# wang-xinyu/tensorrtx

Measured on AMD Instinct MI355X. Metric: images/sec @ batch=32 640x640 fp16 (yolov8n conv backbone + YoloLayer decode + NMS), higher is better.
Workload: dtype f16

## Files before the change

include/trtx_hip.h:

```cpp
#ifndef TRTX_HIP_H_
#define TRTX_HIP_H_

#include <stddef.h>
#include <stdint.h>

#ifdef __cplusplus
extern "C" {
#endif

#ifndef TRTX_NO_HIP_TYPES
struct ihipStream_t;
typedef struct ihipStream_t* trtx_stream_t;
#endif

#define TRTX_ABI_VERSION 1
#define TRTX_OK 0
#define TRTX_ERR_INVALID 1
#define TRTX_ERR_HIP 2
#define TRTX_ERR_WORKSPACE 3
#define TRTX_ERR_UNSUPPORTED 4
#define TRTX_ERR_NO_DEVICE 5
#define TRTX_ERR_IO 6
#define TRTX_ERR_STATE 7

const char* trtx_status_string(int32_t status);
int32_t trtx_abi_version(void);
int32_t trtx_device_count(void);


size_t trtx_yolo_decode_workspace(int batch, int net_h, int net_w, const int* strides, int n_levels);
int32_t trtx_yolo_decode(const float* const* inputs, int n_levels, int batch, int classes, int net_h, int net_w,
                         const int* strides, int max_out, float* output, void* workspace, size_t workspace_bytes,
                         trtx_stream_t stream);

int32_t trtx_yolo_decode_ex(const float* const* inputs, int n_levels, int batch, int classes, int net_h, int net_w,
                            const int* strides, int max_out, int n_kpt, float kpt_conf, int is_seg, int is_pose, int is_obb,
                            float* output, void* workspace, size_t workspace_bytes, trtx_stream_t stream);
size_t trtx_yolo_head_decode_workspace(int batch, int net_h, int net_w, const int* strides, int n_levels);
int32_t trtx_yolo_head_decode_nhwc(const void* const* heads, const int* ld, int n_levels, int batch, int classes,
                                   int net_h, int net_w, const int* strides, const float* dfl_weights, int max_out,
                                   float* output, void* workspace, size_t workspace_bytes, trtx_stream_t stream);
int32_t trtx_yolo_head_decode_nhwc_f32(const void* const* heads, const int* ld, int n_levels, int batch, int classes,
                                   int net_h, int net_w, const int* strides, const float* dfl_weights, int max_out,
                                   float* output, void* workspace, size_t workspace_bytes, trtx_stream_t stream);
int32_t trtx_yolo_task_head_decode_nhwc(const void* const* heads, const int* ld, const void* const* branches, const int* branch_ld,
                                        int n_levels, int batch, int classes, int net_h, int net_w, const int* strides,
                                        const float* dfl_weights, int max_out, int is_seg, int is_pose, int is_obb, int n_kpt,
                                        float kpt_conf, float* output, void* workspace, size_t workspace_bytes, trtx_stream_t stream);
int32_t trtx_yolo_task_head_decode_nhwc_f32(const void* const* heads, const int* ld, const void* const* branches, const int* branch_ld,
                                            int n_levels, int batch, int classes, int net_h, int net_w, const int* strides,
                                            const float* dfl_weights, int max_out, int is_seg, int is_pose, int is_obb, int n_kpt,
                                            float kpt_conf, float* output, void* workspace, size_t workspace_bytes, trtx_stream_t stream);

size_t trtx_yolo_nms_workspace(int batch);
int32_t trtx_yolo_nms(const float* decode_out, int batch, int max_out, float conf_thresh, float nms_thresh,
                      int32_t* keep_idx, int32_t* keep_cnt, float* keep_det, void* workspace, size_t workspace_bytes,
                      trtx_stream_t stream);


size_t trtx_yolov5_decode_workspace(int batch, const int* grid_w, const int* grid_h, int n_levels);
int32_t trtx_yolov5_decode(const float* const* inputs, int n_levels, int batch, int classes, int net_h, int net_w,
                           const int* grid_w, const int* grid_h, const float* anchors, int max_out, int is_segmentation,
                           float* output, void* workspace, size_t workspace_bytes, trtx_stream_t stream);
size_t trtx_yolov5_head_decode_workspace(int batch, const int* grid_w, const int* grid_h, int n_levels);
int32_t trtx_yolov5_head_decode_nhwc(const void* const* heads, const int* ld, int n_levels, int batch, int classes, int net_h, int net_w,
                                     const int* grid_w, const int* grid_h, const float* anchors, int max_out, float* output,
                                     void* workspace, size_t workspace_bytes, trtx_stream_t stream);
int32_t trtx_yolov5_head_decode_nhwc_f32(const void* const* heads, const int* ld, int n_levels, int batch, int classes, int net_h, int net_w,
                                         const int* grid_w, const int* grid_h, const float* anchors, int max_out, float* output,
                                         void* workspace, size_t workspace_bytes, trtx_stream_t stream);
size_t trtx_yolov7_decode_workspace(int batch, const int* grid_w, const int* grid_h, int n_levels);
int32_t trtx_yolov7_decode(const float* const* inputs, int n_levels, int batch, int classes, int net_h, int net_w,
                           const int* grid_w, const int* grid_h, const float* anchors, int max_out, float* output, void* workspace,
                           size_t workspace_bytes, trtx_stream_t stream);
size_t trtx_yolov7_head_decode_workspace(int batch, const int* grid_w, const int* grid_h, int n_levels);
int32_t trtx_yolov7_head_decode_nhwc(const void* const* heads, const int* ld, int n_levels, int batch, int classes, int net_h, int net_w,
                                     const int* grid_w, const int* grid_h, const float* anchors, int max_out, float* output,
                                     void* workspace, size_t workspace_bytes, trtx_stream_t stream);
int32_t trtx_yolov7_head_decode_nhwc_f32(const void* const* heads, const int* ld, int n_levels, int batch, int classes, int net_h, int net_w,
                                         const int* grid_w, const int* grid_h, const float* anchors, int max_out, float* output,
                                         void* workspace, size_t workspace_bytes, trtx_stream_t stream);
size_t trtx_yolov9_decode_workspace(int batch, int net_h, int net_w);
int32_t trtx_yolov9_decode(const float* const* inputs, int batch, int classes, int net_h, int net_w, int max_out, int is_segmentation,
                           float* output, void* workspace, size_t workspace_bytes, trtx_stream_t stream);
size_t trtx_yolov9_head_decode_workspace(int batch, int net_h, int net_w);
int32_t trtx_yolov9_head_decode_nhwc(const void* const* box, const int* box_ld, const void* const* cls, const int* cls_ld, int batch, int classes,
                                     int net_h, int net_w, const float* dfl_weights, int max_out, float* output, void* workspace,
                                     size_t workspace_bytes, trtx_stream_t stream);
int32_t trtx_yolov9_head_decode_nhwc_f32(const void* const* box, const int* box_ld, const void* const* cls, const int* cls_ld, int batch, int classes,
                                         int net_h, int net_w, const float* dfl_weights, int max_out, float* output, void* workspace,
                                         size_t workspace_bytes, trtx_stream_t stream);
int32_t trtx_yolo_nms_obb(const float* decode_out, int batch, int max_out, float conf_thresh, float nms_thresh, int32_t* keep_idx,
                          int32_t* keep_cnt, float* keep_det, void* workspace, size_t workspace_bytes, trtx_stream_t stream);
int32_t trtx_yolo_postprocess_gpu_obb(const float* decode_out, int batch, int max_out, float conf_thresh, float nms_thresh, float* out,
                                      trtx_stream_t stream);
int32_t trtx_yolov5_nms(const float* decode_out, int batch, int max_out, float conf_thresh, float nms_thresh, int32_t* keep_idx,
                        int32_t* keep_cnt, float* keep_det, void* workspace, size_t workspace_bytes, trtx_stream_t stream);
int32_t trtx_yolov9_nms(const float* decode_out, int batch, int max_out, float conf_thresh, float nms_thresh, int32_t* keep_idx,
                        int32_t* keep_cnt, float* keep_det, void* workspace, size_t workspace_bytes, trtx_stream_t stream);
int32_t trtx_yolov7_nms(const float* decode_out, int batch, int max_out, float conf_thresh, float nms_thresh, int32_t* keep_idx,
                        int32_t* keep_cnt, float* keep_det, void* workspace, size_t workspace_bytes, trtx_stream_t stream);
int32_t trtx_seg_masks(const float* decode_out, int det_floats, int box_format, const int32_t* keep_idx, const int32_t* keep_cnt, int batch,
                       int max_out, int max_keep, const float* proto, int mask_h, int mask_w, int net_h, int net_w, float* masks,
                       trtx_stream_t stream);

void trtx_letterbox_matrix(int src_w, int src_h, int dst_w, int dst_h, float* d2s_out );
int32_t trtx_letterbox_batch(const void* const* src, const int* src_w, const int* src_h, int batch, float* dst, int dst_w, int dst_h,
                             trtx_stream_t stream);
int32_t trtx_preprocess_init(int max_image_size, int ring_depth);
void trtx_preprocess_destroy(void);
int32_t trtx_batch_preprocess(const void* const* src_host, const int* src_w, const int* src_h, int batch, float* dst, int dst_w, int dst_h,
                              trtx_stream_t stream);

int32_t trtx_yolo_postprocess_gpu(const float* decode_out, int batch, int max_out, float conf_thresh, float nms_thresh,
                                  float* out, trtx_stream_t stream);

int32_t trtx_mish(const float* in, float* out, size_t n, trtx_stream_t stream);

size_t trtx_retina_decode_output_floats(int net_h, int net_w);
size_t trtx_retina_decode_workspace(int batch, int net_h, int net_w);
int32_t trtx_retina_decode(const float* const* inputs, int batch, int net_h, int net_w, float* output, void* workspace,
                           size_t workspace_bytes, trtx_stream_t stream);
size_t trtx_retina_nms_workspace(int batch, int net_h, int net_w);
int32_t trtx_retina_nms(const float* decode_out, int batch, int net_h, int net_w, double conf_thresh, float nms_thresh,
                        int max_keep, int32_t* keep_idx, int32_t* keep_cnt, float* keep_det, void* workspace,
                        size_t workspace_bytes, trtx_stream_t stream);

size_t trtx_rpn_decode_workspace(int batch, int num_anchors, int height, int width);
int32_t trtx_rpn_decode(int batch, const float* scores, const float* deltas, int height, int width, int image_height,
                        int image_width, float stride, const float* anchors_host, int num_anchors, int top_n,
                        float* out_scores, float* out_boxes, void* workspace, size_t workspace_bytes,
                        trtx_stream_t stream);
size_t trtx_sorted_nms_workspace(int batch, int n);
int32_t trtx_rpn_nms(int batch, const float* scores, const float* boxes, int pre_nms_topk, int post_nms_topk,
                     float nms_thresh, float* out_boxes, void* workspace, size_t workspace_bytes,
                     trtx_stream_t stream);
int32_t trtx_roi_align(int batch, const float* boxes, const float* features, int pooler_resolution, float spatial_scale,
                       int sampling_ratio, int num_proposals, int channels, int feature_h, int feature_w, float* out,
                       trtx_stream_t stream);
int32_t trtx_roi_align_nhwc_f16(int batch, const float* boxes, const void* features, int ld_in, int pooler_resolution,
                                float spatial_scale, int sampling_ratio, int num_proposals, int channels, int feature_h,
                                int feature_w, void* out, int ld_out, trtx_stream_t stream);
int32_t trtx_roi_align_nhwc_f16_strided(int batch, const float* boxes, const void* features, int ld_in, int pooler_resolution,
                                        float spatial_scale, int sampling_ratio, int num_proposals, int channels, int feature_h,
                                        int feature_w, void* out, int ld_out, int bin_step, trtx_stream_t stream);
size_t trtx_predictor_decode_workspace(int batch, int num_boxes, int num_classes);
int32_t trtx_predictor_decode(int batch, const float* scores, const float* deltas, const float* proposals, int num_boxes,
                              int num_classes, int image_height, int image_width, const float* bbox_reg_weights_host,
                              float* out_scores, float* out_boxes, float* out_classes, void* workspace,
                              size_t workspace_bytes, trtx_stream_t stream);
int32_t trtx_batched_nms(int nms_method, int batch, const float* scores, const float* boxes, const float* classes,
                         int count, int detections_per_im, float nms_thresh, float* out_scores, float* out_boxes,
                         float* out_classes, void* workspace, size_t workspace_bytes, trtx_stream_t stream);

int32_t trtx_mask_rcnn_inference(int batch, const float* labels, const float* masks, int detections_per_im, int output_size,
                                 int num_classes, float* out_masks, trtx_stream_t stream);

#define TRTX_ACT_NONE 0
#define TRTX_ACT_RELU 1
#define TRTX_ACT_SIGMOID 2
#define TRTX_ACT_SILU 3
#define TRTX_ACT_LEAKY 4
#define TRTX_ACT_TANH 5
int32_t trtx_conv_packed_dims(int cout, int cin_pad, int kh, int kw, int32_t* cout_pad, int32_t* kpad, int32_t* bn);
int32_t trtx_conv_pack_weights_f16(const float* w_kcrs, int cout, int cin, int kh, int kw, int cin_pad,
                                   const float* ch_scale, uint16_t* packed);
int32_t trtx_op_conv2d_nhwc_f16(const void* in, int N, int H, int W, int Cin, int ld_in, const void* wpacked,
                                const float* bias, void* out, int Cout, int ld_out, int kh, int kw, int sh, int sw,
                                int ph, int pw, int act1, const void* residual, int ld_res, int act2,
                                trtx_stream_t stream);
int32_t trtx_op_conv2d_tactics(int N, int H, int W, int Cin, int ld_in, int Cout, int ld_out, int kh, int kw, int sh, int sw, int ph, int pw,
                               int has_residual, int ld_res, int32_t* out6, int32_t max_out);
int32_t trtx_op_conv_force_tactic(const int32_t* tactic6);
int32_t trtx_op_conv_stem_nchw_f16(const float* in, int N, int C, int H, int W, const float* w_taps_cout, const float* bias, void* out, int Cout,
                                   int ld_out, int k, int stride, int pad, int act, trtx_stream_t stream);
int32_t trtx_op_conv_stem_pair_f16(const float* in, int N, int C, int H, int W, const float* stem_w_taps_cout, const float* stem_bias, int stem_act,
                                   const void* conv_wpacked, const float* conv_bias, int conv_act, void* out, int ld_out, trtx_stream_t stream);
int32_t trtx_op_conv_bneck_pair_f16(const void* in, int N, int H, int W, int ld_in, int in_coff, const void* w1_packed, const float* bias1, int act1,
                                    const void* w2_packed, const float* bias2, int act2, int shortcut, int act_after, void* out, int ld_out,
                                    trtx_stream_t stream);
int32_t trtx_op_conv_bneck_pair_or_two_f16(const void* in, int N, int H, int W, int ld_in, int in_coff, const void* w1_packed, const float* bias1, int act1,
                                           const void* w2_packed, const float* bias2, int act2, int shortcut, int act_after, void* mid, void* out,
                                           int ld_out, trtx_stream_t stream);
int32_t trtx_reorg_fold_weights(const float* w_kcrs, int cout, int cin, int kh, int kw, float* folded);
int32_t trtx_conv_packed_dims_f32(int cout, int cin_pad, int kh, int kw, int32_t* cout_pad, int32_t* kpad, int32_t* cink);
int32_t trtx_conv_pack_weights_f32(const float* w_kcrs, int cout, int cin, int kh, int kw, int cin_pad, const float* ch_scale, float* packed);
int32_t trtx_op_conv2d_nhwc_f32(const void* in, int N, int H, int W, int Cin, int ld_in, const void* wpacked, const float* bias, void* out, int Cout,
                                int ld_out, int kh, int kw, int sh, int sw, int ph, int pw, int act1, const void* residual, int ld_res, int act2,
                                const int32_t* tile4, trtx_stream_t stream);
int32_t trtx_op_conv2d_tactics_f32(int N, int H, int W, int Cin, int ld_in, int Cout, int ld_out, int kh, int kw, int sh, int sw, int ph, int pw,
                                   int has_residual, int ld_res, int32_t* out4, int32_t max_out);
int32_t trtx_conv_pack_weights_i8(const float* w_kcrs, int cout, int cin, int kh, int kw, const float* ch_scale, int8_t* packed, float* wscale_out,
                                  int32_t* cout_pad_out, int32_t* kpad_out);
int32_t trtx_op_conv2d_nhwc_i8(const void* in, int N, int H, int W, int Cin, int ld_in, const void* wpacked, const float* cscale, const float* bias, void* out,
                               int out_is_i8, float out_inv_scale, int Cout, int ld_out, int kh, int kw, int sh, int sw, int ph, int pw, int act1,
                               const void* residual, int res_is_i8, float res_scale, int ld_res, int act2, trtx_stream_t stream);
int32_t trtx_conv_pack_weights_grouped_f16(const float* w_kcrs, int cout, int cin_g, int kh, int kw, const float* ch_scale, uint16_t* packed,
                                           int32_t* kpad_out);
int32_t trtx_op_conv2d_grouped_nhwc_f16(const void* in, int N, int H, int W, int Cin, int ld_in, const void* wpacked, const float* bias, void* out,
                                        int Cout, int ld_out, int groups, int k, int pad, int act1, const void* residual, int ld_res, int act2,
                                        trtx_stream_t stream);
int32_t trtx_op_conv2d_dw_nhwc(const void* in, int dtype, int N, int H, int W, int C, int ld_in, const float* w_taps_c, const float* bias, void* out, int ld_out,
                               const void* residual, int ld_res, int k, int stride, int pad, int dilation, int act1, float alpha1, int act2, float alpha2,
                               trtx_stream_t stream);
int32_t trtx_op_psa_attention_f16(const void* qkv, int ld_qkv, void* out, int ld_out, void* vimg, int ld_v, int B, int heads, int N, int kd, int hd, float scale,
                                  trtx_stream_t stream);
int32_t trtx_op_area_attention_f16(const void* qkv, int ld_qkv, void* out, int ld_out, void* vimg, int ld_v, int B, int heads, int N, int area, int kd, int hd,
                                   float scale, trtx_stream_t stream);
int32_t trtx_op_area_attention_split_f16(const void* q, int ld_q, const void* k, int ld_k, const void* v, int ld_v, void* out, int ld_out, int B, int heads,
                                         int N, int area, int kd, int hd, float scale, trtx_stream_t stream);
size_t trtx_op_hgconv_workspace_bytes(int B, int N, int D, int E);
int32_t trtx_op_hgconv_geometry(int32_t* tiles, int max_tiles, int32_t* n_tiles);
int32_t trtx_op_hgconv_f16(const void* x, int ld_x, void* out, int ld_out, int B, int N, int D, int E, float logit_scale, const float* w_ctx, const float* b_ctx,
                           const float* proto, const float* w_pre, const float* b_pre, const float* w_edge, const float* b_edge, const float* w_node,
                           const float* b_node, void* workspace, size_t workspace_bytes, trtx_stream_t stream);
int32_t trtx_op_poison_lds(void* device_word, trtx_stream_t stream);
int32_t trtx_op_nchw_f32_to_nhwc_f16(const float* in, void* out, int N, int C, int H, int W, int Cpad, int ld_out,
                                     trtx_stream_t stream);
int32_t trtx_op_nhwc_f16_to_nchw_f32(const void* in, float* out, int N, int C, int H, int W, int ld_in,
                                     trtx_stream_t stream);

typedef struct trtx_builder trtx_builder;
typedef struct trtx_network trtx_network;
typedef struct trtx_hostmem trtx_hostmem;
typedef struct trtx_engine trtx_engine;
typedef struct trtx_context trtx_context;
typedef struct trtx_plugin trtx_plugin;

#define TRTX_MAX_DIMS 8
typedef struct trtx_dims {
    int32_t nb;
    int64_t d[TRTX_MAX_DIMS];
} trtx_dims;

#define TRTX_DTYPE_FLOAT 0
#define TRTX_DTYPE_HALF 1
#define TRTX_DTYPE_INT8 2
#define TRTX_DTYPE_INT32 3
#define TRTX_ACTIVATION_RELU 0
#define TRTX_ACTIVATION_SIGMOID 1
#define TRTX_ACTIVATION_TANH 2
#define TRTX_ACTIVATION_LEAKY_RELU 3
#define TRTX_POOLING_MAX 0
#define TRTX_POOLING_AVERAGE 1
#define TRTX_ELEMENTWISE_SUM 0
#define TRTX_ELEMENTWISE_PROD 1
#define TRTX_ELEMENTWISE_MAX 2
#define TRTX_ELEMENTWISE_MIN 3
#define TRTX_ELEMENTWISE_SUB 4
#define TRTX_ELEMENTWISE_DIV 5
#define TRTX_ELEMENTWISE_POW 6
#define TRTX_SCALE_UNIFORM 0
#define TRTX_SCALE_CHANNEL 1
#define TRTX_SCALE_ELEMENTWISE 2
#define TRTX_REDUCE_SUM 0
#define TRTX_REDUCE_PROD 1
#define TRTX_REDUCE_MAX 2
#define TRTX_REDUCE_MIN 3
#define TRTX_REDUCE_AVG 4
#define TRTX_MATMUL_NONE 0
#define TRTX_MATMUL_TRANSPOSE 1
#define TRTX_MATMUL_VECTOR 2
#define TRTX_UNARY_EXP 0
#define TRTX_UNARY_LAST 23
#define TRTX_RESIZE_NEAREST 0
#define TRTX_RESIZE_LINEAR 1
#define TRTX_FLAG_FP16 0
#define TRTX_FLAG_INT8 1
#define TRTX_P_STRIDE 1
#define TRTX_P_PADDING 2
#define TRTX_P_DILATION 3
#define TRTX_P_GROUPS 4
#define TRTX_P_ALPHA 5
#define TRTX_P_BETA 6
#define TRTX_P_AXIS 7
#define TRTX_P_RESHAPE 8
#define TRTX_P_FIRST_TRANSPOSE 9
#define TRTX_P_SECOND_TRANSPOSE 10
#define TRTX_P_RESIZE_MODE 11
#define TRTX_P_RESIZE_SCALES 12
#define TRTX_P_RESIZE_OUT_DIMS 13
#define TRTX_P_AVG_EXCLUSIVE 14
#define TRTX_P_KERNEL 15
#define TRTX_P_NB_OUT 16

typedef struct trtx_plugin_vtbl {
    void* self;
    int32_t (*get_nb_outputs)(void* self);
    int32_t (*get_output_dims)(void* self, int32_t index, const trtx_dims* inputs, int32_t nb_inputs, trtx_dims* out);
    int32_t (*configure)(void* self, const trtx_dims* in, int32_t nb_in, const trtx_dims* out, int32_t nb_out,
                         int32_t max_batch);
    int32_t (*initialize)(void* self);
    void (*terminate)(void* self);
    size_t (*workspace_size)(void* self, int32_t max_batch);
    int32_t (*enqueue)(void* self, int32_t batch, const void* const* inputs, void* const* outputs, void* workspace,
                       trtx_stream_t stream);
    size_t (*serialization_size)(void* self);
    void (*serialize)(void* self, void* buffer);
    const char* (*plugin_type)(void* self);
    const char* (*plugin_version)(void* self);
    int32_t (*clone)(void* self, struct trtx_plugin_vtbl* out);
    void (*destroy)(void* self);
} trtx_plugin_vtbl;

typedef struct trtx_plugin_field {
    const char* name;
    const void* data;
    int32_t type;
    int32_t length;
} trtx_plugin_field;

typedef struct trtx_creator_vtbl {
    void* self;
    const char* (*plugin_name)(void* self);
    const char* (*plugin_version)(void* self);
    int32_t (*create)(void* self, const char* name, const trtx_plugin_field* fields, int32_t nb_fields,
                      trtx_plugin_vtbl* out);
    int32_t (*deserialize)(void* self, const char* name, const void* data, size_t length, trtx_plugin_vtbl* out);
} trtx_creator_vtbl;

int32_t trtx_registry_register(const trtx_creator_vtbl* creator);
int32_t trtx_registry_get(const char* name, const char* version, trtx_creator_vtbl* out);

typedef struct trtx_wts trtx_wts;
int32_t trtx_wts_load(const char* path, trtx_wts** out);
int32_t trtx_wts_count(const trtx_wts* w);
int32_t trtx_wts_entry(const trtx_wts* w, int32_t i, const char** name, const float** values, int64_t* count);
int32_t trtx_wts_find(const trtx_wts* w, const char* name, const float** values, int64_t* count);
void trtx_wts_free(trtx_wts* w);

int32_t trtx_builder_create(trtx_builder** out);
void trtx_builder_destroy(trtx_builder* b);
int32_t trtx_builder_set_max_batch(trtx_builder* b, int32_t n);
int32_t trtx_builder_set_flag(trtx_builder* b, int32_t flag, int32_t on);
int32_t trtx_builder_set_workspace(trtx_builder* b, size_t bytes);
typedef struct trtx_calibrator_vtbl {
    void* self;
    int32_t (*get_batch_size)(void* self);
    int32_t (*get_batch)(void* self, void** bindings, const char* const* names, int32_t nb_bindings);
    const void* (*read_cache)(void* self, size_t* length);
    void (*write_cache)(void* self, const void* cache, size_t length);
    int32_t (*get_algorithm)(void* self);
} trtx_calibrator_vtbl;
int32_t trtx_builder_set_max_aux_streams(trtx_builder* b, int32_t n);
int32_t trtx_builder_set_int8_calibrator(trtx_builder* b, const trtx_calibrator_vtbl* calibrator);
float trtx_int8_entropy_threshold(const double* hist, int32_t bins, float range);
float trtx_int8_clip_limited_threshold(const double* hist, int32_t bins, float range, float thr, double limit);
int32_t trtx_network_create(trtx_builder* b, uint32_t flags, trtx_network** out);
void trtx_network_destroy(trtx_network* n);
const char* trtx_network_last_error(const trtx_network* n);

int32_t trtx_add_input(trtx_network* n, const char* name, int32_t dtype, const trtx_dims* dims);
int32_t trtx_add_convolution(trtx_network* n, int32_t input, int32_t nb_out, int32_t kh, int32_t kw,
                             const float* kernel, int64_t kernel_count, const float* bias, int64_t bias_count);
int32_t trtx_add_deconvolution(trtx_network* n, int32_t input, int32_t nb_out, int32_t kh, int32_t kw,
                               const float* kernel, int64_t kernel_count, const float* bias, int64_t bias_count);
int32_t trtx_add_fully_connected(trtx_network* n, int32_t input, int32_t nb_out, const float* kernel,
                                 int64_t kernel_count, const float* bias, int64_t bias_count);
int32_t trtx_add_activation(trtx_network* n, int32_t input, int32_t type);
int32_t trtx_add_pooling(trtx_network* n, int32_t input, int32_t type, int32_t kh, int32_t kw);
int32_t trtx_add_scale(trtx_network* n, int32_t input, int32_t mode, const float* shift, int64_t shift_count,
                       const float* scale, int64_t scale_count, const float* power, int64_t power_count);
int32_t trtx_add_elementwise(trtx_network* n, int32_t a, int32_t b, int32_t op);
int32_t trtx_add_concatenation(trtx_network* n, const int32_t* inputs, int32_t nb_inputs);
int32_t trtx_add_slice(trtx_network* n, int32_t input, const trtx_dims* start, const trtx_dims* size,
                       const trtx_dims* stride);
int32_t trtx_add_shuffle(trtx_network* n, int32_t input);
int32_t trtx_add_resize(trtx_network* n, int32_t input);
int32_t trtx_add_softmax(trtx_network* n, int32_t input);
int32_t trtx_add_matrix_multiply(trtx_network* n, int32_t a, int32_t op_a, int32_t b, int32_t op_b);
int32_t trtx_add_constant(trtx_network* n, const trtx_dims* dims, const float* values, int64_t count);
int32_t trtx_add_reduce(trtx_network* n, int32_t input, int32_t op, uint32_t axes, int32_t keep_dims);
int32_t trtx_add_identity(trtx_network* n, int32_t input);
int32_t trtx_network_add_unary(trtx_network* n, int32_t input, int32_t op);
int32_t trtx_add_plugin_v2(trtx_network* n, const int32_t* inputs, int32_t nb_inputs, const trtx_plugin_vtbl* plugin);

int32_t trtx_layer_nb_outputs(const trtx_network* n, int32_t layer);
int32_t trtx_layer_output(const trtx_network* n, int32_t layer, int32_t index);
int32_t trtx_layer_set_name(trtx_network* n, int32_t layer, const char* name);
int32_t trtx_layer_set_ints(trtx_network* n, int32_t layer, int32_t param, const int32_t* v, int32_t count);
int32_t trtx_layer_set_floats(trtx_network* n, int32_t layer, int32_t param, const float* v, int32_t count);
int32_t trtx_layer_set_dims(trtx_network* n, int32_t layer, int32_t param, const trtx_dims* d);
int32_t trtx_tensor_get_dims(const trtx_network* n, int32_t tensor, trtx_dims* out);
int32_t trtx_tensor_set_name(trtx_network* n, int32_t tensor, const char* name);
const char* trtx_tensor_get_name(const trtx_network* n, int32_t tensor);
int32_t trtx_mark_output(trtx_network* n, int32_t tensor);

int32_t trtx_build_serialized(trtx_builder* b, trtx_network* n, trtx_hostmem** out);
const void* trtx_hostmem_data(const trtx_hostmem* m);
size_t trtx_hostmem_size(const trtx_hostmem* m);
void trtx_hostmem_destroy(trtx_hostmem* m);
int32_t trtx_hostmem_create(const void* data, size_t size, trtx_hostmem** out);
int32_t trtx_plan_describe(const void* plan, size_t size, int32_t lowered, char** json_out);
void trtx_string_free(char* s);

int32_t trtx_engine_deserialize(const void* plan, size_t size, trtx_engine** out);
int32_t trtx_engine_serialize(const trtx_engine* e, trtx_hostmem** out);
void trtx_engine_destroy(trtx_engine* e);
int32_t trtx_engine_nb_bindings(const trtx_engine* e);
int32_t trtx_engine_binding_index(const trtx_engine* e, const char* name);
const char* trtx_engine_binding_name(const trtx_engine* e, int32_t index);
int32_t trtx_engine_binding_is_input(const trtx_engine* e, int32_t index);
int32_t trtx_engine_binding_dims(const trtx_engine* e, int32_t index, trtx_dims* out);
int32_t trtx_engine_binding_dtype(const trtx_engine* e, int32_t index);
int32_t trtx_engine_max_batch(const trtx_engine* e);
size_t trtx_engine_device_memory(const trtx_engine* e);
int32_t trtx_engine_tactics(const trtx_engine* e, char** json_out);
int32_t trtx_engine_device(const trtx_engine* e);
int32_t trtx_context_create(trtx_engine* e, trtx_context** out);
void trtx_context_destroy(trtx_context* c);
int32_t trtx_context_enqueue(trtx_context* c, int32_t batch, void* const* bindings, trtx_stream_t stream);
int32_t trtx_context_enqueue_frames(trtx_context* c, int32_t batch, const void* const* frames, const int32_t* frame_w, const int32_t* frame_h,
                                    void* const* bindings, trtx_stream_t stream);
int32_t trtx_context_set_tensor_address(trtx_context* c, const char* name, void* ptr);
int32_t trtx_context_enqueue_v3(trtx_context* c, trtx_stream_t stream);
int32_t trtx_context_profile(trtx_context* c, int32_t batch, void* const* bindings, trtx_stream_t stream,
                             char** json_out);

#ifdef __cplusplus
}
#endif
#endif
```

tensorrtx_amd/capi.py:

```python
import ctypes
import os

_HERE = os.path.dirname(os.path.abspath(__file__))
_LIB = None


class TrtxError(RuntimeError):
    def __init__(self, status, what):
        self.status = status
        msg = lib().trtx_status_string(status).decode() if _LIB is not None else "?"
        super().__init__(f"{what}: status {status} ({msg})")


def lib_path() -> str:
    return os.environ.get("TRTX_HIP_LIB") or os.path.join(_HERE, "lib", "libtrtx_hip.so")


def hip_runtimes_mapped():
    seen = []
    with open("/proc/self/maps") as f:
        for line in f:
            path = line.rsplit(" ", 1)[-1].strip()
            if "libamdhip64" in os.path.basename(path) and path not in seen:
                seen.append(path)
# ... 154 lines not shown
        return status
    check(status, "trtx_yolo_task_head_decode_nhwc")
    return out


def yolo_nms_obb(decode_out, max_out=1000, conf_thresh=0.5, nms_thresh=0.45, out=None, ws=None):
    L = lib()
    B = decode_out.shape[0]
    keep_idx, keep_cnt, keep_det, ws = _nms_buffers(B, max_out, 7, decode_out.device, out, ws)
    check(L.trtx_yolo_nms_obb(_p(decode_out), B, max_out, ctypes.c_float(conf_thresh), ctypes.c_float(nms_thresh), _p(keep_idx), _p(keep_cnt),
                              _p(keep_det), _p(ws), ctypes.c_size_t(ws.numel()), _stream()), "trtx_yolo_nms_obb")
    return keep_idx, keep_cnt, keep_det


def yolo_postprocess_gpu_obb(decode_out, max_out=1000, conf_thresh=0.5, nms_thresh=0.45, out=None, ws=None):
    import torch
    if out is None:
        out = torch.empty((decode_out.shape[0], 1 + max_out * 8), dtype=torch.float32, device=decode_out.device)
    check(lib().trtx_yolo_postprocess_gpu_obb(_p(decode_out), decode_out.shape[0], max_out, ctypes.c_float(conf_thresh), ctypes.c_float(nms_thresh),
                                              _p(out), _stream()), "trtx_yolo_postprocess_gpu_obb")
    return out


DET5_FLOATS = 38


def yolov5_decode(inputs, classes, net_h, net_w, grids, anchors, max_out=1000, is_seg=False):
    import numpy as np
    import torch
    L = lib()
    n = len(inputs)
    ins = [x.contiguous() for x in inputs]
    B, dev = ins[0].shape[0], ins[0].device
    arr = (ctypes.c_void_p * n)(*[x.data_ptr() for x in ins])
    gw = (ctypes.c_int * n)(*[g[0] for g in grids])
    gh = (ctypes.c_int * n)(*[g[1] for g in grids])
    an = np.ascontiguousarray(anchors, dtype=np.float32).reshape(n, 6)
    L.trtx_yolov5_decode_workspace.restype = ctypes.c_size_t
    ws_bytes = L.trtx_yolov5_decode_workspace(B, gw, gh, n)
    ws = torch.empty(max(ws_bytes, 256), dtype=torch.uint8, device=dev)
    out = torch.zeros((B, 1 + max_out * DET5_FLOATS), dtype=torch.float32, device=dev)
    check(L.trtx_yolov5_decode(arr, n, B, classes, net_h, net_w, gw, gh, an.ctypes.data_as(ctypes.c_void_p), max_out, 1 if is_seg else 0,
                               _p(out), _p(ws), ctypes.c_size_t(ws_bytes), _stream()), "trtx_yolov5_decode")
    return out


def yolov5_head_decode_nhwc(heads, classes, net_h, net_w, grids, anchors, max_out=1000):
    import numpy as np
    import torch
    L = lib()
    B, n, dev = heads[0].shape[0], len(heads), heads[0].device
    hp, hl = _head_table(heads)
    gw = (ctypes.c_int * n)(*[g[0] for g in grids])
    gh = (ctypes.c_int * n)(*[g[1] for g in grids])
    an = np.ascontiguousarray(anchors, dtype=np.float32).reshape(n, 6)
    L.trtx_yolov5_head_decode_workspace.restype = ctypes.c_size_t
    ws_bytes = L.trtx_yolov5_head_decode_workspace(B, gw, gh, n)
    ws = torch.empty(max(ws_bytes, 256), dtype=torch.uint8, device=dev)
    out = torch.zeros((B, 1 + max_out * DET5_FLOATS), dtype=torch.float32, device=dev)
    fn = L.trtx_yolov5_head_decode_nhwc_f32 if heads[0].dtype == torch.float32 else L.trtx_yolov5_head_decode_nhwc
    check(fn(hp, hl, n, B, classes, net_h, net_w, gw, gh, an.ctypes.data_as(ctypes.c_void_p), max_out, _p(out), _p(ws), ctypes.c_size_t(ws_bytes),
             _stream()), "trtx_yolov5_head_decode_nhwc")
    return out


def yolov5_nms(decode_out, max_out=1000, conf_thresh=0.5, nms_thresh=0.45, out=None, ws=None):
    L = lib()
    B = decode_out.shape[0]
    keep_idx, keep_cnt, keep_det, ws = _nms_buffers(B, max_out, 6, decode_out.device, out, ws)
    check(L.trtx_yolov5_nms(_p(decode_out), B, max_out, ctypes.c_float(conf_thresh), ctypes.c_float(nms_thresh), _p(keep_idx), _p(keep_cnt),
                            _p(keep_det), _p(ws), ctypes.c_size_t(ws.numel()), _stream()), "trtx_yolov5_nms")
    return keep_idx, keep_cnt, keep_det


def reorg_fold_weights(w):
    import numpy as np
    w = np.ascontiguousarray(w, dtype=np.float32)
    cout, c4, kh, kw = w.shape
    out = np.empty((cout, c4 // 4, 2 * kh, 2 * kw), dtype=np.float32)
    check(lib().trtx_reorg_fold_weights(w.ctypes.data_as(ctypes.c_void_p), cout, c4 // 4, kh, kw, out.ctypes.data_as(ctypes.c_void_p)),
          "trtx_reorg_fold_weights")
    return out


DET7_FLOATS = 6


def _grid_tables(grids, anchors, n):
    import numpy as np
    gw = (ctypes.c_int * max(n, 1))(*[g[0] for g in grids[:n]])
    gh = (ctypes.c_int * max(n, 1))(*[g[1] for g in grids[:n]])
    an = np.ascontiguousarray(anchors, dtype=np.float32).reshape(-1, 6)
    return gw, gh, an


def yolov7_decode(inputs, classes, net_h, net_w, grids, anchors, max_out=1000, out=None):
    import torch
    L = lib()
    n = len(inputs)
    ins = [x.contiguous() for x in inputs]
    B, dev = ins[0].shape[0], ins[0].device
    arr = (ctypes.c_void_p * n)(*[x.data_ptr() for x in ins])
    gw, gh, an = _grid_tables(grids, anchors, n)
    L.trtx_yolov7_decode_workspace.restype = ctypes.c_size_t
    ws_bytes = L.trtx_yolov7_decode_workspace(B, gw, gh, n)
    ws = torch.empty(max(ws_bytes, 256), dtype=torch.uint8, device=dev)
    if out is None:
        out = torch.zeros((B, 1 + max_out * DET7_FLOATS), dtype=torch.float32, device=dev)
    check(L.trtx_yolov7_decode(arr, n, B, classes, net_h, net_w, gw, gh, an.ctypes.data_as(ctypes.c_void_p), max_out, _p(out), _p(ws),
                               ctypes.c_size_t(ws_bytes), _stream()), "trtx_yolov7_decode")
    return out


def yolov7_head_decode_workspace(batch, grids):
    L = lib()
    n = len(grids)
    gw, gh, _ = _grid_tables(grids, [0.0] * 6 * n, n)
    L.trtx_yolov7_head_decode_workspace.restype = ctypes.c_size_t
    return L.trtx_yolov7_head_decode_workspace(batch, gw, gh, n)


def yolov7_head_decode_nhwc(heads, classes, net_h, net_w, grids, anchors, max_out=1000, out=None, ws=None, ld=None, n_levels=None,
                            status_only=False):
    import torch
    L = lib()
    B, n, dev = heads[0].shape[0], len(heads), heads[0].device
    hp, hl = _head_table(heads)
    if ld is not None:
        hl = (ctypes.c_int * n)(*ld)
    gw, gh, an = _grid_tables(grids, anchors, n)
    if ws is None:
        ws = torch.empty(max(yolov7_head_decode_workspace(B, grids), 256), dtype=torch.uint8, device=dev)
    if out is None:
        out = torch.zeros((B, 1 + max_out * DET7_FLOATS), dtype=torch.float32, device=dev)
    fn = L.trtx_yolov7_head_decode_nhwc_f32 if heads[0].dtype == torch.float32 else L.trtx_yolov7_head_decode_nhwc
    st = fn(hp, hl, n if n_levels is None else n_levels, B, classes, net_h, net_w, gw, gh, an.ctypes.data_as(ctypes.c_void_p), max_out, _p(out),
            _p(ws), ctypes.c_size_t(ws.numel()), _stream())
    if status_only:
        return st
    check(st, "trtx_yolov7_head_decode_nhwc")
    return out


def yolov7_nms(decode_out, max_out=1000, conf_thresh=0.5, nms_thresh=0.45, out=None, ws=None):
    L = lib()
    B = decode_out.shape[0]
    keep_idx, keep_cnt, keep_det, ws = _nms_buffers(B, max_out, 6, decode_out.device, out, ws)
    check(L.trtx_yolov7_nms(_p(decode_out), B, max_out, ctypes.c_float(conf_thresh), ctypes.c_float(nms_thresh), _p(keep_idx), _p(keep_cnt),
                            _p(keep_det), _p(ws), ctypes.c_size_t(ws.numel()), _stream()), "trtx_yolov7_nms")
    return keep_idx, keep_cnt, keep_det


def yolov9_decode(inputs, classes, net_h, net_w, max_out=1000, is_seg=False, out=None):
    import torch
    L = lib()
    ins = [x.contiguous() for x in inputs]
    assert len(ins) == 3 and all(x.is_cuda and x.dtype == torch.float32 for x in ins)
    B, dev = ins[0].shape[0], ins[0].device
    arr = (ctypes.c_void_p * 3)(*[x.data_ptr() for x in ins])
    L.trtx_yolov9_decode_workspace.restype = ctypes.c_size_t
    ws_bytes = L.trtx_yolov9_decode_workspace(B, net_h, net_w)
    ws = torch.empty(max(ws_bytes, 256), dtype=torch.uint8, device=dev)
    if out is None:
        out = torch.zeros((B, 1 + max_out * DET5_FLOATS), dtype=torch.float32, device=dev)
    check(L.trtx_yolov9_decode(arr, B, classes, net_h, net_w, max_out, 1 if is_seg else 0, _p(out), _p(ws), ctypes.c_size_t(ws_bytes), _stream()),
          "trtx_yolov9_decode")
    return out


def yolov9_head_decode_nhwc(box, cls, classes, net_h, net_w, dfl_w, max_out=1000, out=None, batch=None, box_ld=None, cls_ld=None, ws=None):
    import torch
    L = lib()
    assert len(box) == 3 and len(cls) == 3
    B = box[0].shape[0] if batch is None else batch
    dev = box[0].device
    bp = (ctypes.c_void_p * 3)(*[x.data_ptr() for x in box])
    cp = (ctypes.c_void_p * 3)(*[x.data_ptr() for x in cls])
    bl = (ctypes.c_int * 3)(*(box_ld if box_ld is not None else [x.shape[-1] for x in box]))
    cl = (ctypes.c_int * 3)(*(cls_ld if cls_ld is not None else [x.shape[-1] for x in cls]))
    L.trtx_yolov9_head_decode_workspace.restype = ctypes.c_size_t
    if ws is None:
        ws = torch.empty(max(L.trtx_yolov9_head_decode_workspace(B, net_h, net_w), 256), dtype=torch.uint8, device=dev)
    if out is None:
        out = torch.zeros((B, 1 + max_out * DET5_FLOATS), dtype=torch.float32, device=dev)
    fn = L.trtx_yolov9_head_decode_nhwc_f32 if box[0].dtype == torch.float32 else L.trtx_yolov9_head_decode_nhwc
    check(fn(bp, bl, cp, cl, B, classes, net_h, net_w, _p(dfl_w), max_out, _p(out), _p(ws), ctypes.c_size_t(ws.numel()), _stream()),
          "trtx_yolov9_head_decode_nhwc")
    return out


def yolov9_nms(decode_out, max_out=1000, conf_thresh=0.5, nms_thresh=0.45, out=None, ws=None):
    L = lib()
    B = decode_out.shape[0]
    keep_idx, keep_cnt, keep_det, ws = _nms_buffers(B, max_out, 6, decode_out.device, out, ws)
    check(L.trtx_yolov9_nms(_p(decode_out), B, max_out, ctypes.c_float(conf_thresh), ctypes.c_float(nms_thresh), _p(keep_idx), _p(keep_cnt),
                            _p(keep_det), _p(ws), ctypes.c_size_t(ws.numel()), _stream()), "trtx_yolov9_nms")
    return keep_idx, keep_cnt, keep_det


def seg_masks(decode_out, keep_idx, keep_cnt, proto, net_h, net_w, max_keep, box_format=0, out=None):
    import torch
    B, max_out = keep_idx.shape
    assert decode_out.shape[0] == B and (decode_out.shape[1] - 1) % max_out == 0
    det_floats = (decode_out.shape[1] - 1) // max_out
    assert proto.dim() == 4 and proto.shape[0] == B and proto.shape[1] == 32
    mask_h, mask_w = int(proto.shape[2]), int(proto.shape[3])
    for t, dt in ((decode_out, torch.float32), (keep_idx, torch.int32), (keep_cnt, torch.int32), (proto, torch.float32)):
        assert t.is_cuda and t.dtype == dt and t.is_contiguous()
    if out is None:
        out = torch.zeros((B, max(max_keep, 0), mask_h, mask_w), dtype=torch.float32, device=proto.device)
    assert out.is_cuda and out.dtype == torch.float32 and out.is_contiguous() and out.numel() >= B * max(max_keep, 0) * mask_h * mask_w
    check(lib().trtx_seg_masks(_p(decode_out), det_floats, box_format, _p(keep_idx), _p(keep_cnt), B, max_out, max_keep, _p(proto), mask_h,
                               mask_w, net_h, net_w, _p(out), _stream()), "trtx_seg_masks")
    return out


def yolo_postprocess_gpu(decode_out, max_out=1000, conf_thresh=0.5, nms_thresh=0.45, out=None, ws=None):
    import torch
    B = decode_out.shape[0]
    if out is None:
        out = torch.empty((B, 1 + max_out * 7), dtype=torch.float32, device=decode_out.device)
    check(lib().trtx_yolo_postprocess_gpu(_p(decode_out), B, max_out, ctypes.c_float(conf_thresh), ctypes.c_float(nms_thresh),
                                          _p(out), _stream()), "trtx_yolo_postprocess_gpu")
    return out


ACT = {"none": 0, "relu": 1, "sigmoid": 2, "silu": 3, "leaky": 4, "tanh": 5, "mish": 6}


def _hw(v):
    if isinstance(v, (tuple, list)):
        h, w = v
        return int(h), int(w)
    return int(v), int(v)


def pack_conv_weights_f16(w_kcrs, cin_pad=None, ch_scale=None):
    import numpy as np
    L = lib()
    w = np.ascontiguousarray(w_kcrs, dtype=np.float32)
    cout, cin, kh, kw = w.shape
    cin_pad = cin_pad or (cin + 7) // 8 * 8
    cp, kp, bn = ctypes.c_int32(), ctypes.c_int32(), ctypes.c_int32()
    check(L.trtx_conv_packed_dims(cout, cin_pad, kh, kw, ctypes.byref(cp), ctypes.byref(kp), ctypes.byref(bn)),
          "trtx_conv_packed_dims")
    packed = np.zeros((cp.value, kp.value), dtype=np.uint16)
    sc = None
    if ch_scale is not None:
        sc = np.ascontiguousarray(ch_scale, dtype=np.float32)
    check(L.trtx_conv_pack_weights_f16(w.ctypes.data_as(ctypes.c_void_p), cout, cin, kh, kw, cin_pad,
                                       sc.ctypes.data_as(ctypes.c_void_p) if sc is not None else None,
                                       packed.ctypes.data_as(ctypes.c_void_p)), "trtx_conv_pack_weights_f16")
    return packed, cp.value, kp.value, bn.value


def conv2d_nhwc_f16(x, wpacked, bias, cout, kh, kw, stride, pad, act1="none", residual=None, act2="none",
                    out=None, out_ld=None):
    import torch
    L = lib()
    N, H, W, Cin = x.shape
    (sh, sw), (ph, pw) = _hw(stride), _hw(pad)
    Ho = (H + 2 * ph - kh) // sh + 1
    Wo = (W + 2 * pw - kw) // sw + 1
    if out is None:
        out = torch.empty((N, Ho, Wo, cout), dtype=torch.float16, device=x.device)
    ld_out = out_ld or out.shape[-1]
    check(L.trtx_op_conv2d_nhwc_f16(_p(x), N, H, W, Cin, x.stride(2), _p(wpacked), _p(bias), _p(out), cout, ld_out,
                                    kh, kw, sh, sw, ph, pw, ACT[act1], _p(residual),
                                    residual.stride(2) if residual is not None else 0, ACT[act2], _stream()),
          "trtx_op_conv2d_nhwc_f16")
    return out


def stem_weights(w_kcrs):
    import numpy as np
    w = np.ascontiguousarray(w_kcrs, dtype=np.float32)
    return np.ascontiguousarray(w.reshape(w.shape[0], -1).T)


def conv_stem_nchw_f16(x, w_taps_cout, bias, k, stride, pad, act="none", out=None, out_ld=None):
    import torch
    N, C, H, W = x.shape
    cout = w_taps_cout.shape[1]
    Ho, Wo = (H + 2 * pad - k) // stride + 1, (W + 2 * pad - k) // stride + 1
    if out is None:
        out = torch.empty((N, Ho, Wo, cout), dtype=torch.float16, device=x.device)
    check(lib().trtx_op_conv_stem_nchw_f16(_p(x), N, C, H, W, _p(w_taps_cout), _p(bias), _p(out), cout, out_ld or out.shape[-1], k, stride, pad,
                                           ACT[act], _stream()), "trtx_op_conv_stem_nchw_f16")
    return out


def conv_stem_pair_f16(x, stem_w_taps_cout, stem_bias, conv_wpacked, conv_bias, stem_act="silu", conv_act="silu", out=None, out_ld=None):
    import torch
    N, C, H, W = x.shape
    Hi, Wi = (H - 1) // 2 + 1, (W - 1) // 2 + 1
    Ho, Wo = (Hi - 1) // 2 + 1, (Wi - 1) // 2 + 1
    if out is None:
        out = torch.empty((N, Ho, Wo, 32), dtype=torch.float16, device=x.device)
    check(lib().trtx_op_conv_stem_pair_f16(_p(x), N, C, H, W, _p(stem_w_taps_cout), _p(stem_bias), ACT[stem_act], _p(conv_wpacked), _p(conv_bias),
                                           ACT[conv_act], _p(out), out_ld or out.shape[-1], _stream()), "trtx_op_conv_stem_pair_f16")
    return out


def conv_bneck_pair_f16(x, w1_packed, bias1, w2_packed, bias2, act1="silu", act2="silu", shortcut=True, act_after="none", out=None, out_ld=None, in_coff=None,
                        mid=None):
    import torch
    N, H, W, C = x.shape
    assert x.dtype == torch.float16 and x.stride(3) == 1 and (C == 16 if in_coff is None else in_coff + 16 <= C)
    if out is None:
        out = torch.empty((N, H, W, 16), dtype=torch.float16, device=x.device)
    head = (_p(x), N, H, W, x.stride(2), in_coff or 0, _p(w1_packed), _p(bias1), ACT[act1], _p(w2_packed), _p(bias2), ACT[act2], 1 if shortcut else 0, ACT[act_after])
    if mid is None:
        check(lib().trtx_op_conv_bneck_pair_f16(*head, _p(out), out_ld or out.shape[-1], _stream()), "trtx_op_conv_bneck_pair_f16")
    else:
        assert mid.dtype == torch.float16 and mid.is_contiguous() and tuple(mid.shape) == (N, H, W, 16)
        check(lib().trtx_op_conv_bneck_pair_or_two_f16(*head, _p(mid), _p(out), out_ld or out.shape[-1], _stream()), "trtx_op_conv_bneck_pair_or_two_f16")
    return out


def pack_conv_weights_grouped_f16(w_kcrs, ch_scale=None):
    import numpy as np
    L = lib()
    w = np.ascontiguousarray(w_kcrs, dtype=np.float32)
    cout, cin_g, kh, kw = w.shape
    kp = ctypes.c_int32()
    check(L.trtx_conv_pack_weights_grouped_f16(w.ctypes.data_as(ctypes.c_void_p), cout, cin_g, kh, kw, None, None, ctypes.byref(kp)),
          "trtx_conv_pack_weights_grouped_f16 (dims)")
    packed = np.zeros((cout, kp.value), dtype=np.uint16)
    sc = None if ch_scale is None else np.ascontiguousarray(ch_scale, dtype=np.float32)
    check(L.trtx_conv_pack_weights_grouped_f16(w.ctypes.data_as(ctypes.c_void_p), cout, cin_g, kh, kw,
                                               sc.ctypes.data_as(ctypes.c_void_p) if sc is not None else None,
                                               packed.ctypes.data_as(ctypes.c_void_p), ctypes.byref(kp)), "trtx_conv_pack_weights_grouped_f16")
    return packed


def conv2d_grouped_nhwc_f16(x, wpacked, bias, cout, groups, k, pad, act1="none", residual=None, act2="none", out=None, out_ld=None):
    import torch
    N, H, W, Cin = x.shape
    if out is None:
        out = torch.empty((N, H + 2 * pad - k + 1, W + 2 * pad - k + 1, cout), dtype=torch.float16, device=x.device)
    check(lib().trtx_op_conv2d_grouped_nhwc_f16(_p(x), N, H, W, Cin, x.stride(2), _p(wpacked), _p(bias), _p(out), cout, out_ld or out.shape[-1], groups, k,
                                                pad, ACT[act1], _p(residual), residual.stride(2) if residual is not None else 0, ACT[act2], _stream()),
          "trtx_op_conv2d_grouped_nhwc_f16")
    return out


def conv2d_dw_nhwc(x, w, bias, k, stride, act1="none", residual=None, act2="none", out=None, out_ld=None, alpha1=0.1, alpha2=0.1, pad=None, dilation=1):
    import numpy as np
    import torch
    N, H, W, C = x.shape
    assert x.dtype in (torch.float16, torch.float32) and (residual is None or residual.dtype == x.dtype)
    pad = k // 2 if pad is None else pad
    Ho, Wo = (H + 2 * pad - dilation * (k - 1) - 1) // stride + 1, (W + 2 * pad - dilation * (k - 1) - 1) // stride + 1
    taps = np.ascontiguousarray(np.asarray(w, dtype=np.float32).reshape(C, k * k).T)
    wg = torch.from_numpy(taps).to(x.device)
    if out is None:
        out = torch.empty((N, Ho, Wo, C), dtype=x.dtype, device=x.device)
    assert out.dtype == x.dtype
    check(lib().trtx_op_conv2d_dw_nhwc(_p(x), 1 if x.dtype == torch.float16 else 0, N, H, W, C, x.stride(2), _p(wg), _p(bias), _p(out),
                                       out_ld or out.shape[-1], _p(residual), residual.stride(2) if residual is not None else 0, k, stride, pad, dilation,
                                       ACT[act1], ctypes.c_float(alpha1), ACT[act2], ctypes.c_float(alpha2), _stream()), "trtx_op_conv2d_dw_nhwc")
    return out


def _attention(fn, what, qkv, heads, scale, out, vimg, out_ld, v_ld, qkv_ld, kd, hd, extra):
    import torch
    B, N, _ = qkv.shape
    for t in (qkv, out, vimg):
        assert t.is_cuda and t.dtype == torch.float16
    check(fn(_p(qkv), qkv_ld or qkv.stride(1), _p(out), out_ld or out.stride(1), _p(vimg), v_ld or vimg.stride(1), B, heads, N, *extra, kd, hd,
             ctypes.c_float(scale), _stream()), what)
    return out, vimg


def psa_attention(qkv, heads, scale, out=None, vimg=None, out_ld=None, v_ld=None, qkv_ld=None, kd=32, hd=64):
    import torch
    B, N, _ = qkv.shape
    out = torch.empty((B, N, heads * hd), dtype=torch.float16, device=qkv.device) if out is None else out
    vimg = torch.empty((B, N, heads * hd), dtype=torch.float16, device=qkv.device) if vimg is None else vimg
    return _attention(lib().trtx_op_psa_attention_f16, "trtx_op_psa_attention_f16", qkv, heads, scale, out, vimg, out_ld, v_ld, qkv_ld, kd, hd, ())


def area_attention(qkv, heads, area, scale, out=None, vimg=None, out_ld=None, v_ld=None, qkv_ld=None, kd=32, hd=32):
    import torch
    B, N, _ = qkv.shape
    out = torch.empty((B, N, heads * hd), dtype=torch.float16, device=qkv.device) if out is None else out
    vimg = torch.empty((B, N, heads * hd), dtype=torch.float16, device=qkv.device) if vimg is None else vimg
    return _attention(lib().trtx_op_area_attention_f16, "trtx_op_area_attention_f16", qkv, heads, scale, out, vimg, out_ld, v_ld, qkv_ld, kd, hd, (area,))


def area_attention_split(q, k, v, heads, area, scale, out=None, q_ld=None, k_ld=None, v_ld=None, out_ld=None, kd=32, hd=32):
    import torch
    B, N, _ = q.shape
    out = torch.empty((B, N, heads * hd), dtype=torch.float16, device=q.device) if out is None else out
    for t in (q, k, v, out):
        assert t.is_cuda and t.dtype == torch.float16
    check(lib().trtx_op_area_attention_split_f16(_p(q), q_ld or q.stride(1), _p(k), k_ld or k.stride(1), _p(v), v_ld or v.stride(1), _p(out),
                                                 out_ld or out.stride(1), B, heads, N, area, kd, hd, ctypes.c_float(scale), _stream()),
          "trtx_op_area_attention_split_f16")
    return out


HGCONV_WEIGHTS = ("w_ctx", "b_ctx", "proto", "w_pre", "b_pre", "w_edge", "b_edge", "w_node", "b_node")


def hgconv_workspace_bytes(B, N, D, E):
    L = lib()
    L.trtx_op_hgconv_workspace_bytes.restype = ctypes.c_size_t
    return int(L.trtx_op_hgconv_workspace_bytes(int(B), int(N), int(D), int(E)))


def hgconv_geometry():
    arr, n = (ctypes.c_int32 * 8)(), ctypes.c_int32()
    check(lib().trtx_op_hgconv_geometry(arr, 8, ctypes.byref(n)), "trtx_op_hgconv_geometry")
    return [int(arr[i]) for i in range(min(n.value, 8))]


def hgconv(x, E, logit_scale, weights, out=None, x_ld=None, out_ld=None, D=None, workspace=None):
    import torch
    L = lib()
    B, N, Dx = x.shape
    D = Dx if D is None else D
    assert x.is_cuda and x.dtype == torch.float16
    out = torch.empty((B, N, D), dtype=torch.float16, device=x.device) if out is None else out
    assert out.is_cuda and out.dtype == torch.float16
    ws = workspace if workspace is not None else torch.empty(max(hgconv_workspace_bytes(B, N, D, E), 256), dtype=torch.uint8, device=x.device)
    ws_arr = [weights[k].contiguous() for k in HGCONV_WEIGHTS]
    for w in ws_arr:
        assert w.is_cuda and w.dtype == torch.float32
    L.trtx_op_hgconv_f16.argtypes = ([ctypes.c_void_p, ctypes.c_int, ctypes.c_void_p, ctypes.c_int] + [ctypes.c_int] * 4 + [ctypes.c_float] +
                                     [ctypes.c_void_p] * 9 + [ctypes.c_void_p, ctypes.c_size_t, ctypes.c_void_p])
    check(L.trtx_op_hgconv_f16(_p(x), x_ld or x.stride(1), _p(out), out_ld or out.stride(1), B, N, D, E, float(logit_scale), *[_p(w) for w in ws_arr],
                               _p(ws), ws.numel(), _stream()), "trtx_op_hgconv_f16")
    return out


def pack_conv_weights_f32(w_kcrs, cin_pad=None, ch_scale=None):
    import numpy as np
    L = lib()
    w = np.ascontiguousarray(w_kcrs, dtype=np.float32)
    cout, cin, kh, kw = w.shape
    cin_pad = cin_pad or (cin + 3) // 4 * 4
    cp, kp, ck = ctypes.c_int32(), ctypes.c_int32(), ctypes.c_int32()
    check(L.trtx_conv_packed_dims_f32(cout, cin_pad, kh, kw, ctypes.byref(cp), ctypes.byref(kp), ctypes.byref(ck)), "trtx_conv_packed_dims_f32")
    packed = np.zeros((cp.value, kp.value), dtype=np.float32)
    sc = np.ascontiguousarray(ch_scale, dtype=np.float32) if ch_scale is not None else None
    check(L.trtx_conv_pack_weights_f32(w.ctypes.data_as(ctypes.c_void_p), cout, cin, kh, kw, cin_pad,
                                       sc.ctypes.data_as(ctypes.c_void_p) if sc is not None else None,
                                       packed.ctypes.data_as(ctypes.c_void_p)), "trtx_conv_pack_weights_f32")
    return packed, cp.value, kp.value, ck.value


def conv2d_nhwc_f32(x, wpacked, bias, cout, kh, kw, stride, pad, act1="none", residual=None, act2="none", out=None, out_ld=None, tile=None):
    import torch
    L = lib()
    N, H, W, Cin = x.shape
    if bias is not None and bias.numel() < (cout + 15) // 16 * 16:
        raise ValueError(f"bias holds {bias.numel()} floats, the fp32 tile reads cout_pad = {(cout + 15) // 16 * 16}")
    (sh, sw), (ph, pw) = _hw(stride), _hw(pad)
    Ho = (H + 2 * ph - kh) // sh + 1
    Wo = (W + 2 * pw - kw) // sw + 1
    if out is None:
        out = torch.empty((N, Ho, Wo, cout), dtype=torch.float32, device=x.device)
    ld_out = out_ld or out.shape[-1]
    t2 = (ctypes.c_int32 * 4)(*tile) if tile is not None else None
    check(L.trtx_op_conv2d_nhwc_f32(_p(x), N, H, W, Cin, x.stride(2), _p(wpacked), _p(bias), _p(out), cout, ld_out, kh, kw, sh, sw, ph, pw,
                                    ACT[act1], _p(residual), residual.stride(2) if residual is not None else 0, ACT[act2], t2, _stream()),
          "trtx_op_conv2d_nhwc_f32")
    return out


def conv2d_tactics_f32(N, H, W, Cin, Cout, k, stride, pad, residual=False, ld_in=None, ld_out=None, ld_res=None, max_out=32):
    arr = (ctypes.c_int32 * (4 * max_out))()
    (kh, kw), (sh, sw), (ph, pw) = _hw(k), _hw(stride), _hw(pad)
    n = lib().trtx_op_conv2d_tactics_f32(N, H, W, Cin, ld_in or Cin, Cout, ld_out or Cout, kh, kw, sh, sw, ph, pw, 1 if residual else 0,
                                         (ld_res or Cout) if residual else 0, arr, max_out)
    return [(arr[4 * i], arr[4 * i + 1], arr[4 * i + 2], arr[4 * i + 3]) for i in range(n)]


def poison_lds(sync=True):
    import torch
    w = torch.zeros(4, dtype=torch.int32, device="cuda")
    check(lib().trtx_op_poison_lds(_p(w), _stream()), "trtx_op_poison_lds")
    if sync:
        torch.cuda.synchronize()


def conv2d_tactics(N, H, W, Cin, Cout, k, stride, pad, residual=False, ld_in=None, ld_out=None, ld_res=None, max_out=32):
    arr = (ctypes.c_int32 * (6 * max_out))()
    (kh, kw), (sh, sw), (ph, pw) = _hw(k), _hw(stride), _hw(pad)
    n = lib().trtx_op_conv2d_tactics(N, H, W, Cin, ld_in or Cin, Cout, ld_out or Cout, kh, kw, sh, sw, ph, pw, 1 if residual else 0,
                                     (ld_res or Cout) if residual else 0, arr, max_out)
    return [tuple(arr[6 * i + j] for j in range(6)) for i in range(n)]


def conv_force_tactic(tactic=None):
    if tactic is None:
        check(lib().trtx_op_conv_force_tactic(None), "trtx_op_conv_force_tactic")
    else:
        check(lib().trtx_op_conv_force_tactic((ctypes.c_int32 * 6)(*tactic)), "trtx_op_conv_force_tactic")


def pack_conv_weights_i8(w_kcrs, ch_scale=None):
    import numpy as np
    L = lib()
    w = np.ascontiguousarray(w_kcrs, dtype=np.float32)
    cout, cin, kh, kw = w.shape
    cp, kp = ctypes.c_int32(), ctypes.c_int32()
    check(L.trtx_conv_pack_weights_i8(w.ctypes.data_as(ctypes.c_void_p), cout, cin, kh, kw, None, None, None, ctypes.byref(cp), ctypes.byref(kp)),
          "trtx_conv_pack_weights_i8 (dims)")
    packed = np.zeros((cp.value, kp.value), dtype=np.int8)
    wscale = np.zeros((cp.value,), dtype=np.float32)
    sc = None if ch_scale is None else np.ascontiguousarray(ch_scale, dtype=np.float32)
    check(L.trtx_conv_pack_weights_i8(w.ctypes.data_as(ctypes.c_void_p), cout, cin, kh, kw,
                                      sc.ctypes.data_as(ctypes.c_void_p) if sc is not None else None, packed.ctypes.data_as(ctypes.c_void_p),
                                      wscale.ctypes.data_as(ctypes.c_void_p), ctypes.byref(cp), ctypes.byref(kp)), "trtx_conv_pack_weights_i8")
    return packed, wscale


def conv2d_nhwc_i8(x_i8, wpacked, cscale, bias, cout, kh, kw, stride, pad, act1="none", out_scale=None, residual=None, res_scale=1.0,
                   act2="none", out=None, out_ld=None):
    import torch
    N, H, W, Cin = x_i8.shape
    (sh, sw), (ph, pw) = _hw(stride), _hw(pad)
    Ho, Wo = (H + 2 * ph - kh) // sh + 1, (W + 2 * pw - kw) // sw + 1
    if out is None:
        out = torch.empty((N, Ho, Wo, cout), dtype=torch.int8 if out_scale else torch.float16, device=x_i8.device)
    res_i8 = residual is not None and residual.dtype == torch.int8
    check(lib().trtx_op_conv2d_nhwc_i8(_p(x_i8), N, H, W, Cin, x_i8.stride(2), _p(wpacked), _p(cscale), _p(bias), _p(out), 1 if out_scale else 0,
                                       ctypes.c_float(1.0 / out_scale if out_scale else 0.0), cout, out_ld or out.shape[-1], kh, kw, sh, sw, ph, pw, ACT[act1],
                                       _p(residual), 1 if res_i8 else 0, ctypes.c_float(res_scale), residual.stride(2) if residual is not None else 0,
                                       ACT[act2], _stream()), "trtx_op_conv2d_nhwc_i8")
    return out
```

tensorrtx_amd/csrc/kernels/conv_stem_pair.hip:

```cpp
#include <hip/hip_fp16.h>
#include <hip/hip_runtime.h>
#include <stdint.h>

#include "../common.h"
#include "act.h"
#include "kernels.h"
#include "launch.h"
#include "stem_pair_index.h"
#include "stem_tile.h"

namespace trtx {
namespace {

namespace px = pairidx;

constexpr int kPairPatchBytesMax = (4 * px::kPR * px::kPCA / 4 + 255) / 256 * 256 * 16;
static_assert(kPairPatchBytesMax + px::kImageBytes <= 80 * 1024, "two workgroups per CU and room for other contexts");

__device__ __forceinline__ size_t pair_patch_bytes(int cin) { return (size_t)((cin * px::kPR * px::kPCA / 4 + 255) / 256 * 256) * 16; }

__global__ __launch_bounds__(256) void conv_stem_pair_kernel(const ConvArgs ps, const ConvArgs p1, const StemGeom g, unsigned in_bytes, int total_tiles) {
    extern __shared__ __attribute__((aligned(16))) float s_patch[];
    char* const s_img = reinterpret_cast<char*>(s_patch) + pair_patch_bytes(ps.Cin);
    const int tid = threadIdx.x;
    const int lane = tid & 63;
    const int wave = __builtin_amdgcn_readfirstlane(tid >> 6);
    const int grp = lane >> 4, col = lane & 15;

    StemRegs<1, 1> R;
    stem_setup<1, 1>(ps, g, R);
    half8 w1[2][px::kSteps];
    {
        const _Float16* __restrict__ w = static_cast<const _Float16*>(p1.wgt);
#pragma unroll
        for (int j = 0; j < 2; ++j)
#pragma unroll
            for (int kt = 0; kt < px::kSteps; ++kt)
                w1[j][kt] = *reinterpret_cast<const half8*>(w + (size_t)px::weight_row_channel(j, col) * p1.Kpad + kt * 32 + grp * 8);
    }
    float4 b0 = make_float4(0.f, 0.f, 0.f, 0.f), b1 = b0;
    if (p1.bias) {
        b0 = *reinterpret_cast<const float4*>(p1.bias + grp * 8);
        b1 = *reinterpret_cast<const float4*>(p1.bias + grp * 8 + 4);
    }
    _Float16* __restrict__ out = static_cast<_Float16*>(p1.out);

    auto fetch = [&](int tile) {
        const px::Tile t = px::tile_of(tile, g.tiles_x, g.tiles_y);
        stem_patch_fetch(ps, g, in_bytes, s_patch, t.n, px::patch_start(t.y0), px::patch_aligned_start(px::patch_start(t.x0)));
    };
    if ((int)blockIdx.x < total_tiles) fetch(blockIdx.x);
    for (int tile = blockIdx.x; tile < total_tiles; tile += gridDim.x) {
        const px::Tile t = px::tile_of(tile, g.tiles_x, g.tiles_y);
        const int hi_start = px::patch_start(t.y0), wi_start = px::patch_start(t.x0);
        const int al_start = px::patch_aligned_start(wi_start);
        const int shift = wi_start - al_start;
        asm volatile("s_waitcnt vmcnt(0)" ::: "memory");
        __syncthreads();
        stem_patch_tail(ps, g, s_patch, t.n, hi_start, al_start);
        const int iy0 = px::region_start(t.y0), ix0 = px::region_start(t.x0);
#pragma nounroll
        for (int gi = wave; gi < px::kGroups; gi += 4) {
            const px::RegionPixel rp = px::region_pixel(gi, lane);
            floatx4 acc[1];
            stem_group_mfma<1, 1>(R, s_patch + px::patch_offset(rp.ry, rp.rx, shift), acc);
            half4 o = stem_finish4(ps, acc[0], R.bias4[0]);
            const int iy = iy0 + rp.ry, ix = ix0 + rp.rx;
            if ((unsigned)iy >= (unsigned)p1.H || (unsigned)ix >= (unsigned)p1.W) o = half4{0, 0, 0, 0};
            if (rp.live) *reinterpret_cast<half4*>(s_img + px::image_offset(rp.ry, rp.rx, grp * 4)) = o;
        }
        __syncthreads();
        const int next = tile + (int)gridDim.x;
        if (next < total_tiles) fetch(next);
        floatx4 acc[2][2];
#pragma unroll
        for (int i = 0; i < 2; ++i)
#pragma unroll
            for (int j = 0; j < 2; ++j) acc[i][j] = floatx4{0.f, 0.f, 0.f, 0.f};
#pragma unroll
        for (int kt = 0; kt < px::kSteps; ++kt) {
            const int tap = px::step_tap(kt, lane);
            half8 xf[2];
#pragma unroll
            for (int i = 0; i < 2; ++i) {
                xf[i] = half8{0, 0, 0, 0, 0, 0, 0, 0};
                if (tap < px::kTaps) xf[i] = *reinterpret_cast<const half8*>(s_img + px::frag_offset(2 * wave + i, col, tap, px::step_chunk(lane)));
            }
#pragma unroll
            for (int j = 0; j < 2; ++j)
#pragma unroll
                for (int i = 0; i < 2; ++i) acc[i][j] = __builtin_amdgcn_mfma_f32_16x16x32_f16(w1[j][kt], xf[i], acc[i][j], 0, 0, 0);
        }
#pragma unroll
        for (int i = 0; i < 2; ++i) {
            const int ho = t.y0 + 2 * wave + i, wo = t.x0 + col;
            if (ho >= p1.Ho || wo >= p1.Wo) continue;
            float x[8] = {acc[i][0][0], acc[i][0][1], acc[i][0][2], acc[i][0][3], acc[i][1][0], acc[i][1][1], acc[i][1][2], acc[i][1][3]};
            if (p1.bias) {
                x[0] += b0.x; x[1] += b0.y; x[2] += b0.z; x[3] += b0.w;
                x[4] += b1.x; x[5] += b1.y; x[6] += b1.z; x[7] += b1.w;
            }
            half8 v;
            if (p1.act1 == ACT_SILU) {
#pragma unroll
                for (int e = 0; e < 8; ++e) v[e] = round_to_half(x[e] * __builtin_amdgcn_rcpf(1.0f + __expf(-x[e])));
            } else if (p1.act1 == ACT_RELU) {
#pragma unroll
                for (int e = 0; e < 8; ++e) v[e] = round_to_half(x[e] > 0.f ? x[e] : 0.f);
            } else {
#pragma unroll
                for (int e = 0; e < 8; ++e) v[e] = round_to_half(x[e]);
            }
            const size_t m = ((size_t)t.n * p1.Ho + ho) * p1.Wo + wo;
            *reinterpret_cast<half8*>(out + m * p1.ld_out + grp * 8) = v;
        }
    }
}

}

bool conv_stem_pair_possible(const ConvArgs& s, const ConvArgs& c) {
    const bool stem_ok = conv_stem_supported(s) && !s.f32 && s.Cin <= 4 && s.Cout == 16 && s.kh == 3 && s.kw == 3 && s.stride_h == 2 && s.stride_w == 2 &&
                         s.pad_h == 1 && s.pad_w == 1 && s.N >= 1 && (size_t)s.N * s.Cin * s.H * s.W * 4 < 2000000000u &&
                         s.Ho == (s.H - 1) / 2 + 1 && s.Wo == (s.W - 1) / 2 + 1;
    const bool fast_act = c.act1 == ACT_SILU || c.act1 == ACT_RELU || c.act1 == ACT_NONE;
    const bool conv_ok = !c.f32 && !c.in_i8 && !c.out_i8 && !c.res_i8 && !c.residual && !c.up_C && c.act2 == ACT_NONE && fast_act && !c.scalar_out &&
                         c.groups == 1 && c.dil_h == 1 && c.dil_w == 1 && c.Cin == 16 && c.CinK == 16 && c.bk == 32 && c.Kpad == 160 && c.Cout == 32 &&
                         c.Cout_pad == 32 && c.kh == 3 && c.kw == 3 && c.stride_h == 2 && c.stride_w == 2 && c.pad_h == 1 && c.pad_w == 1 &&
                         c.ld_out % 8 == 0 && c.ld_out >= 32;
    const bool chained = c.N == s.N && c.H == s.Ho && c.W == s.Wo && c.Ho == (c.H - 1) / 2 + 1 && c.Wo == (c.W - 1) / 2 + 1;
    const bool aligned = (reinterpret_cast<uintptr_t>(s.in) & 15) == 0 && (reinterpret_cast<uintptr_t>(c.out) & 15) == 0 &&
                         (reinterpret_cast<uintptr_t>(c.wgt) & 15) == 0 && (reinterpret_cast<uintptr_t>(c.bias) & 15) == 0;
    return stem_ok && conv_ok && chained && aligned;
}

int32_t conv_stem_pair_f16(const ConvArgs& s, const ConvArgs& c, hipStream_t stream) {
    if (!conv_stem_pair_possible(s, c) || !s.in || !s.wgt || !c.wgt || !c.out) return TRTX_ERR_UNSUPPORTED;
    namespace px = pairidx;
    StemGeom g;
    g.PR = px::kPR;
    g.PCA = px::kPCA;
    g.tiles_x = (c.Wo + px::kTW - 1) / px::kTW;
    g.tiles_y = (c.Ho + px::kTH - 1) / px::kTH;
    g.chunks = s.Cin * g.PR * g.PCA / 4;
    const size_t lds = (size_t)((g.chunks + 255) / 256 * 256) * 16 + px::kImageBytes;
    const unsigned in_bytes = (unsigned)((size_t)s.N * s.Cin * s.H * s.W * 4);
    const long total_l = (long)s.N * g.tiles_x * g.tiles_y;
    if (total_l > 0x7fffffffL - 65536) return TRTX_ERR_UNSUPPORTED;
    const int total = (int)total_l;
    static thread_local int resident[3] = {-1, 0, 0};
    int dev = 0;
    if (hipGetDevice(&dev) != hipSuccess) dev = 0;
    if (resident[0] != dev || resident[1] != (int)lds || resident[2] <= 0) {
        int per_cu = 0, cus = 0;
        if (hipOccupancyMaxActiveBlocksPerMultiprocessor(&per_cu, conv_stem_pair_kernel, 256, lds) != hipSuccess || per_cu < 1) per_cu = 1;
        if (hipDeviceGetAttribute(&cus, hipDeviceAttributeMultiprocessorCount, dev) != hipSuccess || cus < 1) cus = 256;
        (void)hipGetLastError();
        resident[0] = dev;
        resident[1] = (int)lds;
        resident[2] = per_cu * cus;
    }
    const int grid = total < resident[2] ? total : resident[2];
    TRTX_LAUNCH(conv_stem_pair_kernel, dim3((unsigned)grid), dim3(256), lds, stream, s, c, g, in_bytes, total);
    return check_launch("conv_stem_pair_f16");
}

}
```

tensorrtx_amd/csrc/kernels/kernels.h:

```cpp
#pragma once
#include <hip/hip_runtime.h>
#include <stddef.h>
#include <stdint.h>

namespace trtx {

enum Act : int { ACT_NONE = 0, ACT_RELU = 1, ACT_SIGMOID = 2, ACT_SILU = 3, ACT_LEAKY = 4, ACT_TANH = 5,
                 ACT_MISH = 6 ,
                 ACT_GELU_TANH = 7 ,
                 ACT_EXP = 8  };
enum DType : int { DT_F32 = 0, DT_F16 = 1, DT_I8 = 2 };
inline size_t dtype_size(int dt) { return dt == DT_F16 ? 2 : (dt == DT_I8 ? 1 : 4); }
enum EwOp : int { EW_SUM = 0, EW_PROD = 1, EW_MAX = 2, EW_MIN = 3, EW_SUB = 4, EW_DIV = 5, EW_POW = 6 };
enum PoolOp : int { POOL_MAX = 0, POOL_AVG = 1 };

enum Ws : int {
    WS_AUTO = 0,
    WS_OFF = 1,
    WS_ON = 2,
    WS_PATCH = 3,
    WS_F32_REGS = 5,
    WS_F32_ROLES = 6,
    WS_RES3 = 7,
    WS_RES1 = 8,
};
enum Wsk : int {
    WSK_RULE = 0,
    WSK_OFF = 1,
    WSK_ON = 2,
};

struct ConvArgs {
    const void* in;
    const void* wgt;
    const float* bias;
    void* out;
    const void* residual;
    int N, H, W, Cin, ld_in;
    int Ho, Wo, Cout, Cout_pad, ld_out, ld_res;
    int kh, kw, stride_h, stride_w, pad_h, pad_w, dil_h, dil_w, groups;
    int K, Kpad, M;
    int act1, act2;
    float alpha1, alpha2;
    int bn;
    int scalar_out;
    int CinK;
    int bk;
    int in_i8, out_i8, res_i8;
    const float* cscale;
    float out_inv_scale, res_scale;
    int bm;
    int t_wsk;
    int t_ws;
    int t_rs;
    const void* up_in;
    int up_C, up_ld, up_H, up_W;
    int f32;
    int k_pinned;
};

struct ConvTactic {
    int bn, bk, bm;
    int wsk, ws;
};

struct LaunchProbe {
    hipEvent_t start = nullptr, stop = nullptr;
    int launches = 0;
};
void conv_set_launch_probe(LaunchProbe* p);
LaunchProbe* conv_launch_probe();

int conv_igemm_pick_bn(int cout);
int conv_igemm_pick_bk(int cin, int taps);
int conv_igemm_pick_cink(int cin, int bk);
bool conv_igemm_supported(const ConvArgs& a);
void conv_pack_weights_i8(const float* w_kcrs, int cout, int cin, int kh, int kw, int cink, const float* ch_scale, int cout_pad, int kpad,
                          int8_t* packed, float* wscale_out);
int32_t conv_igemm_f16(const ConvArgs& a, hipStream_t s);
int conv_tactics(const ConvArgs& a, ConvTactic* out, int max_out, bool work_efficient_only = false);
void conv_apply_tactic(ConvArgs* a, const ConvTactic& t);
constexpr int kMaxConvGroup = 4;
bool conv_igemm_group_supported(const ConvArgs* a, int n);
int32_t conv_igemm_group_f16(const ConvArgs* a, int n, hipStream_t s);
bool conv_gemm256_possible(const ConvArgs& a);
bool conv_gemm256_worthwhile(const ConvArgs& a);
int32_t conv_gemm256_f16(const ConvArgs& a, hipStream_t s);
int conv_igemm_f32_pick_cink(int cin);
bool conv_igemm_f32_supported(const ConvArgs& a);
int32_t conv_igemm_f32(const ConvArgs& a, hipStream_t s);
int conv_tactics_f32(const ConvArgs& a, ConvTactic* out, int max_out);
void conv_pack_weights_igemm_f32(const float* w_kcrs, int cout, int cin, int kh, int kw, int cink, int kpad, int cout_pad, const float* ch_scale, float* packed);
bool conv_res_possible(const ConvArgs& a);
bool conv_res_group_possible(const ConvArgs* a, int n);
int32_t conv_res_f16(const ConvArgs* a, int n, hipStream_t s);
bool conv_res1_possible(const ConvArgs& a);
int32_t conv_res1_f16(const ConvArgs& a, hipStream_t s);
bool conv_ws_supported(const ConvArgs& a);
int32_t conv_ws_f16(const ConvArgs& a, hipStream_t s);
int32_t poison_lds(unsigned* device_word, hipStream_t s);
bool conv_stem_supported(const ConvArgs& a);
int32_t conv_stem_nchw_f32(const ConvArgs& a, hipStream_t s);
bool conv_stem_f32_supported(const ConvArgs& a);
int32_t conv_stem_nchw_f32_out_f32(const ConvArgs& a, hipStream_t s);
constexpr int kStemMaxFrames = 64;
struct StemFrame {
    const void* src;
    int w, h;
    float d2s[6];
};
int32_t conv_stem_frames_f32(const ConvArgs& a, const StemFrame* frames, hipStream_t s);
bool conv_stem_pair_possible(const ConvArgs& stem, const ConvArgs& conv);
int32_t conv_stem_pair_f16(const ConvArgs& stem, const ConvArgs& conv, hipStream_t s);
bool conv_bneck_pair_possible(const ConvArgs& first, const ConvArgs& second);
int32_t conv_bneck_pair_f16(const ConvArgs& first, const ConvArgs& second, hipStream_t s);
int32_t conv_bneck_pair_or_two_f16(const ConvArgs& first, const ConvArgs& second, hipStream_t s);
int32_t conv_direct(const ConvArgs& a, int dtype, hipStream_t s);
bool conv_dw_supported(const ConvArgs& a);
bool psa_attention_supported(int kd, int hd);
int32_t psa_attention_f16(const void* qkv, int ld_qkv, void* out, int ld_out, void* vimg, int ld_v, int B, int heads, int N, int kd, int hd,
                          float scale, hipStream_t s);
bool area_attention_supported(int kd, int hd);
int32_t area_attention_f16(const void* qkv, int ld_qkv, void* out, int ld_out, void* vimg, int ld_v, int B, int heads, int N, int area, int kd,
                           int hd, float scale, hipStream_t s);
bool area_attention_split_supported(int kd, int hd);
int32_t area_attention_split_f16(const void* q, int ld_q, const void* k, int ld_k, const void* v, int ld_v, void* out, int ld_out, int B, int heads, int N,
                                 int area, int kd, int hd, float scale, hipStream_t s);
int32_t conv_dw(const ConvArgs& a, int dtype, hipStream_t s);
struct HgconvWeights {
    const float* w_ctx;
    const float* b_ctx;
    const float* proto;
    const float* w_pre;
    const float* b_pre;
    const float* w_edge;
    const float* b_edge;
    const float* w_node;
    const float* b_node;
};
bool hgconv_supported(int D, int E);
size_t hgconv_workspace_bytes(int B, int N, int D, int E);
int hgconv_geometry(int32_t* tiles, int max_tiles);
int32_t hgconv_f16(const void* x, int ld_x, void* out, int ld_out, int B, int N, int D, int E, float logit_scale, const HgconvWeights& w, void* workspace,
                   size_t workspace_bytes, hipStream_t s);
bool conv_grouped_supported(const ConvArgs& a);
int conv_grouped_kpad(const ConvArgs& a);
int32_t conv_grouped(const ConvArgs& a, hipStream_t s);
int32_t deconv_direct(const ConvArgs& a, int dtype, hipStream_t s);

int32_t nchw_f32_to_nhwc(const float* in, void* out, int dtype, int N, int C, int H, int W, int Cpad, int ld_out,
                         hipStream_t s);
int32_t nhwc_to_nchw_f32(const void* in, int dtype, float* out, int N, int C, int H, int W, int ld_in, hipStream_t s);

int32_t nhwc_maxpool_chain3_f16(const void* in, void* o1, void* o2, void* o3, int N, int H, int W, int C, int ld_in, int ld1,
                                int ld2, int ld3, int k, hipStream_t s, int f32 = 0);
int32_t nhwc_depth_to_space_f16(const void* in, void* out, int N, int H, int W, int C, int bh, int bw, int ld_in, int ld_out,
                                hipStream_t s);
int32_t nhwc_pool(const void* in, void* out, int dtype, int op, int N, int H, int W, int C, int ld_in, int Ho, int Wo,
                  int ld_out, int kh, int kw, int sh, int sw, int ph, int pw, int avg_exclusive, hipStream_t s);
int32_t nhwc_resize_nearest(const void* in, void* out, int dtype, int N, int H, int W, int C, int ld_in, int Ho,
                            int Wo, int ld_out, hipStream_t s);
int32_t nhwc_elementwise(const void* a, const void* b, void* out, int dtype, int op, long pixels, int C, int ld_a,
                         int ld_b, int ld_out, hipStream_t s);
int32_t nhwc_activation(const void* in, void* out, int dtype, int act, float alpha, long pixels, int C, int ld_in,
                        int ld_out, hipStream_t s);
int32_t nhwc_gated_add(const void* a, const void* b, const float* gate, void* out, int dtype, long pixels, int C, int ld_a, int ld_b, int ld_out,
                       hipStream_t s);
int32_t nhwc_scale(const void* in, void* out, int dtype, const float* scale, const float* shift, long pixels, int C,
                   int ld_in, int ld_out, hipStream_t s);
int32_t nhwc_copy(const void* in, void* out, int dtype, long pixels, int C, int ld_in, int ld_out, hipStream_t s);
int32_t nhwc_reduce_hw_avg(const void* in, void* out, int dtype, int N, int HW, int C, int ld_in, int ld_out,
                           hipStream_t s);

int32_t nhwc_absmax_f16(const void* x, long pixels, int C, int ld, unsigned* out_float_bits, hipStream_t s);
int32_t nhwc_hist_f16(const void* x, long pixels, int C, int ld, float range, unsigned long long* hist8192, hipStream_t s);
int32_t nhwc_resize_nearest_i8(const void* in, void* out, int N, int H, int W, int C, int ld_in, int Ho, int Wo, int ld_out, float ratio,
                               hipStream_t s);

struct StridedView {
    int rank;
    long shape[6];
    long stride_in[6];
    long stride_in2[6];
};
int32_t lin_gather(const float* in, float* out, const StridedView& v, hipStream_t s);
int32_t lin_scatter(const float* in, float* out, const StridedView& v, hipStream_t s);
int32_t lin_elementwise(const float* a, const float* b, float* out, int op, const StridedView& v, hipStream_t s);
int32_t lin_activation(const float* in, float* out, int act, float alpha, long n, hipStream_t s);
int32_t lin_softmax(const float* in, float* out, long outer, long axis, long inner, hipStream_t s);
int32_t lin_matmul(const float* A, const float* B, float* C, int batch, int M, int N, int K, int ta, int tb,
                   long bsA, long bsB, hipStream_t s, int binner = 1, long bsA2 = 0, long bsB2 = 0);
int32_t lin_reduce(const float* in, float* out, int op , long outer, long axis, long inner,
                   hipStream_t s);
int32_t lin_scale(const float* in, float* out, const float* scale, const float* shift, const float* power, int mode,
                  long outer, long C, long inner, hipStream_t s);

}
```

tensorrtx_amd/csrc/ops_capi.cpp:

```cpp
#include <hip/hip_runtime.h>
#include <stdlib.h>
#include <string.h>

#include <vector>

#include "common.h"
#include "options.h"
#include "kernels/kernels.h"
#include "runtime/pack.h"

using namespace trtx;

extern "C" const char* trtx_status_string(int32_t s) {
    switch (s) {
        case TRTX_OK: return "ok";
        case TRTX_ERR_INVALID: return "invalid argument";
        case TRTX_ERR_HIP: return "HIP error";
        case TRTX_ERR_WORKSPACE: return "workspace too small";
        case TRTX_ERR_UNSUPPORTED: return "unsupported configuration";
        case TRTX_ERR_NO_DEVICE: return "no HIP device";
        case TRTX_ERR_IO: return "I/O or parse error";
        case TRTX_ERR_STATE: return "invalid call order";
        default: return "unknown status";
    }
}

extern "C" int32_t trtx_abi_version(void) {
    return TRTX_ABI_VERSION;
}

extern "C" int32_t trtx_device_count(void) {
    int n = 0;
    if (hipGetDeviceCount(&n) != hipSuccess) {
        (void)hipGetLastError();
        return 0;
    }
    return n;
}

extern "C" int32_t trtx_conv_packed_dims(int cout, int cin_pad, int kh, int kw, int32_t* cout_pad, int32_t* kpad,
                                         int32_t* bn) {
    if (cout < 1 || cin_pad < 1 || kh < 1 || kw < 1) return TRTX_ERR_INVALID;
    const int b = conv_igemm_pick_bn(cout);
    if (bn) *bn = b;
    if (cout_pad) *cout_pad = (cout + b - 1) / b * b;
    if (kpad) {
        const int bk = conv_igemm_pick_bk(cin_pad, kh * kw);
        *kpad = (kh * kw * conv_igemm_pick_cink(cin_pad, bk) + bk - 1) / bk * bk;
    }
    return TRTX_OK;
}

extern "C" int32_t trtx_conv_pack_weights_f16(const float* w_kcrs, int cout, int cin, int kh, int kw, int cin_pad,
                                              const float* ch_scale, uint16_t* packed) {
    if (!w_kcrs || !packed || cin_pad < cin) return TRTX_ERR_INVALID;
    const int bk = conv_igemm_pick_bk(cin_pad, kh * kw);
    pack_conv_weights_f16(w_kcrs, cout, cin, kh, kw, conv_igemm_pick_cink(cin_pad, bk), bk, ch_scale, packed);
    return TRTX_OK;
}

static ConvArgs op_conv_args(int N, int H, int W, int Cin, int ld_in, int Cout, int ld_out, int kh, int kw, int sh, int sw, int ph, int pw,
                             int act1, int has_res, int ld_res, int act2) {
    ConvArgs a{};
    a.N = N; a.H = H; a.W = W; a.Cin = Cin; a.ld_in = ld_in;
    a.Ho = (H + 2 * ph - kh) / sh + 1;
    a.Wo = (W + 2 * pw - kw) / sw + 1;
    a.Cout = Cout;
    a.bn = conv_igemm_pick_bn(Cout);
    a.Cout_pad = (Cout + a.bn - 1) / a.bn * a.bn;
    a.ld_out = ld_out; a.ld_res = ld_res;
    a.kh = kh; a.kw = kw; a.stride_h = sh; a.stride_w = sw; a.pad_h = ph; a.pad_w = pw; a.dil_h = 1; a.dil_w = 1;
    a.groups = 1;
    a.bk = conv_igemm_pick_bk(Cin, kh * kw);
    a.CinK = conv_igemm_pick_cink(Cin, a.bk);
    a.K = kh * kw * a.CinK;
    a.Kpad = (a.K + a.bk - 1) / a.bk * a.bk;
    a.M = N * a.Ho * a.Wo;
    a.act1 = act1; a.act2 = act2; a.alpha1 = 0.1f; a.alpha2 = 0.1f;
    a.scalar_out = (Cout % 8 || ld_out % 8 || (has_res && ld_res % 8)) ? 1 : 0;
    return a;
}

static bool g_force_tactic = false;
static ConvTactic g_forced{};

extern "C" int32_t trtx_op_conv_force_tactic(const int32_t* t) {
    if (t && t[5] != 0) return TRTX_ERR_UNSUPPORTED;
    g_force_tactic = t != nullptr;
    if (t) g_forced = ConvTactic{t[0], t[1], t[2], t[3], t[4]};
    return TRTX_OK;
}

extern "C" int32_t trtx_op_conv2d_tactics(int N, int H, int W, int Cin, int ld_in, int Cout, int ld_out, int kh, int kw, int sh, int sw, int ph,
                                          int pw, int has_residual, int ld_res, int32_t* out6, int32_t max_out) {
    if (!out6 || max_out < 1 || N < 1 || kh < 1 || kw < 1 || sh < 1 || sw < 1) return 0;
    ConvArgs a = op_conv_args(N, H, W, Cin, ld_in, Cout, ld_out, kh, kw, sh, sw, ph, pw, 0, has_residual, ld_res, 0);
    a.residual = has_residual ? reinterpret_cast<const void*>(1) : nullptr;
    std::vector<ConvTactic> t(max_out);
    const int n = conv_tactics(a, t.data(), max_out);
    for (int i = 0; i < n; ++i) {
        out6[6 * i + 0] = t[i].bn; out6[6 * i + 1] = t[i].bk; out6[6 * i + 2] = t[i].bm; out6[6 * i + 3] = t[i].wsk; out6[6 * i + 4] = t[i].ws;
        out6[6 * i + 5] = 0;
    }
    return n;
}

extern "C" int32_t trtx_op_conv2d_nhwc_f16(const void* in, int N, int H, int W, int Cin, int ld_in, const void* wpacked,
                                           const float* bias, void* out, int Cout, int ld_out, int kh, int kw, int sh,
                                           int sw, int ph, int pw, int act1, const void* residual, int ld_res,
                                           int act2, trtx_stream_t stream) {
    ConvArgs a = op_conv_args(N, H, W, Cin, ld_in, Cout, ld_out, kh, kw, sh, sw, ph, pw, act1, residual != nullptr, ld_res, act2);
    a.in = in;
    a.wgt = wpacked;
    a.bias = bias;
    a.out = out;
    a.residual = residual;
    if (reinterpret_cast<uintptr_t>(out) & 15) a.scalar_out = 1;
    if (g_force_tactic) conv_apply_tactic(&a, g_forced);
    const int reps = options().op_reps;
    int32_t st = TRTX_OK;
    for (int r = 0; r < reps && st == TRTX_OK; ++r) st = conv_igemm_f16(a, stream);
    return st;
}

static ConvArgs op_stem_args(const float* in, int N, int C, int H, int W, const float* w_taps_cout, const float* bias, int Cout, int k, int stride, int pad, int act) {
    ConvArgs a{};
    a.in = in; a.wgt = w_taps_cout; a.bias = bias;
    a.N = N; a.H = H; a.W = W; a.Cin = C; a.ld_in = C;
    a.Ho = (H + 2 * pad - k) / stride + 1;
    a.Wo = (W + 2 * pad - k) / stride + 1;
    a.Cout = Cout; a.Cout_pad = Cout;
    a.kh = k; a.kw = k; a.stride_h = stride; a.stride_w = stride; a.pad_h = pad; a.pad_w = pad; a.dil_h = 1; a.dil_w = 1;
    a.groups = 1;
    a.K = k * k * C; a.Kpad = a.K;
    a.M = N * a.Ho * a.Wo;
    a.act1 = act; a.alpha1 = 0.1f; a.alpha2 = 0.1f;
    return a;
}

extern "C" int32_t trtx_op_conv_stem_nchw_f16(const float* in, int N, int C, int H, int W, const float* w_taps_cout, const float* bias, void* out, int Cout,
                                              int ld_out, int k, int stride, int pad, int act, trtx_stream_t stream) {
    if (!in || !w_taps_cout || !out || N < 1 || C < 1 || H < 1 || W < 1 || k < 1 || stride < 1 || pad < 0 || H + 2 * pad < k || W + 2 * pad < k) return TRTX_ERR_INVALID;
    ConvArgs a = op_stem_args(in, N, C, H, W, w_taps_cout, bias, Cout, k, stride, pad, act);
    a.out = out;
    a.ld_out = ld_out;
    return conv_stem_nchw_f32(a, static_cast<hipStream_t>(stream));
}

extern "C" int32_t trtx_op_conv_stem_pair_f16(const float* in, int N, int C, int H, int W, const float* stem_w_taps_cout, const float* stem_bias, int stem_act,
                                              const void* conv_wpacked, const float* conv_bias, int conv_act, void* out, int ld_out, trtx_stream_t stream) {
    if (!in || !stem_w_taps_cout || !conv_wpacked || !out || N < 1 || C < 1 || H < 1 || W < 1) return TRTX_ERR_INVALID;
    const ConvArgs s = op_stem_args(in, N, C, H, W, stem_w_taps_cout, stem_bias, 16, 3, 2, 1, stem_act);
    ConvArgs c = op_conv_args(N, s.Ho, s.Wo, 16, 16, 32, ld_out, 3, 3, 2, 2, 1, 1, conv_act, 0, 0, 0);
    c.wgt = conv_wpacked;
    c.bias = conv_bias;
    c.out = out;
    return conv_stem_pair_f16(s, c, static_cast<hipStream_t>(stream));
}

static int32_t op_bneck_pair(const void* in, int N, int H, int W, int ld_in, int in_coff, const void* w1_packed, const float* bias1, int act1, const void* w2_packed,
                             const float* bias2, int act2, int shortcut, int act_after, void* mid, void* out, int ld_out, bool or_two, trtx_stream_t stream) {
    if (!in || !w1_packed || !w2_packed || !out || N < 1 || H < 1 || W < 1 || ld_in < 16 || ld_in % 8 || in_coff < 0 || in_coff % 8 || in_coff + 16 > ld_in ||
        ld_out < 16 || ld_out % 8 || (or_two && !mid))
        return TRTX_ERR_INVALID;
    ConvArgs a = op_conv_args(N, H, W, 16, ld_in, 16, 16, 3, 3, 1, 1, 1, 1, act1, 0, 0, 0);
    ConvArgs b = op_conv_args(N, H, W, 16, 16, 16, ld_out, 3, 3, 1, 1, 1, 1, act2, shortcut ? 1 : 0, shortcut ? ld_in : 0, act_after);
    a.in = static_cast<const uint16_t*>(in) + in_coff;
    a.wgt = w1_packed;
    a.bias = bias1;
    a.out = mid;
    b.in = mid;
    b.wgt = w2_packed;
    b.bias = bias2;
    b.out = out;
    b.residual = shortcut ? a.in : nullptr;
    if (or_two) return conv_bneck_pair_or_two_f16(a, b, static_cast<hipStream_t>(stream));
    if (!conv_bneck_pair_possible(a, b)) return TRTX_ERR_INVALID;
    return conv_bneck_pair_f16(a, b, static_cast<hipStream_t>(stream));
}

extern "C" int32_t trtx_op_conv_bneck_pair_f16(const void* in, int N, int H, int W, int ld_in, int in_coff, const void* w1_packed, const float* bias1, int act1,
                                               const void* w2_packed, const float* bias2, int act2, int shortcut, int act_after, void* out, int ld_out,
                                               trtx_stream_t stream) {
    return op_bneck_pair(in, N, H, W, ld_in, in_coff, w1_packed, bias1, act1, w2_packed, bias2, act2, shortcut, act_after, nullptr, out, ld_out, false, stream);
}

extern "C" int32_t trtx_op_conv_bneck_pair_or_two_f16(const void* in, int N, int H, int W, int ld_in, int in_coff, const void* w1_packed, const float* bias1, int act1,
                                                      const void* w2_packed, const float* bias2, int act2, int shortcut, int act_after, void* mid, void* out,
                                                      int ld_out, trtx_stream_t stream) {
    return op_bneck_pair(in, N, H, W, ld_in, in_coff, w1_packed, bias1, act1, w2_packed, bias2, act2, shortcut, act_after, mid, out, ld_out, true, stream);
}

extern "C" int32_t trtx_conv_pack_weights_grouped_f16(const float* w_kcrs, int cout, int cin_g, int kh, int kw, const float* ch_scale, uint16_t* packed,
                                                      int32_t* kpad_out) {
    if (!w_kcrs || cout < 1 || cin_g < 1 || kh < 1 || kw < 1) return TRTX_ERR_INVALID;
    const int kpad = (kh * kw * cin_g + 31) / 32 * 32;
    if (kpad_out) *kpad_out = kpad;
    if (packed) pack_conv_weights_grouped_f16(w_kcrs, cout, cin_g, kh, kw, kpad, ch_scale, packed);
    return TRTX_OK;
}

extern "C" int32_t trtx_op_conv2d_grouped_nhwc_f16(const void* in, int N, int H, int W, int Cin, int ld_in, const void* wpacked, const float* bias, void* out,
                                                   int Cout, int ld_out, int groups, int k, int pad, int act1, const void* residual, int ld_res, int act2,
                                                   trtx_stream_t stream) {
    if (N < 1 || H < 1 || W < 1 || Cin < 1 || Cout < 1 || groups < 1 || k < 1 || pad < 0 || H + 2 * pad < k || W + 2 * pad < k) return TRTX_ERR_INVALID;
    ConvArgs a{};
    a.in = in; a.wgt = wpacked; a.bias = bias; a.out = out; a.residual = residual;
    a.N = N; a.H = H; a.W = W; a.Cin = Cin; a.ld_in = ld_in;
    a.Ho = H + 2 * pad - k + 1;
    a.Wo = W + 2 * pad - k + 1;
    a.Cout = Cout; a.Cout_pad = Cout; a.ld_out = ld_out; a.ld_res = ld_res;
    a.kh = k; a.kw = k; a.stride_h = 1; a.stride_w = 1; a.pad_h = pad; a.pad_w = pad; a.dil_h = 1; a.dil_w = 1;
    a.groups = groups;
    a.K = k * k * (Cin / groups);
    a.Kpad = conv_grouped_kpad(a);
    a.M = N * a.Ho * a.Wo;
    a.act1 = act1; a.act2 = act2; a.alpha1 = 0.1f; a.alpha2 = 0.1f;
    const int reps = options().op_reps;
    int32_t st = TRTX_OK;
    for (int r = 0; r < reps && st == TRTX_OK; ++r) st = conv_grouped(a, static_cast<hipStream_t>(stream));
    return st;
}

extern "C" int32_t trtx_op_conv2d_dw_nhwc(const void* in, int dtype, int N, int H, int W, int C, int ld_in, const float* w_taps_c, const float* bias, void* out,
                                          int ld_out, const void* residual, int ld_res, int k, int stride, int pad, int dilation, int act1, float alpha1,
                                          int act2, float alpha2, trtx_stream_t stream) {
    if (!in || !w_taps_c || !out || N < 1 || H < 1 || W < 1 || C < 1 || k < 1 || stride < 1 || pad < 0 || dilation < 1) return TRTX_ERR_INVALID;
    if (dtype != DT_F16 && dtype != DT_F32) return TRTX_ERR_UNSUPPORTED;
    if (H + 2 * pad < dilation * (k - 1) + 1 || W + 2 * pad < dilation * (k - 1) + 1) return TRTX_ERR_INVALID;
    ConvArgs a{};
    a.in = in; a.wgt = w_taps_c; a.bias = bias; a.out = out; a.residual = residual;
    a.N = N; a.H = H; a.W = W; a.Cin = C; a.ld_in = ld_in;
    a.Ho = (H + 2 * pad - dilation * (k - 1) - 1) / stride + 1;
    a.Wo = (W + 2 * pad - dilation * (k - 1) - 1) / stride + 1;
    a.Cout = C; a.Cout_pad = C; a.ld_out = ld_out; a.ld_res = ld_res;
    a.kh = k; a.kw = k; a.stride_h = stride; a.stride_w = stride; a.pad_h = pad; a.pad_w = pad; a.dil_h = dilation; a.dil_w = dilation;
    a.groups = C;
    a.K = k * k;
    a.Kpad = a.K;
    a.M = N * a.Ho * a.Wo;
    a.act1 = act1; a.act2 = act2; a.alpha1 = alpha1; a.alpha2 = alpha2;
    a.f32 = dtype == DT_F32;
    return conv_dw(a, dtype, static_cast<hipStream_t>(stream));
}

extern "C" int32_t trtx_op_psa_attention_f16(const void* qkv, int ld_qkv, void* out, int ld_out, void* vimg, int ld_v, int B, int heads, int N, int kd, int hd,
                                             float scale, trtx_stream_t stream) {
    if (!qkv || !out || !vimg) return TRTX_ERR_INVALID;
    return psa_attention_f16(qkv, ld_qkv, out, ld_out, vimg, ld_v, B, heads, N, kd, hd, scale, static_cast<hipStream_t>(stream));
}

extern "C" int32_t trtx_op_area_attention_f16(const void* qkv, int ld_qkv, void* out, int ld_out, void* vimg, int ld_v, int B, int heads, int N, int area,
                                              int kd, int hd, float scale, trtx_stream_t stream) {
    if (!qkv || !out || !vimg) return TRTX_ERR_INVALID;
    return area_attention_f16(qkv, ld_qkv, out, ld_out, vimg, ld_v, B, heads, N, area, kd, hd, scale, static_cast<hipStream_t>(stream));
}

extern "C" int32_t trtx_op_area_attention_split_f16(const void* q, int ld_q, const void* k, int ld_k, const void* v, int ld_v, void* out, int ld_out, int B,
                                                    int heads, int N, int area, int kd, int hd, float scale, trtx_stream_t stream) {
    if (!q || !k || !v || !out) return TRTX_ERR_INVALID;
    return area_attention_split_f16(q, ld_q, k, ld_k, v, ld_v, out, ld_out, B, heads, N, area, kd, hd, scale, static_cast<hipStream_t>(stream));
}

extern "C" size_t trtx_op_hgconv_workspace_bytes(int B, int N, int D, int E) { return hgconv_workspace_bytes(B, N, D, E); }

extern "C" int32_t trtx_op_hgconv_geometry(int32_t* tiles, int max_tiles, int32_t* n_tiles) {
    if (!tiles || !n_tiles || max_tiles < 1) return TRTX_ERR_INVALID;
    *n_tiles = hgconv_geometry(tiles, max_tiles);
    return TRTX_OK;
}

extern "C" int32_t trtx_op_hgconv_f16(const void* x, int ld_x, void* out, int ld_out, int B, int N, int D, int E, float logit_scale, const float* w_ctx,
                                      const float* b_ctx, const float* proto, const float* w_pre, const float* b_pre, const float* w_edge, const float* b_edge,
                                      const float* w_node, const float* b_node, void* workspace, size_t workspace_bytes, trtx_stream_t stream) {
    if (!x || !out || !w_ctx || !b_ctx || !proto || !w_pre || !b_pre || !w_edge || !b_edge || !w_node || !b_node || !workspace) return TRTX_ERR_INVALID;
    const HgconvWeights w{w_ctx, b_ctx, proto, w_pre, b_pre, w_edge, b_edge, w_node, b_node};
    return hgconv_f16(x, ld_x, out, ld_out, B, N, D, E, logit_scale, w, workspace, workspace_bytes, static_cast<hipStream_t>(stream));
}

static ConvArgs op_conv_args_f32(int N, int H, int W, int Cin, int ld_in, int Cout, int ld_out, int kh, int kw, int sh, int sw, int ph, int pw,
                                 int act1, int has_res, int ld_res, int act2) {
    ConvArgs a{};
    a.f32 = 1;
    a.N = N; a.H = H; a.W = W; a.Cin = Cin; a.ld_in = ld_in;
    a.Ho = (H + 2 * ph - kh) / sh + 1;
    a.Wo = (W + 2 * pw - kw) / sw + 1;
    a.Cout = Cout;
    a.Cout_pad = (Cout + 15) / 16 * 16;
    a.ld_out = ld_out; a.ld_res = ld_res;
    a.kh = kh; a.kw = kw; a.stride_h = sh; a.stride_w = sw; a.pad_h = ph; a.pad_w = pw; a.dil_h = 1; a.dil_w = 1;
    a.groups = 1;
    a.bk = 16;
    a.CinK = conv_igemm_f32_pick_cink(Cin);
    a.K = kh * kw * a.CinK;
    a.Kpad = (a.K + 15) / 16 * 16;
    a.M = N * a.Ho * a.Wo;
    a.act1 = act1; a.act2 = act2; a.alpha1 = 0.1f; a.alpha2 = 0.1f;
    a.scalar_out = (Cout % 4 || ld_out % 4 || (has_res && ld_res % 4)) ? 1 : 0;
    return a;
}

extern "C" int32_t trtx_conv_packed_dims_f32(int cout, int cin_pad, int kh, int kw, int32_t* cout_pad, int32_t* kpad, int32_t* cink) {
    if (cout < 1 || cin_pad < 1 || kh < 1 || kw < 1) return TRTX_ERR_INVALID;
    const int ck = conv_igemm_f32_pick_cink(cin_pad);
    if (cout_pad) *cout_pad = (cout + 15) / 16 * 16;
    if (kpad) *kpad = (kh * kw * ck + 15) / 16 * 16;
    if (cink) *cink = ck;
    return TRTX_OK;
}

extern "C" int32_t trtx_conv_pack_weights_f32(const float* w_kcrs, int cout, int cin, int kh, int kw, int cin_pad, const float* ch_scale, float* packed) {
    if (!w_kcrs || !packed || cin_pad < cin) return TRTX_ERR_INVALID;
    const int ck = conv_igemm_f32_pick_cink(cin_pad);
    conv_pack_weights_igemm_f32(w_kcrs, cout, cin, kh, kw, ck, (kh * kw * ck + 15) / 16 * 16, (cout + 15) / 16 * 16, ch_scale, packed);
    return TRTX_OK;
}

extern "C" int32_t trtx_op_conv2d_tactics_f32(int N, int H, int W, int Cin, int ld_in, int Cout, int ld_out, int kh, int kw, int sh, int sw, int ph,
                                              int pw, int has_residual, int ld_res, int32_t* out2, int32_t max_out) {
    if (!out2 || max_out < 1 || N < 1 || kh < 1 || kw < 1 || sh < 1 || sw < 1) return 0;
    ConvArgs a = op_conv_args_f32(N, H, W, Cin, ld_in, Cout, ld_out, kh, kw, sh, sw, ph, pw, 0, has_residual, ld_res, 0);
    a.residual = has_residual ? reinterpret_cast<const void*>(1) : nullptr;
    std::vector<ConvTactic> t(max_out);
    const int n = conv_tactics_f32(a, t.data(), max_out);
    for (int i = 0; i < n; ++i) {
        out2[4 * i + 0] = t[i].bn;
        out2[4 * i + 1] = t[i].bm;
        out2[4 * i + 2] = t[i].ws;
        out2[4 * i + 3] = t[i].bk;
    }
    return n;
}

extern "C" int32_t trtx_op_conv2d_nhwc_f32(const void* in, int N, int H, int W, int Cin, int ld_in, const void* wpacked, const float* bias, void* out,
                                           int Cout, int ld_out, int kh, int kw, int sh, int sw, int ph, int pw, int act1, const void* residual,
                                           int ld_res, int act2, const int32_t* tile2, trtx_stream_t stream) {
    ConvArgs a = op_conv_args_f32(N, H, W, Cin, ld_in, Cout, ld_out, kh, kw, sh, sw, ph, pw, act1, residual != nullptr, ld_res, act2);
    a.in = in;
    a.wgt = wpacked;
    a.bias = bias;
    a.out = out;
    a.residual = residual;
    if ((reinterpret_cast<uintptr_t>(out) & 15) || (residual && (reinterpret_cast<uintptr_t>(residual) & 15))) a.scalar_out = 1;
    if (tile2) {
        a.bn = tile2[0];
        a.bm = tile2[1];
        a.t_ws = tile2[2];
        a.bk = tile2[3];
    }
    const int reps = options().op_reps;
    int32_t st = TRTX_OK;
    for (int r = 0; r < reps && st == TRTX_OK; ++r) st = conv_igemm_f32(a, stream);
    return st;
}

extern "C" int32_t trtx_conv_pack_weights_i8(const float* w_kcrs, int cout, int cin, int kh, int kw, const float* ch_scale, int8_t* packed,
                                             float* wscale_out, int32_t* cout_pad_out, int32_t* kpad_out) {
    if (!w_kcrs || cout < 1 || cin < 1) return TRTX_ERR_INVALID;
    const int bn = conv_igemm_pick_bn(cout);
    const int cout_pad = (cout + bn - 1) / bn * bn, cink = (cin + 63) / 64 * 64, kpad = kh * kw * cink;
    if (cout_pad_out) *cout_pad_out = cout_pad;
    if (kpad_out) *kpad_out = kpad;
    if (packed && wscale_out) conv_pack_weights_i8(w_kcrs, cout, cin, kh, kw, cink, ch_scale, cout_pad, kpad, packed, wscale_out);
    return TRTX_OK;
}

extern "C" int32_t trtx_op_conv2d_nhwc_i8(const void* in, int N, int H, int W, int Cin, int ld_in, const void* wpacked, const float* cscale,
                                          const float* bias, void* out, int out_is_i8, float out_inv_scale, int Cout, int ld_out, int kh,
                                          int kw, int sh, int sw, int ph, int pw, int act1, const void* residual, int res_is_i8,
                                          float res_scale, int ld_res, int act2, trtx_stream_t stream) {
    if (Cin % 16 || ld_in % 16) return TRTX_ERR_INVALID;
    ConvArgs a{};
    a.in = in; a.wgt = wpacked; a.bias = bias; a.out = out; a.residual = residual;
    a.N = N; a.H = H; a.W = W;
    a.Ho = (H + 2 * ph - kh) / sh + 1;
    a.Wo = (W + 2 * pw - kw) / sw + 1;
    a.Cout = Cout;
    a.bn = conv_igemm_pick_bn(Cout);
    a.Cout_pad = (Cout + a.bn - 1) / a.bn * a.bn;
    a.ld_out = ld_out; a.ld_res = ld_res;
    a.kh = kh; a.kw = kw; a.stride_h = sh; a.stride_w = sw; a.pad_h = ph; a.pad_w = pw; a.dil_h = 1; a.dil_w = 1; a.groups = 1;
    a.bk = 32;
    const int cink = (Cin + 63) / 64 * 64;
    a.in_i8 = 1; a.out_i8 = out_is_i8; a.res_i8 = res_is_i8;
    a.cscale = cscale; a.out_inv_scale = out_inv_scale; a.res_scale = res_scale;
    a.Cin = Cin / 2; a.ld_in = ld_in / 2; a.CinK = cink / 2;
    a.K = kh * kw * a.CinK;
    a.Kpad = a.K;
    a.M = N * a.Ho * a.Wo;
    a.act1 = act1; a.act2 = act2; a.alpha1 = 0.1f; a.alpha2 = 0.1f;
    a.scalar_out = 0;
    if (Cout % 8 || ld_out % 8 || (residual && ld_res % 8)) return TRTX_ERR_UNSUPPORTED;
    return conv_igemm_f16(a, stream);
}

extern "C" int32_t trtx_op_nchw_f32_to_nhwc_f16(const float* in, void* out, int N, int C, int H, int W, int Cpad,
                                                int ld_out, trtx_stream_t stream) {
    return nchw_f32_to_nhwc(in, out, DT_F16, N, C, H, W, Cpad, ld_out, stream);
}

extern "C" int32_t trtx_op_nhwc_f16_to_nchw_f32(const void* in, float* out, int N, int C, int H, int W, int ld_in,
                                                trtx_stream_t stream) {
    return nhwc_to_nchw_f32(in, DT_F16, out, N, C, H, W, ld_in, stream);
}

extern "C" int32_t trtx_op_poison_lds(void* device_word, trtx_stream_t stream) {
    if (!device_word) return TRTX_ERR_INVALID;
    return poison_lds(static_cast<unsigned*>(device_word), static_cast<hipStream_t>(stream));
}


extern "C" int32_t trtx_reorg_fold_weights(const float* w_kcrs, int cout, int cin, int kh, int kw, float* folded) {
    if (!w_kcrs || !folded || cout < 1 || cin < 1 || kh < 1 || kw < 1) return TRTX_ERR_INVALID;
    reorg_fold_weights(w_kcrs, cout, cin, kh, kw, folded);
    return TRTX_OK;
}
```

tensorrtx_amd/csrc/options.cpp:

```cpp
#include "options.h"

#include <stdlib.h>

namespace trtx {
namespace {
const char* env(const char* name) { return getenv(name); }
int env_int(const char* name, int unset) {
    const char* v = env(name);
    return (v && *v) ? atoi(v) : unset;
}
bool env_is(const char* name, int value) {
    const char* v = env(name);
    return v && *v && atoi(v) == value;
}
bool env_set(const char* name) { return env(name) != nullptr; }
}

Options read_options() {
    Options o;
    o.tune = env_int("TRTX_TUNE", -1);
    o.tune_verbose = env_set("TRTX_TUNE_VERBOSE");
    o.tune_margin = env_int("TRTX_TUNE_MARGIN", -1);
    if (const char* v = env("TRTX_TACTIC_CACHE")) o.tactic_cache = v;
    o.graph = env_is("TRTX_GRAPH", 1);
    if (const char* v = env("TRTX_CALIB_REPORT")) o.calib_report = v;
    if (const char* v = env("TRTX_INT8_CLIP_LIMIT"); v && *v) o.int8_clip_limit = atof(v);
    o.lanes = env_int("TRTX_LANES", 0);
    o.group_convs = !env_is("TRTX_GROUP_CONVS", 0);
    o.fold_upsample = !env_is("TRTX_FOLD_UPSAMPLE", 0);
    o.stem_pair = !env_is("TRTX_STEM_PAIR", 0);
    o.bneck_pair = !env_is("TRTX_BNECK_PAIR", 0);
    o.ws = !env_set("TRTX_CONV_NOWS");
    o.wsk = !env_set("TRTX_CONV_NOWSK");
    o.gemm256 = !env_is("TRTX_GEMM256", 0);
    o.patch = !env_is("TRTX_CONV_PATCH", 0);
    o.res = env_int("TRTX_CONV_RES", 7);
    o.roles = !env_is("TRTX_CONV_ROLES", 0);
    o.f32_mfma = !env_set("TRTX_F32_DIRECT");
    o.conv_grouped = !env_is("TRTX_CONV_GROUPED", 0);
    o.area_attention = !env_is("TRTX_AREA_ATTENTION", 0);
    o.aattn_split = !env_is("TRTX_AATTN_SPLIT", 0);
    o.hgconv = !env_is("TRTX_HGCONV", 0);
    o.gated_add = !env_is("TRTX_GATED_ADD", 0);
    o.yolo5_head = !env_is("TRTX_YOLO5_HEAD", 0);
    o.yolo7_head = !env_is("TRTX_YOLO7_HEAD", 0);
    o.reorg_fold = !env_is("TRTX_REORG_FOLD", 0);
    o.spp_parallel_chain = !env_is("TRTX_SPP_PARALLEL_CHAIN", 0);
    o.yolo9_head = !env_is("TRTX_YOLO9_HEAD", 0);
    o.roialign_fused = !env_set("TRTX_ROIALIGN_PLUGIN");
    o.roialign_fold_stride = !env_is("TRTX_ROIALIGN_FOLD_STRIDE", 0);
    o.profile_kernel_events = !env_set("TRTX_PROFILE_NO_KERNEL_EVENTS");
    o.op_reps = env_int("TRTX_OP_REPS", 1);
    return o;
}

const Options& options() {
    static const Options o = read_options();
    return o;
}

}
```

tensorrtx_amd/csrc/options.h:

```cpp
#pragma once
#include <string>

namespace trtx {

struct Options {
    int tune = -1;
    bool tune_verbose = false;
    int tune_margin = -1;
    std::string tactic_cache;
    bool graph = false;
    std::string calib_report;
    double int8_clip_limit = 1e-4;
    int lanes = 0;
    bool group_convs = true;
    bool fold_upsample = true;
    bool stem_pair = true;
    bool bneck_pair = true;
    bool ws = true;
    bool wsk = true;
    bool gemm256 = true;
    bool patch = true;
    int res = 7;
    bool roles = true;
    bool f32_mfma = true;
    bool conv_grouped = true;
    bool area_attention = true;
    bool aattn_split = true;
    bool hgconv = true;
    bool gated_add = true;
    bool yolo9_head = true;
    bool yolo5_head = true;
    bool yolo7_head = true;
    bool reorg_fold = true;
    bool spp_parallel_chain = true;
    bool roialign_fused = true;
    bool roialign_fold_stride = true;
    bool profile_kernel_events = true;
    int op_reps = 1;
};

Options read_options();
const Options& options();

}
```

tensorrtx_amd/csrc/runtime/engine.cpp:

```cpp
#include "engine.h"

#include <stdlib.h>
#include <string.h>

#include <sstream>

#include "../common.h"
#include "../options.h"
#include "int8.h"
#include "plugin.h"

using namespace trtx;

trtx_engine::~trtx_engine() {
    int left = plugins_initialized;
    for (auto& op : plan.ops)
        if (op.kind == OP_PLUGIN && left-- > 0 && op.plugin->v.terminate) op.plugin->v.terminate(op.plugin->v.self);
    if (d_weights) (void)hipFree(d_weights);
}

trtx_context::~trtx_context() {
    for (hipStream_t st : lane_stream)
        if (st) {
            (void)hipStreamSynchronize(st);
            (void)hipStreamDestroy(st);
        }
    for (hipEvent_t ev : op_event)
        if (ev) (void)hipEventDestroy(ev);
    for (hipEvent_t ev : lane_done)
        if (ev) (void)hipEventDestroy(ev);
    if (start_event) (void)hipEventDestroy(start_event);
    for (auto& g : graphs) {
        if (g.exec) (void)hipGraphExecDestroy(g.exec);
        if (g.graph) (void)hipGraphDestroy(g.graph);
    }
    if (d_arena) (void)hipFree(d_arena);
}

namespace trtx {

namespace {

struct Resolver {
    const Plan& plan;
    char* arena;
    char* weights;
    void* const* bindings;
    char* base(const PTensor& t) const {
        const Storage& s = plan.storages[t.storage];
        switch (s.kind) {
            case ST_ARENA: return arena + s.offset;
            case ST_WEIGHTS: return weights + s.offset;
            default: return static_cast<char*>(bindings[s.binding]);
        }
    }
    void* ptr(int tid) const {
        const PTensor& t = plan.tensors[tid];
        const size_t es = dtype_size(t.dtype);
        return base(t) + (t.layout == LAY_NHWC ? (size_t)t.rcoff : (size_t)t.reoff) * es;
    }
};

StridedView batch_view(const StridedView& v, int batch, long bs_in, long bs_in2) {
    StridedView o{};
    o.rank = v.rank + 1;
    o.shape[0] = batch;
    o.stride_in[0] = bs_in;
    o.stride_in2[0] = bs_in2;
    for (int d = 0; d < v.rank; ++d) {
        o.shape[d + 1] = v.shape[d];
        o.stride_in[d + 1] = v.stride_in[d];
        o.stride_in2[d + 1] = v.stride_in2[d];
    }
    return o;
}

}

int32_t execute_plan(trtx_context* c, int batch, void* const* bindings, hipStream_t stream,
                     std::vector<OpTiming>* prof) {
    trtx_engine* e = c->engine;
    const Plan& plan = e->plan;
    if (batch < 1 || batch > plan.max_batch) {
        fprintf(stderr, "[trtx_hip] enqueue: batch %d outside [1, %d]\n", batch, plan.max_batch);
        return TRTX_ERR_INVALID;
    }
    for (size_t b = 0; b < plan.binding_tensor.size(); ++b)
        if (!bindings[b] && !(c->frames && plan.binding_is_input[b])) {
            fprintf(stderr, "[trtx_hip] enqueue: binding %zu is null\n", b);
            return TRTX_ERR_INVALID;
        }
    Resolver R{plan, static_cast<char*>(c->d_arena), static_cast<char*>(e->d_weights), bindings};
    char* W = static_cast<char*>(e->d_weights);
    std::vector<hipEvent_t> evs;
    std::vector<LaunchProbe> probes;
    const bool no_probe = !options().profile_kernel_events;
    if (prof) {
        evs.resize(plan.ops.size() + 1);
        for (auto& ev : evs) TRTX_HIP_TRY(hipEventCreate(&ev));
        probes.resize(plan.ops.size());
        if (!no_probe && !c->tuning)
            for (size_t k = 0; k < plan.ops.size(); ++k)
                if ((plan.ops[k].kind == OP_CONV && plan.ops[k].igemm) || plan.ops[k].kind == OP_CONV_GROUP)
                    if (hipEventCreate(&probes[k].start) != hipSuccess || hipEventCreate(&probes[k].stop) != hipSuccess) (void)hipGetLastError();
        TRTX_HIP_TRY(hipEventRecord(evs[0], stream));
    }
    auto free_probes = [&]() {
        conv_set_launch_probe(nullptr);
        for (auto& pr : probes) {
            if (pr.start) (void)hipEventDestroy(pr.start);
            if (pr.stop) (void)hipEventDestroy(pr.stop);
        }
        probes.clear();
    };
    hipStream_t const user_stream = stream;
    const bool lanes = !prof && !c->observer && plan.num_lanes > 1;
    std::vector<char> lane_started(plan.num_lanes, 0);
    auto bail = [&](int32_t st) {
        (void)hipGetLastError();
        if (lanes)
            for (int l = 1; l < plan.num_lanes; ++l)
                if (lane_started[l] && hipEventRecord(c->lane_done[l], c->lane_stream[l]) == hipSuccess)
                    (void)hipStreamWaitEvent(user_stream, c->lane_done[l], 0);
        for (auto& ev : evs) (void)hipEventDestroy(ev);
        evs.clear();
        free_probes();
        return st;
    };
    if (lanes && hipEventRecord(c->start_event, user_stream) != hipSuccess) return bail(TRTX_ERR_HIP);
    ConvArgs pair_stem{};
    bool pair_pending = false;
    auto defers_to_next = [&](size_t k) {
        if (c->observer || c->tuning || k + 1 >= plan.ops.size()) return false;
        const POp &o = plan.ops[k], &nx = plan.ops[k + 1];
        return nx.bneck_pair && nx.kind == OP_CONV && o.kind == OP_CONV && o.igemm && nx.lane == o.lane && nx.in[0] == o.out[0];
    };
    for (size_t k = 0; k < plan.ops.size(); ++k) {
        const POp& op = plan.ops[k];
        hipStream_t stream = user_stream;
        if (lanes) {
            if (op.lane > 0) {
                stream = c->lane_stream[op.lane];
                if (!lane_started[op.lane]) {
                    if (hipStreamWaitEvent(stream, c->start_event, 0) != hipSuccess) return bail(TRTX_ERR_HIP);
                    lane_started[op.lane] = 1;
                }
            }
            for (int d : op.wait_ops)
                if (hipStreamWaitEvent(stream, c->op_event[d], 0) != hipSuccess) return bail(TRTX_ERR_HIP);
        }
        const PTensor& t0 = plan.tensors[op.in.empty() ? op.out[0] : op.in[0]];
        const PTensor& to = plan.tensors[op.out[0]];
        auto nb = [&](const PTensor& t) { return (t.nfix ? t.nfix : batch) * t.nmul; };
        int32_t st = TRTX_OK;
        const bool skip = c->tuning && (op.kind == OP_PLUGIN || op.kind == OP_YOLO_HEAD || op.kind == OP_YOLO_TASK_HEAD || op.kind == OP_YOLO5_HEAD || op.kind == OP_YOLO9_HEAD || op.kind == OP_YOLO7_HEAD || op.kind == OP_ROI_ALIGN);
        if (!skip) switch (op.kind) {
            case OP_CONV:
            case OP_DECONV: {
                ConvArgs a = op.conv;
                a.in = R.ptr(op.in[0]);
                a.out = R.ptr(op.out[0]);
                a.residual = op.in.size() > 1 ? R.ptr(op.in[1]) : nullptr;
                a.up_in = op.extra_in.empty() ? nullptr : R.ptr(op.extra_in[0]);
                a.wgt = W + op.w_off;
                a.bias = reinterpret_cast<const float*>(W + op.b_off);
                a.cscale = a.in_i8 ? reinterpret_cast<const float*>(W + op.s_off) : nullptr;
                a.N = op.stem ? (plan.explicit_batch ? (int)t0.dims.d[0] : batch) : nb(t0);
                a.M = a.N * a.Ho * a.Wo;
                if (op.stem && !c->frames && !c->observer && !c->tuning && k + 1 < plan.ops.size() && plan.ops[k + 1].stem_pair && plan.ops[k + 1].lane == op.lane) {
                    const POp& nx = plan.ops[k + 1];
                    ConvArgs b = nx.conv;
                    b.out = R.ptr(nx.out[0]);
                    b.wgt = W + nx.w_off;
                    b.bias = reinterpret_cast<const float*>(W + nx.b_off);
                    b.N = nb(to);
                    b.M = b.N * b.Ho * b.Wo;
                    if (conv_stem_pair_possible(a, b)) {
                        pair_stem = a;
                        pair_pending = true;
                        break;
                    }
                }
                if (op.stem_pair && pair_pending) {
                    pair_pending = false;
                    if (prof && probes[k].start && probes[k].stop) conv_set_launch_probe(&probes[k]);
                    st = conv_stem_pair_f16(pair_stem, a, stream);
                    conv_set_launch_probe(nullptr);
                    break;
                }
                if (defers_to_next(k)) break;
                if (op.bneck_pair && k > 0 && defers_to_next(k - 1)) {
                    const POp& fo = plan.ops[k - 1];
                    ConvArgs f = fo.conv;
                    f.in = R.ptr(fo.in[0]);
                    f.out = R.ptr(fo.out[0]);
                    f.wgt = W + fo.w_off;
                    f.bias = reinterpret_cast<const float*>(W + fo.b_off);
                    f.N = nb(plan.tensors[fo.in[0]]);
                    f.M = f.N * f.Ho * f.Wo;
                    if (prof && probes[k].start && probes[k].stop) conv_set_launch_probe(&probes[k]);
                    st = conv_bneck_pair_or_two_f16(f, a, stream);
                    conv_set_launch_probe(nullptr);
                    break;
                }
                if (op.kind == OP_DECONV)
                    st = deconv_direct(a, op.dtype, stream);
                else if (op.stem && c->frames)
                    st = a.f32 ? TRTX_ERR_UNSUPPORTED : conv_stem_frames_f32(a, c->frames, stream);
                else if (op.stem)
                    st = a.f32 ? conv_stem_nchw_f32_out_f32(a, stream) : conv_stem_nchw_f32(a, stream);
                else if (op.igemm) {
                    if (prof && probes[k].start && probes[k].stop) conv_set_launch_probe(&probes[k]);
                    st = a.f32 ? conv_igemm_f32(a, stream) : conv_igemm_f16(a, stream);
                    conv_set_launch_probe(nullptr);
                } else if (op.dw)
                    st = conv_dw(a, op.dtype, stream);
                else if (op.grouped)
                    st = conv_grouped(a, stream);
                else
                    st = conv_direct(a, op.dtype, stream);
                break;
            }
            case OP_CONV_GROUP: {
                ConvArgs ga[kMaxConvGroup];
                const int gn = (int)op.group.size();
                if (gn < 2 || gn > kMaxConvGroup) { st = TRTX_ERR_STATE; break; }
                for (int m = 0; m < gn; ++m) {
                    const POp& mo = op.group[m];
                    ConvArgs& a = ga[m];
                    a = mo.conv;
                    a.in = R.ptr(mo.in[0]);
                    a.out = R.ptr(mo.out[0]);
                    a.residual = mo.in.size() > 1 ? R.ptr(mo.in[1]) : nullptr;
                    a.up_in = nullptr;
                    a.wgt = W + mo.w_off;
                    a.bias = reinterpret_cast<const float*>(W + mo.b_off);
                    a.cscale = a.in_i8 ? reinterpret_cast<const float*>(W + mo.s_off) : nullptr;
                    a.N = nb(plan.tensors[mo.in[0]]);
                    a.M = a.N * a.Ho * a.Wo;
                }
                if (prof && probes[k].start && probes[k].stop) conv_set_launch_probe(&probes[k]);
                st = conv_igemm_group_f16(ga, gn, stream);
                conv_set_launch_probe(nullptr);
                if (st == TRTX_ERR_UNSUPPORTED) {
                    st = TRTX_OK;
                    for (int m = 0; m < gn && st == TRTX_OK; ++m) st = conv_igemm_f16(ga[m], stream);
                }
                break;
            }
            case OP_POOL:
                st = nhwc_pool(R.ptr(op.in[0]), R.ptr(op.out[0]), op.dtype, op.i[0], nb(t0), t0.H, t0.W, t0.C, t0.ld, to.H,
                               to.W, to.ld, op.i[1], op.i[2], op.i[3], op.i[4], op.i[5], op.i[6], op.i[7], stream);
                break;
            case OP_POOL_CHAIN: {
                const PTensor &y1 = plan.tensors[op.out[0]], &y2 = plan.tensors[op.out[1]], &y3 = plan.tensors[op.out[2]];
                st = nhwc_maxpool_chain3_f16(R.ptr(op.in[0]), R.ptr(op.out[0]), R.ptr(op.out[1]), R.ptr(op.out[2]), nb(t0), t0.H,
                                             t0.W, t0.C, t0.ld, y1.ld, y2.ld, y3.ld, op.i[1], stream, op.dtype == DT_F32 ? 1 : 0);
                break;
            }
            case OP_D2S:
                st = nhwc_depth_to_space_f16(R.ptr(op.in[0]), R.ptr(op.out[0]), nb(t0), t0.H, t0.W, to.C, op.i[0], op.i[1], t0.ld,
                                             to.ld, stream);
                break;
            case OP_RESIZE:
                if (t0.dtype == DT_I8) {
                    st = nhwc_resize_nearest_i8(R.ptr(op.in[0]), R.ptr(op.out[0]), nb(t0), t0.H, t0.W, t0.C, t0.ld, to.H, to.W, to.ld,
                                                t0.scale / to.scale, stream);
                    break;
                }
                st = nhwc_resize_nearest(R.ptr(op.in[0]), R.ptr(op.out[0]), op.dtype, nb(t0), t0.H, t0.W, t0.C, t0.ld, to.H,
                                         to.W, to.ld, stream);
                break;
            case OP_EW_NHWC: {
                const PTensor& t1 = plan.tensors[op.in[1]];
                st = nhwc_elementwise(R.ptr(op.in[0]), R.ptr(op.in[1]), R.ptr(op.out[0]), op.dtype, op.i[0],
                                      (long)nb(t0) * t0.H * t0.W, t0.C, t0.ld, t1.ld, to.ld, stream);
                break;
            }
            case OP_GATED_ADD: {
                const PTensor& t1 = plan.tensors[op.in[1]];
                st = nhwc_gated_add(R.ptr(op.in[0]), R.ptr(op.in[1]), reinterpret_cast<const float*>(W + op.w_off), R.ptr(op.out[0]), op.dtype,
                                    (long)nb(t0) * t0.H * t0.W, t0.C, t0.ld, t1.ld, to.ld, stream);
                break;
            }
            case OP_ACT_NHWC:
                st = nhwc_activation(R.ptr(op.in[0]), R.ptr(op.out[0]), op.dtype, op.i[0], op.f[0],
                                     (long)nb(t0) * t0.H * t0.W, t0.C, t0.ld, to.ld, stream);
                break;
            case OP_SCALE_NHWC:
                st = nhwc_scale(R.ptr(op.in[0]), R.ptr(op.out[0]), op.dtype, reinterpret_cast<const float*>(W + op.s_off),
                                reinterpret_cast<const float*>(W + op.b_off), (long)nb(t0) * t0.H * t0.W, t0.C, t0.ld,
                                to.ld, stream);
                break;
            case OP_COPY_NHWC:
                st = nhwc_copy(R.ptr(op.in[0]), R.ptr(op.out[0]), op.dtype, (long)nb(t0) * t0.H * t0.W, t0.C, t0.ld, to.ld,
                               stream);
                break;
            case OP_REDUCE_HW:
                st = nhwc_reduce_hw_avg(R.ptr(op.in[0]), R.ptr(op.out[0]), op.dtype, nb(t0), t0.H * t0.W, t0.C, t0.ld, to.ld,
                                        stream);
                break;
            case OP_TO_NHWC:
                st = nchw_f32_to_nhwc(static_cast<const float*>(R.ptr(op.in[0])), R.ptr(op.out[0]), to.dtype, nb(to), to.C,
                                      to.H, to.W, to.Calloc ? to.Calloc : to.C, to.ld, stream);
                break;
            case OP_TO_LINEAR:
                st = nhwc_to_nchw_f32(R.ptr(op.in[0]), t0.dtype, static_cast<float*>(R.ptr(op.out[0])), nb(t0), t0.C, t0.H,
                                      t0.W, t0.ld, stream);
                break;
            case OP_GATHER: {
                const float* src = static_cast<const float*>(R.ptr(op.in[0])) + op.off0;
                const StridedView v = to.batched ? batch_view(op.view, batch, t0.batched ? t0.dims.volume() : 0, 0) : op.view;
                st = lin_gather(src, static_cast<float*>(R.ptr(op.out[0])), v, stream);
                break;
            }
            case OP_SCATTER: {
                float* dst = static_cast<float*>(R.ptr(op.out[0])) + op.off0;
                StridedView v = op.view;
                if (to.batched) {
                    if (!t0.batched) {
                        for (int b = 0; b < batch && st == TRTX_OK; ++b)
                            st = lin_scatter(static_cast<const float*>(R.ptr(op.in[0])), dst + (long)b * to.dims.volume(), v,
                                             stream);
                        break;
                    }
                    v = batch_view(op.view, batch, to.dims.volume(), 0);
                }
                st = lin_scatter(static_cast<const float*>(R.ptr(op.in[0])), dst, v, stream);
                break;
            }
            case OP_EW_LIN: {
                const PTensor& t1 = plan.tensors[op.in[1]];
                const StridedView v = to.batched ? batch_view(op.view, batch, t0.batched ? t0.dims.volume() : 0,
                                                              t1.batched ? t1.dims.volume() : 0)
                                                 : op.view;
                st = lin_elementwise(static_cast<const float*>(R.ptr(op.in[0])), static_cast<const float*>(R.ptr(op.in[1])),
                                     static_cast<float*>(R.ptr(op.out[0])), op.i[0], v, stream);
                break;
            }
            case OP_ACT_LIN:
                st = lin_activation(static_cast<const float*>(R.ptr(op.in[0])), static_cast<float*>(R.ptr(op.out[0])), op.i[0],
                                    op.f[0], (long)(to.batched ? batch : 1) * to.dims.volume(), stream);
                break;
            case OP_SCALE_LIN: {
                const long bmul = to.batched ? batch : 1;
                st = lin_scale(static_cast<const float*>(R.ptr(op.in[0])), static_cast<float*>(R.ptr(op.out[0])),
                               reinterpret_cast<const float*>(W + op.s_off), reinterpret_cast<const float*>(W + op.b_off),
                               reinterpret_cast<const float*>(W + op.w_off), op.i[0], bmul * op.i[1], op.i[2], op.i[3],
                               stream);
                break;
            }
            case OP_SOFTMAX:
                st = lin_softmax(static_cast<const float*>(R.ptr(op.in[0])), static_cast<float*>(R.ptr(op.out[0])),
                                 (long)(to.batched ? batch : 1) * op.i[0], op.i[1], op.i[2], stream);
                break;
            case OP_MATMUL: {
                const PTensor& t1 = plan.tensors[op.in[1]];
                if (op.view.rank > 0) {
                    const StridedView& v = op.view;
                    const long outer = v.rank == 2 ? v.shape[0] : 1, inner = v.shape[v.rank - 1];
                    st = lin_matmul(static_cast<const float*>(R.ptr(op.in[0])), static_cast<const float*>(R.ptr(op.in[1])),
                                    static_cast<float*>(R.ptr(op.out[0])), (int)(outer * inner), op.i[0], op.i[1], op.i[2], op.i[3], op.i[4],
                                    v.rank == 2 ? v.stride_in[0] : 0, v.rank == 2 ? v.stride_in2[0] : 0, stream, (int)inner,
                                    v.stride_in[v.rank - 1], v.stride_in2[v.rank - 1]);
                    break;
                }
                st = lin_matmul(static_cast<const float*>(R.ptr(op.in[0])), static_cast<const float*>(R.ptr(op.in[1])),
                                static_cast<float*>(R.ptr(op.out[0])), to.batched ? batch : 1, op.i[0], op.i[1], op.i[2],
                                op.i[3], op.i[4], t0.batched ? t0.dims.volume() : 0, t1.batched ? t1.dims.volume() : 0,
                                stream);
                break;
            }
            case OP_REDUCE_LIN:
                st = lin_reduce(static_cast<const float*>(R.ptr(op.in[0])), static_cast<float*>(R.ptr(op.out[0])), op.i[0],
                                (long)(to.batched ? batch : 1) * op.i[1], op.i[2], op.i[3], stream);
                break;
            case OP_PLUGIN: {
                std::vector<const void*> ins;
                std::vector<void*> outs;
                for (int t : op.in) ins.push_back(R.ptr(t));
                for (int t : op.out) outs.push_back(R.ptr(t));
                void* ws = op.ws_bytes ? static_cast<char*>(c->d_arena) + op.ws_off : nullptr;
                const int pb = plan.explicit_batch && op.i[0] > 0 ? op.i[0] : batch;
                const int rc = op.plugin->v.enqueue(op.plugin->v.self, pb, ins.data(), outs.data(), ws, stream);
                if (rc != 0) {
                    fprintf(stderr, "[trtx_hip] plugin %s enqueue returned %d\n", op.name.c_str(), rc);
                    st = TRTX_ERR_HIP;
                }
                break;
            }
            case OP_YOLO_HEAD: {
                const int nl = op.i[4];
                const void* heads[8];
                int lds[8];
                for (int k = 0; k < nl; ++k) {
                    heads[k] = R.ptr(op.in[k]);
                    lds[k] = plan.tensors[op.in[k]].ld;
                }
                st = (t0.dtype == DT_F32 ? trtx_yolo_head_decode_nhwc_f32 : trtx_yolo_head_decode_nhwc)(
                        heads, lds, nl, op.i[11] > 0 ? op.i[11] : batch, op.i[0], op.i[1], op.i[2], &op.i[5], reinterpret_cast<const float*>(W + op.w_off), op.i[3],
                        static_cast<float*>(R.ptr(op.out[0])), static_cast<char*>(c->d_arena) + op.ws_off, op.ws_bytes, stream);
                break;
            }
            case OP_YOLO_TASK_HEAD: {
                const int nl = op.i[4];
                const void* heads[4];
                const void* branches[4];
                int lds[4], blds[4];
                for (int k = 0; k < nl; ++k) {
                    heads[k] = R.ptr(op.in[k]);
                    lds[k] = plan.tensors[op.in[k]].ld;
                    branches[k] = R.ptr(op.extra_in[k]);
                    blds[k] = plan.tensors[op.extra_in[k]].ld;
                }
                st = (t0.dtype == DT_F32 ? trtx_yolo_task_head_decode_nhwc_f32 : trtx_yolo_task_head_decode_nhwc)(
                        heads, lds, branches, blds, nl, op.i[11] > 0 ? op.i[11] : batch, op.i[0], op.i[1], op.i[2], &op.i[5],
                        reinterpret_cast<const float*>(W + op.w_off), op.i[3], op.i[9] == 1, op.i[9] == 2, op.i[9] == 3, op.i[10], op.f[0],
                        static_cast<float*>(R.ptr(op.out[0])), static_cast<char*>(c->d_arena) + op.ws_off, op.ws_bytes, stream);
                break;
            }
            case OP_YOLO5_HEAD:
            case OP_YOLO7_HEAD: {
                const int nl = op.i[4];
                const void* heads[8];
                int lds[8], gw[8], gh[8];
                if (nl < 1 || nl > 8 || (int)op.iv.size() != 2 * nl || (int)op.fv.size() != 6 * nl) { st = TRTX_ERR_STATE; break; }
                for (int k = 0; k < nl; ++k) {
                    heads[k] = R.ptr(op.in[k]);
                    lds[k] = plan.tensors[op.in[k]].ld;
                    gw[k] = op.iv[2 * k];
                    gh[k] = op.iv[2 * k + 1];
                }
                const bool f32 = t0.dtype == DT_F32;
                const auto decode = op.kind == OP_YOLO7_HEAD ? (f32 ? trtx_yolov7_head_decode_nhwc_f32 : trtx_yolov7_head_decode_nhwc)
                                                             : (f32 ? trtx_yolov5_head_decode_nhwc_f32 : trtx_yolov5_head_decode_nhwc);
                st = decode(
                        heads, lds, nl, op.i[11] > 0 ? op.i[11] : batch, op.i[0], op.i[1], op.i[2], gw, gh, op.fv.data(), op.i[3],
                        static_cast<float*>(R.ptr(op.out[0])), static_cast<char*>(c->d_arena) + op.ws_off, op.ws_bytes, stream);
                break;
            }
            case OP_YOLO9_HEAD: {
                const void* box[3];
                const void* cls[3];
                int box_ld[3], cls_ld[3];
                if (op.i[4] != 3 || op.in.size() != 3 || op.extra_in.size() != 3) { st = TRTX_ERR_STATE; break; }
                for (int k = 0; k < 3; ++k) {
                    box[k] = R.ptr(op.in[k]);
                    box_ld[k] = plan.tensors[op.in[k]].ld;
                    cls[k] = R.ptr(op.extra_in[k]);
                    cls_ld[k] = plan.tensors[op.extra_in[k]].ld;
                }
                st = (t0.dtype == DT_F32 ? trtx_yolov9_head_decode_nhwc_f32 : trtx_yolov9_head_decode_nhwc)(
                        box, box_ld, cls, cls_ld, batch, op.i[0], op.i[1], op.i[2], reinterpret_cast<const float*>(W + op.w_off), op.i[3],
                        static_cast<float*>(R.ptr(op.out[0])), static_cast<char*>(c->d_arena) + op.ws_off, op.ws_bytes, stream);
                break;
            }
            case OP_ATTENTION: {
                const PTensor &to2 = plan.tensors[op.out[1]];
                if (op.i[4] > 0)
                    st = area_attention_f16(R.ptr(op.in[0]), t0.ld, R.ptr(op.out[0]), to.ld, R.ptr(op.out[1]), to2.ld, nb(t0), op.i[0], op.i[1], op.i[4],
                                            op.i[2], op.i[3], op.f[0], stream);
                else
                    st = psa_attention_f16(R.ptr(op.in[0]), t0.ld, R.ptr(op.out[0]), to.ld, R.ptr(op.out[1]), to2.ld, nb(t0), op.i[0], op.i[1], op.i[2],
                                           op.i[3], op.f[0], stream);
                break;
            }
            case OP_ATTENTION_SPLIT: {
                const PTensor& tv = plan.tensors[op.in[1]];
                const char* qk = static_cast<const char*>(R.ptr(op.in[0]));
                st = area_attention_split_f16(qk, t0.ld, qk + (size_t)op.i[5] * dtype_size(t0.dtype), t0.ld, R.ptr(op.in[1]), tv.ld, R.ptr(op.out[0]), to.ld,
                                              nb(t0), op.i[0], op.i[1], op.i[4], op.i[2], op.i[3], op.f[0], stream);
                break;
            }
            case OP_HGCONV: {
                const size_t D = (size_t)op.i[1], ED = (size_t)op.i[2] * D;
                const float* p = reinterpret_cast<const float*>(W + op.w_off);
                HgconvWeights w{};
                w.w_ctx = p;  p += ED * 2 * D;
                w.b_ctx = p;  p += ED;
                w.proto = p;  p += ED;
                w.w_pre = p;  p += D * D;
                w.b_pre = p;  p += D;
                w.w_edge = p; p += D * D;
                w.b_edge = p; p += D;
                w.w_node = p; p += D * D;
                w.b_node = p;
                st = hgconv_f16(R.ptr(op.in[0]), t0.ld, R.ptr(op.out[0]), to.ld, nb(t0), op.i[0], op.i[1], op.i[2], op.f[0], w,
                                static_cast<char*>(c->d_arena) + op.ws_off, op.ws_bytes, stream);
                break;
            }
            case OP_ROI_ALIGN: {
                const PTensor& ft = plan.tensors[op.in[1]];
// ... 382 lines not shown
```

tensorrtx_amd/csrc/runtime/plan.cpp:

```cpp
#include "plan.h"

#include <sstream>

namespace trtx {

const char* op_kind_name(int k) {
    static const char* n[] = {"conv",     "deconv",    "pool",      "resize",     "ew_nhwc", "act_nhwc", "scale_nhwc",
                              "copy_nhwc", "reduce_hw", "to_nhwc",   "to_linear",  "gather",  "scatter",  "ew_lin",
                              "act_lin",  "scale_lin", "softmax",   "matmul",     "reduce_lin", "plugin", "copy_lin", "yolo_head",
                              "pool_chain", "depth_to_space", "roi_align", "conv_chain", "conv_group", "attention",
                              "yolo_task_head", "yolo5_head", "yolo9_head", "yolo7_head", "hgconv", "gated_add", "attention_split"};
    return (k >= 0 && k <= OP_ATTENTION_SPLIT) ? n[k] : "?";
}

std::string Plan::describe_json() const {
    std::ostringstream o;
    double flops = 0, bytes = 0;
    int n_conv = 0, n_igemm = 0;
    for (const auto& op : ops) {
        flops += op.flops;
        bytes += op.bytes;
        if (op.kind == OP_CONV) {
            ++n_conv;
            n_igemm += op.igemm ? 1 : 0;
        }
        n_conv += (int)op.group.size();
        n_igemm += (int)op.group.size();
    }
    o << "{\"fp16\":" << (fp16 ? "true" : "false") << ",\"max_batch\":" << max_batch << ",\"arena_bytes\":" << arena_bytes
      << ",\"weight_bytes\":" << weight_bytes << ",\"n_lanes\":" << num_lanes << ",\"n_ops\":" << ops.size() << ",\"n_conv\":" << n_conv
      << ",\"n_igemm\":" << n_igemm << ",\"flops_per_sample\":" << flops << ",\"bytes_per_sample\":" << bytes
      << ",\"ops\":[";
    for (size_t k = 0; k < ops.size(); ++k) {
        const POp& op = ops[k];
        o << (k ? "," : "") << "{\"kind\":\"" << op_kind_name(op.kind) << "\",\"name\":\"";
        for (char c : op.name) o << ((c == '"' || c == '\\' || (unsigned char)c < 0x20) ? ' ' : c);
        o << "\",\"flops\":" << op.flops << ",\"bytes\":" << op.bytes;
        auto conv_fields = [&](const POp& op) {
            const ConvArgs& a = op.conv;
            o << ",\"igemm\":" << (op.igemm ? "true" : "false") << ",\"stem\":" << (op.stem ? "true" : "false") << (op.stem_pair ? ",\"stem_pair\":true" : "")
              << (op.bneck_pair ? ",\"bneck_pair\":true" : "") << ",\"cin\":" << (a.in_i8 ? 2 * a.Cin : a.Cin) << ",\"cout\":" << a.Cout
              << ",\"k\":[" << a.kh << "," << a.kw << "],\"stride\":[" << a.stride_h << "," << a.stride_w << "],\"hw_in\":["
              << a.H << "," << a.W << "],\"hw_out\":[" << a.Ho << "," << a.Wo << "],\"act1\":" << a.act1
              << ",\"act2\":" << a.act2 << ",\"alpha1\":" << a.alpha1 << ",\"alpha2\":" << a.alpha2 << ",\"up_c\":" << a.up_C << ",\"residual\":" << (op.in.size() > 1 ? "true" : "false")
              << ",\"bn_folded\":" << (op.scale_layer >= 0 ? "true" : "false") << ",\"ld_in\":" << a.ld_in
              << ",\"ld_out\":" << a.ld_out << ",\"i8\":[" << a.in_i8 << "," << a.out_i8 << "," << a.res_i8 << "],\"nmul\":" << (op.stem ? 1 : tensors[op.in[0]].nmul) << ",\"nfix\":"
              << (op.stem ? 0 : tensors[op.in[0]].nfix);
            if (op.dw) o << ",\"dw\":true";
            if (op.grouped) o << ",\"grouped\":true";
            if (op.cout_real) o << ",\"cout_real\":" << op.cout_real;
            if (op.reorg_cin) o << ",\"reorg_cin\":" << op.reorg_cin;
        };
        if (op.kind == OP_CONV || op.kind == OP_DECONV) conv_fields(op);
        if (op.kind == OP_ACT_NHWC || op.kind == OP_ACT_LIN) o << ",\"act\":" << op.i[0];
        if (op.kind == OP_ATTENTION) o << ",\"heads\":" << op.i[0] << ",\"n\":" << op.i[1] << ",\"kd\":" << op.i[2] << ",\"hd\":" << op.i[3];
        if (op.kind == OP_ATTENTION && op.i[4] > 0) o << ",\"area\":" << op.i[4] << ",\"kernel\":\"mfma\"";
        if (op.kind == OP_ATTENTION_SPLIT)
            o << ",\"heads\":" << op.i[0] << ",\"n\":" << op.i[1] << ",\"kd\":" << op.i[2] << ",\"hd\":" << op.i[3] << ",\"area\":" << op.i[4] << ",\"k_offset\":" << op.i[5];
        if (op.kind == OP_HGCONV)
            o << ",\"n\":" << op.i[0] << ",\"d\":" << op.i[1] << ",\"e\":" << op.i[2] << ",\"logit_scale\":" << op.f[0] << ",\"ld\":[" << tensors[op.in[0]].ld << ","
              << tensors[op.out[0]].ld << "],\"ws_bytes\":" << op.ws_bytes;
        if (op.kind == OP_YOLO_TASK_HEAD) {
            o << ",\"task\":\"" << (op.i[9] == 1 ? "seg" : (op.i[9] == 2 ? "pose" : "obb")) << "\",\"classes\":" << op.i[0] << ",\"nk\":" << op.i[10]
              << ",\"branch_ld\":[";
            for (size_t j = 0; j < op.extra_in.size(); ++j) o << (j ? "," : "") << tensors[op.extra_in[j]].ld;
            o << "]";
        }
        if (op.kind == OP_POOL || op.kind == OP_POOL_CHAIN)
            o << ",\"k\":[" << op.i[1] << "," << op.i[2] << "],\"stride\":[" << op.i[3] << "," << op.i[4] << "],\"outputs\":" << op.out.size();
        if (op.kind == OP_YOLO5_HEAD || op.kind == OP_YOLO7_HEAD) {
            o << ",\"classes\":" << op.i[0] << ",\"levels\":" << op.i[4] << ",\"anchor_levels\":" << op.fv.size() / 6 << ",\"grids\":[";
            for (int j = 0; j < op.i[4]; ++j) o << (j ? "," : "") << "[" << op.iv[2 * j] << "," << op.iv[2 * j + 1] << "]";
            o << "],\"ld\":[";
            for (size_t j = 0; j < op.in.size(); ++j) o << (j ? "," : "") << tensors[op.in[j]].ld;
            o << "]";
        }
        if (op.kind == OP_YOLO9_HEAD) {
            o << ",\"classes\":" << op.i[0] << ",\"levels\":" << op.i[4] << ",\"grids\":[";
            for (int j = 0; j < op.i[4]; ++j) o << (j ? "," : "") << "[" << op.i[2] / (8 << j) << "," << op.i[1] / (8 << j) << "]";
            o << "],\"strides\":[";
            for (int j = 0; j < op.i[4]; ++j) o << (j ? "," : "") << (8 << j);
            o << "],\"box_ld\":[";
            for (size_t j = 0; j < op.in.size(); ++j) o << (j ? "," : "") << tensors[op.in[j]].ld;
            o << "],\"cls_ld\":[";
            for (size_t j = 0; j < op.extra_in.size(); ++j) o << (j ? "," : "") << tensors[op.extra_in[j]].ld;
            o << "]";
        }
        if (op.kind == OP_CONV_GROUP) {
            o << ",\"members\":[";
            for (size_t j = 0; j < op.group.size(); ++j) {
                const POp& m = op.group[j];
                o << (j ? "," : "") << "{\"name\":\"";
                for (char c : m.name) o << ((c == '"' || c == '\\' || (unsigned char)c < 0x20) ? ' ' : c);
                o << "\",\"flops\":" << m.flops << ",\"bytes\":" << m.bytes;
                conv_fields(m);
                o << ",\"in\":[";
                for (size_t q = 0; q < m.in.size(); ++q) o << (q ? "," : "") << m.in[q];
                o << "],\"out\":[" << m.out[0] << "]}";
            }
            o << "]";
        }
        o << ",\"lane\":" << op.lane << ",\"waits\":[";
        for (size_t j = 0; j < op.wait_ops.size(); ++j) o << (j ? "," : "") << op.wait_ops[j];
        o << "],\"in\":[";
        for (size_t j = 0; j < op.in.size(); ++j) o << (j ? "," : "") << op.in[j];
        o << "],\"out\":[";
        for (size_t j = 0; j < op.out.size(); ++j) o << (j ? "," : "") << op.out[j];
        o << "]}";
    }
    o << "],\"tensors\":[";
    for (size_t k = 0; k < tensors.size(); ++k) {
        const PTensor& t = tensors[k];
        o << (k ? "," : "") << "{\"id\":" << t.id << ",\"net\":" << t.net_tensor << ",\"layout\":\""
          << (t.layout == LAY_NHWC ? "nhwc" : "linear") << "\",\"dims\":[";
        for (int d = 0; d < t.dims.nb; ++d) o << (d ? "," : "") << t.dims.d[d];
        o << "],\"storage\":" << t.storage << ",\"coff\":" << t.rcoff << ",\"ld\":" << t.ld << ",\"dtype\":" << t.dtype << ",\"scale\":" << t.scale
          << ",\"view\":"
          << (t.parent >= 0 ? "true" : "false") << "}";
    }
    o << "],\"storages\":[";
    for (size_t k = 0; k < storages.size(); ++k) {
        const Storage& s = storages[k];
        o << (k ? "," : "") << "{\"kind\":" << s.kind << ",\"bytes\":" << s.bytes << ",\"offset\":" << s.offset
          << ",\"first\":" << s.first_use << ",\"last\":" << s.last_use << "}";
    }
    o << "]}";
    return o.str();
}

}
```

tensorrtx_amd/csrc/runtime/plan.h:

```cpp
#pragma once
#include <memory>
#include <string>
#include <vector>

#include "../kernels/kernels.h"
#include "graph.h"
#include "plugin.h"

namespace trtx {

enum Layout : int { LAY_LINEAR = 0, LAY_NHWC = 1 };
enum StorageKind : int { ST_ARENA = 0, ST_WEIGHTS = 1, ST_BINDING = 2 };

enum OpKind : int {
    OP_CONV = 0,
    OP_DECONV,
    OP_POOL,
    OP_RESIZE,
    OP_EW_NHWC,
    OP_ACT_NHWC,
    OP_SCALE_NHWC,
    OP_COPY_NHWC,
    OP_REDUCE_HW,
    OP_TO_NHWC,
    OP_TO_LINEAR,
    OP_GATHER,
    OP_SCATTER,
    OP_EW_LIN,
    OP_ACT_LIN,
    OP_SCALE_LIN,
    OP_SOFTMAX,
    OP_MATMUL,
    OP_REDUCE_LIN,
    OP_PLUGIN,
    OP_COPY_LIN,
    OP_YOLO_HEAD,
    OP_POOL_CHAIN,
    OP_D2S,
    OP_ROI_ALIGN,
    OP_RESERVED_47,
    OP_CONV_GROUP,
    OP_ATTENTION,
    OP_YOLO_TASK_HEAD,
    OP_YOLO5_HEAD,
    OP_YOLO9_HEAD,
    OP_YOLO7_HEAD,
    OP_HGCONV,
    OP_GATED_ADD,
    OP_ATTENTION_SPLIT,
};
const char* op_kind_name(int k);

struct PTensor {
    int id = -1;
    int net_tensor = -1;
    std::string name;
    Dims dims;
    bool batched = true;
    int layout = LAY_LINEAR;
    int dtype = DT_F32;
    int nfix = 0;
    int nmul = 1;
    int C = 0, H = 0, W = 0;
    bool pad_zeroed = false;
    int parent = -1;
    int coff = 0;
    long eoff = 0;
    int ld = 0;
    int storage = -1;
    int rcoff = 0;
    long reoff = 0;
    int Calloc = 0;
    float scale = 0.f;
    long sample_elems() const { return layout == LAY_NHWC ? (long)nmul * H * W * ld : (long)dims.volume(); }
};

struct Storage {
    int kind = ST_ARENA;
    size_t bytes = 0;
    size_t offset = 0;
    int binding = -1;
    int first_use = 1 << 30, last_use = -1;
};
inline size_t align256(size_t v) { return (v + 255) / 256 * 256; }

struct POp {
    int kind = 0;
    std::string name;
    std::vector<int> in, out;
    std::vector<int> extra_in;
    int dtype = DT_F32;
    ConvArgs conv{};
    bool igemm = false;
    bool stem = false;
    bool stem_pair = false;
    bool bneck_pair = false;
    bool from_deconv = false;
    bool dw = false;
    bool grouped = false;
    int reorg_cin = 0;
    int cout_real = 0;
    std::vector<POp> group;
    int src_layer = -1;
    int scale_layer = -1;
    size_t w_off = 0, b_off = 0, s_off = 0;
    int i[12] = {0};
    float f[4] = {0};
    std::vector<int> iv;
    std::vector<float> fv;
    StridedView view{};
    long off0 = 0;
    bool view_batched_in = false, view_batched_in2 = false, view_batched_out = true;
    std::shared_ptr<PluginHolder> plugin;
    size_t ws_off = 0, ws_bytes = 0;
    int lane = 0;
    std::vector<int> wait_ops;
    bool signal = false;
    double flops = 0;
    double bytes = 0;
};

struct Plan {
    bool explicit_batch = false;
    bool fp16 = false;
    int max_batch = 1;
    std::vector<PTensor> tensors;
    std::vector<Storage> storages;
    std::vector<POp> ops;
    std::vector<int> binding_tensor;
    std::vector<int> binding_ptensor;
    std::vector<bool> binding_is_input;
    int num_lanes = 1;
    size_t arena_bytes = 0;
    size_t weight_bytes = 0;
    std::vector<uint8_t> weight_blob;
    std::string error;

    std::string describe_json() const;
};

bool lower_network(const Network& net, Plan* plan);
struct CalibrationLowering {
    CalibrationLowering();
    ~CalibrationLowering();
    static bool active();
};
bool pack_weights(const Network& net, Plan* plan);

}
```

tensorrtx_amd/csrc/runtime/plan_passes.cpp:

```cpp
#include "plan_passes.h"

#include <algorithm>

namespace trtx {
namespace {

bool fail(std::string* err, const std::string& m) {
    *err = m;
    return false;
}

size_t tensor_bytes(const Plan& plan, const PTensor& t) {
    const size_t es = dtype_size(t.dtype);
    if (t.layout == LAY_NHWC) {
        const size_t n = (t.nfix ? (size_t)t.nfix : (size_t)plan.max_batch) * (size_t)t.nmul;
        return n * t.H * t.W * (size_t)t.Calloc * es;
    }
    return (t.batched ? (size_t)plan.max_batch : 1) * (size_t)t.dims.volume() * es;
}

bool choose_conv_kernel(const Plan& plan, const PassInputs& e, POp& op) {
    ConvArgs& a = op.conv;
    const PTensor& ti = plan.tensors[op.in[0]];
    const PTensor& to = plan.tensors[op.out[0]];
// ... 390 lines not shown
            }
        }
        if (!ok) continue;
        const int y1 = plan.ops[by[0]].out[0], y2 = plan.ops[by[1]].out[0], y3 = plan.ops[by[2]].out[0];
        POp& a = plan.ops[k];
        a.kind = OP_POOL_CHAIN;
        a.name += " [x3 parallel, chained]";
        a.i[1] = a.i[2] = k1;
        a.i[5] = a.i[6] = k1 / 2;
        a.out = {y1, y2, y3};
        plan.ops.erase(plan.ops.begin() + idx[2]);
        plan.ops.erase(plan.ops.begin() + idx[1]);
    }
}

std::vector<std::vector<int>> op_dependencies(const Plan& plan) {
    const int nops = (int)plan.ops.size();
    struct Range { int storage; long lo, hi; int op; bool write; };
    auto access_of = [&](int t, int op, bool write) {
        const PTensor& pt = plan.tensors[t];
        Range a{pt.storage, 0, 0, op, write};
        if (pt.layout == LAY_NHWC) {
            a.lo = pt.rcoff;
            a.hi = pt.rcoff + (pt.parent < 0 && pt.Calloc > pt.C ? pt.Calloc : pt.C);
        } else {
            a.lo = pt.reoff;
            a.hi = pt.reoff + pt.dims.volume();
        }
        return a;
    };
    std::vector<std::vector<int>> deps(nops);
    std::vector<Range> log;
    for (int k = 0; k < nops; ++k) {
        const POp& op = plan.ops[k];
        std::vector<Range> mine;
        for (int t : op.in) mine.push_back(access_of(t, k, false));
        for (int t : op.extra_in) mine.push_back(access_of(t, k, false));
        for (int t : op.out) mine.push_back(access_of(t, k, true));
        for (const Range& m : mine)
            for (const Range& o : log)
                if (o.storage == m.storage && o.lo < m.hi && m.lo < o.hi && (o.write || m.write) && o.op != k) deps[k].push_back(o.op);
        std::sort(deps[k].begin(), deps[k].end());
        deps[k].erase(std::unique(deps[k].begin(), deps[k].end()), deps[k].end());
        log.insert(log.end(), mine.begin(), mine.end());
    }
    return deps;
}

struct Ancestors {
    int words;
    std::vector<uint64_t> bits;
    bool has(int a, int of) const { return (bits[(size_t)of * words + (a >> 6)] >> (a & 63)) & 1ull; }
};
Ancestors ancestors(const Plan& plan, const std::vector<std::vector<int>>& deps, bool lane_order) {
    const int n = (int)deps.size();
    Ancestors anc{(n + 63) / 64, {}};
    anc.bits.assign((size_t)n * anc.words, 0);
    std::vector<int> prev_on_lane(plan.num_lanes, -1);
    for (int k = 0; k < n; ++k) {
        uint64_t* row = &anc.bits[(size_t)k * anc.words];
        auto absorb = [&](int d) {
            for (int w = 0; w < anc.words; ++w) row[w] |= anc.bits[(size_t)d * anc.words + w];
            row[d >> 6] |= 1ull << (d & 63);
        };
        for (int d : deps[k]) absorb(d);
        if (!lane_order) continue;
        const int lane = plan.ops[k].lane;
        if (prev_on_lane[lane] >= 0) absorb(prev_on_lane[lane]);
        prev_on_lane[lane] = k;
    }
    return anc;
}

void group_convs(Plan& plan, const PassInputs& e) {
    if (e.dt != DT_F16 || CalibrationLowering::active()) return;
    const bool mark_only = !e.opt.group_convs;
    const int n = (int)plan.ops.size();
    if (n < 2 || n > 4096) return;
    const std::vector<std::vector<int>> deps = op_dependencies(plan);
    const Ancestors anc = ancestors(plan, deps, false);
    auto args_at_max_batch = [&](const POp& op) {
        ConvArgs a = op.conv;
        const PTensor& ti = plan.tensors[op.in[0]];
        a.N = (ti.nfix ? ti.nfix : plan.max_batch) * ti.nmul;
        a.M = a.N * a.Ho * a.Wo;
        a.residual = op.in.size() > 1 ? reinterpret_cast<const void*>(1) : nullptr;
        return a;
    };
    auto candidate = [&](const POp& op) {
        if (op.kind != OP_CONV || !op.igemm || op.stem || op.from_deconv || !op.extra_in.empty()) return false;
        ConvArgs two[2] = {args_at_max_batch(op), args_at_max_batch(op)};
        return conv_igemm_group_supported(two, 2);
    };
    auto same_layer_shape = [&](const POp& x, const POp& y) {
        const ConvArgs &a = x.conv, &b = y.conv;
        return a.kh == b.kh && a.kw == b.kw && a.stride_h == b.stride_h && a.stride_w == b.stride_w && a.pad_h == b.pad_h && a.pad_w == b.pad_w &&
               a.Cout == b.Cout && a.act1 == b.act1 && a.act2 == b.act2 && a.alpha1 == b.alpha1 && a.alpha2 == b.alpha2 && x.in.size() == y.in.size() &&
               a.in_i8 == b.in_i8 && a.out_i8 == b.out_i8 && a.res_i8 == b.res_i8;
    };
    std::vector<int> height(n, 0);
    for (int k = n - 1; k >= 0; --k)
        for (int d : deps[k]) height[d] = std::max(height[d], height[k] + 1);
    std::vector<int> group_of(n, -1);
    std::vector<std::vector<int>> groups;
    struct Contracted { std::vector<int> first_op, indeg; std::vector<std::vector<int>> succ; };
    auto contract = [&]() {
        Contracted c;
        std::vector<int> node(n), gnode(groups.size(), -1);
        for (int k = 0; k < n; ++k) {
            if (group_of[k] >= 0 && gnode[group_of[k]] >= 0) {
                node[k] = gnode[group_of[k]];
                continue;
            }
            if (group_of[k] >= 0) gnode[group_of[k]] = (int)c.first_op.size();
            node[k] = (int)c.first_op.size();
            c.first_op.push_back(k);
        }
        c.succ.resize(c.first_op.size());
        c.indeg.assign(c.first_op.size(), 0);
        for (int k = 0; k < n; ++k)
            for (int d : deps[k])
                if (node[d] != node[k]) {
                    c.succ[node[d]].push_back(node[k]);
                    ++c.indeg[node[k]];
                }
        return c;
    };
    auto acyclic = [&]() {
        Contracted c = contract();
        const int nn = (int)c.first_op.size();
        std::vector<int>& indeg = c.indeg;
        const std::vector<std::vector<int>>& succ = c.succ;
        std::vector<int> q;
        for (int v = 0; v < nn; ++v)
            if (!indeg[v]) q.push_back(v);
        size_t done = 0;
        while (done < q.size()) {
            const int v = q[done++];
            for (int w : succ[v])
                if (--indeg[w] == 0) q.push_back(w);
        }
        return (int)q.size() == nn;
    };
    for (int k = 0; k < n; ++k) {
        if (group_of[k] >= 0 || !candidate(plan.ops[k])) continue;
        std::vector<int> mem = {k};
        std::vector<ConvArgs> margs = {args_at_max_batch(plan.ops[k])};
        for (int j = k + 1; j < n && (int)mem.size() < kMaxConvGroup; ++j) {
            if (group_of[j] >= 0 || height[j] != height[k] || !candidate(plan.ops[j]) || !same_layer_shape(plan.ops[k], plan.ops[j])) continue;
            bool indep = true;
            for (int m : mem) indep = indep && !anc.has(m, j) && !anc.has(j, m);
            if (!indep) continue;
            margs.push_back(args_at_max_batch(plan.ops[j]));
            std::vector<ConvArgs> trial = margs;
            int big = 0;
            for (size_t q = 1; q < trial.size(); ++q)
                if (trial[q].M > trial[big].M) big = (int)q;
            const int rs = trial[big].t_rs;
            for (ConvArgs& ma : trial) ma.t_rs = rs;
            if (!conv_igemm_group_supported(trial.data(), (int)trial.size())) {
                margs.pop_back();
                continue;
            }
            mem.push_back(j);
        }
        if (mem.size() < 2) continue;
        const int gi = (int)groups.size();
        groups.push_back(mem);
        for (int m : mem) group_of[m] = gi;
        if (!acyclic()) {
            for (int m : mem) group_of[m] = -1;
            groups.pop_back();
        }
    }
    if (groups.empty()) return;
    if (mark_only) {
        for (const auto& mem : groups)
            for (int m : mem) {
                plan.ops[m].conv.t_wsk = WSK_OFF;
                plan.ops[m].conv.k_pinned = 1;
            }
        return;
    }
    Contracted c = contract();
    const int nn = (int)c.first_op.size();
    std::vector<int>&indeg = c.indeg, &first_op = c.first_op;
    const std::vector<std::vector<int>>& succ = c.succ;
    std::vector<char> emitted(nn, 0);
    std::vector<POp> out;
    out.reserve(nn);
    for (int step = 0; step < nn; ++step) {
        int pick = -1;
        for (int v = 0; v < nn; ++v)
            if (!emitted[v] && indeg[v] == 0) { pick = v; break; }
        if (pick < 0) return;
        emitted[pick] = 1;
        for (int w : succ[pick]) --indeg[w];
        const int k0 = first_op[pick];
        if (group_of[k0] < 0) {
            out.push_back(plan.ops[k0]);
            continue;
        }
        POp g;
        g.kind = OP_CONV_GROUP;
        g.dtype = plan.ops[k0].dtype;
        g.conv = plan.ops[k0].conv;
        int big = groups[group_of[k0]][0];
        for (int m : groups[group_of[k0]])
            if ((long)plan.ops[m].conv.Ho * plan.ops[m].conv.Wo * plan.tensors[plan.ops[m].in[0]].nmul >
                (long)plan.ops[big].conv.Ho * plan.ops[big].conv.Wo * plan.tensors[plan.ops[big].in[0]].nmul)
                big = m;
        for (int m : groups[group_of[k0]]) {
            POp mo = plan.ops[m];
            mo.conv.t_rs = plan.ops[big].conv.t_rs;
            mo.conv.t_wsk = WSK_OFF;
            mo.conv.k_pinned = 1;
            g.group.push_back(mo);
            g.name += (g.name.empty() ? "" : " + ") + mo.name;
            for (int t : mo.in)
                if (std::find(g.in.begin(), g.in.end(), t) == g.in.end()) g.in.push_back(t);
            g.out.push_back(mo.out[0]);
            g.flops += mo.flops;
            g.bytes += mo.bytes;
        }
        g.name = "[group of " + std::to_string(g.group.size()) + "] " + g.name;
        out.push_back(std::move(g));
    }
    plan.ops = std::move(out);
}

void mark_stem_pair(Plan& plan, const PassInputs& e) {
    if (!e.opt.stem_pair || e.dt != DT_F16 || e.int8 || CalibrationLowering::active()) return;
    const int n = (int)plan.ops.size();
    for (int k = 0; k + 1 < n; ++k) {
        const POp& st = plan.ops[k];
        POp& cv = plan.ops[k + 1];
        if (st.kind != OP_CONV || !st.stem || st.conv.f32 || st.out.size() != 1) continue;
        if (cv.kind != OP_CONV || !cv.igemm || cv.stem || cv.from_deconv || cv.in.size() != 1 || !cv.extra_in.empty() || cv.in[0] != st.out[0]) continue;
        const PTensor& mid = plan.tensors[st.out[0]];
        if (mid.storage < 0 || plan.storages[mid.storage].kind != ST_ARENA || is_binding_tensor(plan, mid.id) || is_binding_tensor(plan, owner_of(plan, mid.id))) continue;
        bool shared = false;
        auto touches = [&](const POp& op) {
            for (const std::vector<int>* v : {&op.in, &op.out, &op.extra_in})
                for (int t : *v)
                    if (plan.tensors[t].storage == mid.storage) return true;
            return false;
        };
        for (int j = 0; j < n && !shared; ++j) {
            if (j == k || j == k + 1) continue;
            shared = touches(plan.ops[j]);
            for (const POp& m : plan.ops[j].group) shared = shared || touches(m);
        }
        if (shared) continue;
        ConvArgs a = st.conv, b = cv.conv;
        const PTensor& t_in = plan.tensors[st.in[0]];
        a.N = plan.explicit_batch ? (int)t_in.dims.d[0] : plan.max_batch;
        a.M = a.N * a.Ho * a.Wo;
        b.N = (mid.nfix ? mid.nfix : plan.max_batch) * mid.nmul;
        b.M = b.N * b.Ho * b.Wo;
        if (!conv_stem_pair_possible(a, b)) continue;
        cv.stem_pair = true;
    }
}

void mark_bneck_pair(Plan& plan, const PassInputs& e) {
    if (!e.opt.bneck_pair || e.dt != DT_F16 || e.int8 || CalibrationLowering::active()) return;
    const int n = (int)plan.ops.size();
    auto plain = [](const POp& op) { return op.kind == OP_CONV && op.igemm && !op.stem && !op.stem_pair && !op.bneck_pair && !op.from_deconv && op.extra_in.empty() && op.out.size() == 1; };
    for (int k = 0; k + 1 < n; ++k) {
        const POp& c0 = plan.ops[k];
        POp& c1 = plan.ops[k + 1];
        if (!plain(c0) || !plain(c1) || c0.in.size() != 1 || c1.in.empty() || c1.in.size() > 2 || c1.in[0] != c0.out[0]) continue;
        if (c1.in.size() == 2 && c1.in[1] != c0.in[0]) continue;
        const PTensor& mid = plan.tensors[c0.out[0]];
        if (mid.parent >= 0 || mid.storage < 0 || plan.storages[mid.storage].kind != ST_ARENA || is_binding_tensor(plan, mid.id)) continue;
        bool shared = false;
        auto touches = [&](const POp& op) {
            for (const std::vector<int>* v : {&op.in, &op.out, &op.extra_in})
                for (int t : *v)
                    if (plan.tensors[t].storage == mid.storage) return true;
            return false;
        };
        for (int j = 0; j < n && !shared; ++j) {
            if (j == k || j == k + 1) continue;
            shared = touches(plan.ops[j]);
            for (const POp& m : plan.ops[j].group) shared = shared || touches(m);
        }
        const PTensor &t_in = plan.tensors[c0.in[0]], &t_out = plan.tensors[c1.out[0]];
        if (shared || t_in.storage == mid.storage || t_out.storage == mid.storage) continue;
        if (t_in.layout != LAY_NHWC || t_out.layout != LAY_NHWC) continue;
        if (t_in.storage == t_out.storage && t_in.rcoff < t_out.rcoff + std::max(t_out.C, 1) && t_out.rcoff < t_in.rcoff + std::max(t_in.C, 1)) continue;
        ConvArgs a = c0.conv, b = c1.conv;
        a.N = (t_in.nfix ? t_in.nfix : plan.max_batch) * t_in.nmul;
        a.M = a.N * a.Ho * a.Wo;
        b.N = (mid.nfix ? mid.nfix : plan.max_batch) * mid.nmul;
        b.M = b.N * b.Ho * b.Wo;
        b.residual = c1.in.size() > 1 ? reinterpret_cast<const void*>(1) : nullptr;
        if (!conv_bneck_pair_possible(a, b)) continue;
        c1.bneck_pair = true;
        ++k;
    }
}

void assign_lanes(Plan& plan, const PassInputs& e, const std::vector<std::vector<int>>& deps) {
    const int nops = (int)plan.ops.size();
    int max_lanes = e.max_aux_streams >= 0 ? 1 + e.max_aux_streams : 4;
    if (e.opt.lanes > 0) max_lanes = std::max(1, std::min(16, e.opt.lanes));
    std::vector<int> tail(max_lanes, -1);
    plan.num_lanes = 1;
    for (int k = 0; k < nops; ++k) {
        int lane = -1;
        for (int d : deps[k])
            if (tail[plan.ops[d].lane] == d && (lane < 0 || d > tail[lane])) lane = plan.ops[d].lane;
        if (lane < 0 && deps[k].empty()) lane = 0;
        if (lane < 0) {
            for (int l = 0; l < max_lanes && lane < 0; ++l)
                if (tail[l] < 0) lane = l;
        }
        if (lane < 0) {
            lane = 0;
            for (int l = 1; l < max_lanes; ++l)
                if (tail[l] < tail[lane]) lane = l;
        }
        plan.ops[k].lane = lane;
        tail[lane] = k;
        plan.num_lanes = std::max(plan.num_lanes, lane + 1);
    }
    std::vector<std::vector<int>> covered(max_lanes, std::vector<int>(max_lanes, -1));
    for (int k = 0; k < nops; ++k) {
        POp& op = plan.ops[k];
        for (int d : deps[k]) {
            const int ld = plan.ops[d].lane;
            if (ld == op.lane || covered[op.lane][ld] >= d) continue;
            op.wait_ops.push_back(d);
            plan.ops[d].signal = true;
            covered[op.lane][ld] = d;
        }
    }
}

void plan_arena(Plan& plan, const Ancestors& anc) {
    const int nops = (int)plan.ops.size();
    auto before = [&](int a, int b) { return a == b || anc.has(a, b); };
    std::vector<std::vector<int>> touch(plan.storages.size());
    for (int k = 0; k < nops; ++k) {
        const POp& op = plan.ops[k];
        auto mark = [&](int t) {
            const int st = plan.tensors[t].storage;
            Storage& s = plan.storages[st];
            s.first_use = std::min(s.first_use, k);
            s.last_use = std::max(s.last_use, k);
            if (touch[st].empty() || touch[st].back() != k) touch[st].push_back(k);
        };
        for (int t : op.in) mark(t);
        for (int t : op.extra_in) mark(t);
        for (int t : op.out) mark(t);
        if (op.bneck_pair && k > 0)
            for (int t : plan.ops[k - 1].in) mark(t);
    }
    std::vector<std::pair<int, int>> ws_storage;
    for (int k = 0; k < nops; ++k) {
        const int kind = plan.ops[k].kind;
        if ((kind != OP_PLUGIN && kind != OP_YOLO_HEAD && kind != OP_YOLO_TASK_HEAD && kind != OP_YOLO5_HEAD && kind != OP_YOLO9_HEAD && kind != OP_YOLO7_HEAD && kind != OP_HGCONV) || plan.ops[k].ws_bytes == 0) continue;
        Storage s;
        s.kind = ST_ARENA;
        s.bytes = plan.ops[k].ws_bytes;
        s.first_use = s.last_use = k;
        ws_storage.push_back({k, (int)plan.storages.size()});
        plan.storages.push_back(s);
        touch.push_back({k});
    }
    auto ordered = [&](int sa, int sb) {
        for (int x : touch[sa])
            for (int y : touch[sb])
                if (!before(x, y) || x == y) return false;
        return true;
    };
    std::vector<int> order;
    for (size_t si = 0; si < plan.storages.size(); ++si)
        if (plan.storages[si].kind == ST_ARENA && plan.storages[si].last_use >= 0) order.push_back((int)si);
    std::stable_sort(order.begin(), order.end(),
                     [&](int x, int y) { return plan.storages[x].first_use < plan.storages[y].first_use; });
    std::vector<int> placed;
    size_t arena = 0;
    for (int si : order) {
        Storage& st = plan.storages[si];
        const size_t need = align256(st.bytes);
        std::vector<std::pair<size_t, size_t>> busy;
        for (int pj : placed) {
            const Storage& o = plan.storages[pj];
            if (ordered(pj, si) || ordered(si, pj)) continue;
            busy.push_back({o.offset, o.offset + align256(o.bytes)});
        }
        std::sort(busy.begin(), busy.end());
        size_t off = 0;
        for (auto& bz : busy) {
            if (off + need <= bz.first) break;
            off = std::max(off, bz.second);
        }
        st.offset = off;
        arena = std::max(arena, off + need);
        placed.push_back(si);
    }
    plan.arena_bytes = arena;
    for (auto& w : ws_storage) plan.ops[w.first].ws_off = plan.storages[w.second].offset;
}

}

bool finalize_plan(Plan& plan, const PassInputs& e, std::string* err) {
    resolve_view_geometry(plan);
    fold_upsample(plan, e);
    assign_int8_served(plan, e);
    assign_storages(plan);
    if (!select_conv_kernels(plan, e, err) || !configure_plugins(plan, err)) return false;
    chain_sppf_pools(plan, e);
    chain_spp_parallel_pools(plan, e);
    group_convs(plan, e);
    mark_stem_pair(plan, e);
    mark_bneck_pair(plan, e);
    const std::vector<std::vector<int>> deps = op_dependencies(plan);
    assign_lanes(plan, e, deps);
    for (size_t k = 1; k < plan.ops.size(); ++k)
        if (plan.ops[k].bneck_pair && (plan.ops[k].lane != plan.ops[k - 1].lane || plan.ops[k - 1].signal)) plan.ops[k].bneck_pair = false;
    plan_arena(plan, ancestors(plan, deps, true));
    return true;
}

}
```

Baseline: 40320.

## Fuse trailing 1x1 conv into the stem-pair kernel

```diff
diff --git a/include/trtx_hip.h b/include/trtx_hip.h
--- a/include/trtx_hip.h
+++ b/include/trtx_hip.h
@@ -176,6 +176,9 @@
                                    int ld_out, int k, int stride, int pad, int act, trtx_stream_t stream);
 int32_t trtx_op_conv_stem_pair_f16(const float* in, int N, int C, int H, int W, const float* stem_w_taps_cout, const float* stem_bias, int stem_act,
                                    const void* conv_wpacked, const float* conv_bias, int conv_act, void* out, int ld_out, trtx_stream_t stream);
+int32_t trtx_op_conv_stem_pair_tail_f16(const float* in, int N, int C, int H, int W, const float* stem_w_taps_cout, const float* stem_bias, int stem_act,
+                                        const void* conv_wpacked, const float* conv_bias, int conv_act, const void* tail_wpacked, const float* tail_bias,
+                                        int tail_act, void* out, int ld_out, trtx_stream_t stream);
 int32_t trtx_op_conv_bneck_pair_f16(const void* in, int N, int H, int W, int ld_in, int in_coff, const void* w1_packed, const float* bias1, int act1,
                                     const void* w2_packed, const float* bias2, int act2, int shortcut, int act_after, void* out, int ld_out,
                                     trtx_stream_t stream);
diff --git a/tensorrtx_amd/capi.py b/tensorrtx_amd/capi.py
--- a/tensorrtx_amd/capi.py
+++ b/tensorrtx_amd/capi.py
@@ -480,6 +480,20 @@
     return out
 
 
+def conv_stem_pair_tail_f16(x, stem_w_taps_cout, stem_bias, conv_wpacked, conv_bias, tail_wpacked, tail_bias, stem_act="silu", conv_act="silu", tail_act="silu",
+                            out=None, out_ld=None):
+    import torch
+    N, C, H, W = x.shape
+    Hi, Wi = (H - 1) // 2 + 1, (W - 1) // 2 + 1
+    Ho, Wo = (Hi - 1) // 2 + 1, (Wi - 1) // 2 + 1
+    if out is None:
+        out = torch.empty((N, Ho, Wo, 32), dtype=torch.float16, device=x.device)
+    check(lib().trtx_op_conv_stem_pair_tail_f16(_p(x), N, C, H, W, _p(stem_w_taps_cout), _p(stem_bias), ACT[stem_act], _p(conv_wpacked), _p(conv_bias),
+                                                ACT[conv_act], _p(tail_wpacked), _p(tail_bias), ACT[tail_act], _p(out), out_ld or out.shape[-1], _stream()),
+          "trtx_op_conv_stem_pair_tail_f16")
+    return out
+
+
 def conv_bneck_pair_f16(x, w1_packed, bias1, w2_packed, bias2, act1="silu", act2="silu", shortcut=True, act_after="none", out=None, out_ld=None, in_coff=None,
                         mid=None):
     import torch
diff --git a/tensorrtx_amd/csrc/kernels/conv_stem_pair.hip b/tensorrtx_amd/csrc/kernels/conv_stem_pair.hip
--- a/tensorrtx_amd/csrc/kernels/conv_stem_pair.hip
+++ b/tensorrtx_amd/csrc/kernels/conv_stem_pair.hip
@@ -20,101 +20,14 @@
 __device__ __forceinline__ size_t pair_patch_bytes(int cin) { return (size_t)((cin * px::kPR * px::kPCA / 4 + 255) / 256 * 256) * 16; }
 
 __global__ __launch_bounds__(256) void conv_stem_pair_kernel(const ConvArgs ps, const ConvArgs p1, const StemGeom g, unsigned in_bytes, int total_tiles) {
-    extern __shared__ __attribute__((aligned(16))) float s_patch[];
-    char* const s_img = reinterpret_cast<char*>(s_patch) + pair_patch_bytes(ps.Cin);
-    const int tid = threadIdx.x;
-    const int lane = tid & 63;
-    const int wave = __builtin_amdgcn_readfirstlane(tid >> 6);
-    const int grp = lane >> 4, col = lane & 15;
+    constexpr bool TAIL = false;
+    const ConvArgs& pt = p1;
+#include "stem_pair_kernel_body.h"
+}
 
-    StemRegs<1, 1> R;
-    stem_setup<1, 1>(ps, g, R);
-    half8 w1[2][px::kSteps];
-    {
-        const _Float16* __restrict__ w = static_cast<const _Float16*>(p1.wgt);
-#pragma unroll
-        for (int j = 0; j < 2; ++j)
-#pragma unroll
-            for (int kt = 0; kt < px::kSteps; ++kt)
-                w1[j][kt] = *reinterpret_cast<const half8*>(w + (size_t)px::weight_row_channel(j, col) * p1.Kpad + kt * 32 + grp * 8);
-    }
-    float4 b0 = make_float4(0.f, 0.f, 0.f, 0.f), b1 = b0;
-    if (p1.bias) {
-        b0 = *reinterpret_cast<const float4*>(p1.bias + grp * 8);
-        b1 = *reinterpret_cast<const float4*>(p1.bias + grp * 8 + 4);
-    }
-    _Float16* __restrict__ out = static_cast<_Float16*>(p1.out);
-
-    auto fetch = [&](int tile) {
-        const px::Tile t = px::tile_of(tile, g.tiles_x, g.tiles_y);
-        stem_patch_fetch(ps, g, in_bytes, s_patch, t.n, px::patch_start(t.y0), px::patch_aligned_start(px::patch_start(t.x0)));
-    };
-    if ((int)blockIdx.x < total_tiles) fetch(blockIdx.x);
-    for (int tile = blockIdx.x; tile < total_tiles; tile += gridDim.x) {
-        const px::Tile t = px::tile_of(tile, g.tiles_x, g.tiles_y);
-        const int hi_start = px::patch_start(t.y0), wi_start = px::patch_start(t.x0);
-        const int al_start = px::patch_aligned_start(wi_start);
-        const int shift = wi_start - al_start;
-        asm volatile("s_waitcnt vmcnt(0)" ::: "memory");
-        __syncthreads();
-        stem_patch_tail(ps, g, s_patch, t.n, hi_start, al_start);
-        const int iy0 = px::region_start(t.y0), ix0 = px::region_start(t.x0);
-#pragma nounroll
-        for (int gi = wave; gi < px::kGroups; gi += 4) {
-            const px::RegionPixel rp = px::region_pixel(gi, lane);
-            floatx4 acc[1];
-            stem_group_mfma<1, 1>(R, s_patch + px::patch_offset(rp.ry, rp.rx, shift), acc);
-            half4 o = stem_finish4(ps, acc[0], R.bias4[0]);
-            const int iy = iy0 + rp.ry, ix = ix0 + rp.rx;
-            if ((unsigned)iy >= (unsigned)p1.H || (unsigned)ix >= (unsigned)p1.W) o = half4{0, 0, 0, 0};
-            if (rp.live) *reinterpret_cast<half4*>(s_img + px::image_offset(rp.ry, rp.rx, grp * 4)) = o;
-        }
-        __syncthreads();
-        const int next = tile + (int)gridDim.x;
-        if (next < total_tiles) fetch(next);
-        floatx4 acc[2][2];
-#pragma unroll
-        for (int i = 0; i < 2; ++i)
-#pragma unroll
-            for (int j = 0; j < 2; ++j) acc[i][j] = floatx4{0.f, 0.f, 0.f, 0.f};
-#pragma unroll
-        for (int kt = 0; kt < px::kSteps; ++kt) {
-            const int tap = px::step_tap(kt, lane);
-            half8 xf[2];
-#pragma unroll
-            for (int i = 0; i < 2; ++i) {
-                xf[i] = half8{0, 0, 0, 0, 0, 0, 0, 0};
-                if (tap < px::kTaps) xf[i] = *reinterpret_cast<const half8*>(s_img + px::frag_offset(2 * wave + i, col, tap, px::step_chunk(lane)));
-            }
-#pragma unroll
-            for (int j = 0; j < 2; ++j)
-#pragma unroll
-                for (int i = 0; i < 2; ++i) acc[i][j] = __builtin_amdgcn_mfma_f32_16x16x32_f16(w1[j][kt], xf[i], acc[i][j], 0, 0, 0);
-        }
-#pragma unroll
-        for (int i = 0; i < 2; ++i) {
-            const int ho = t.y0 + 2 * wave + i, wo = t.x0 + col;
-            if (ho >= p1.Ho || wo >= p1.Wo) continue;
-            float x[8] = {acc[i][0][0], acc[i][0][1], acc[i][0][2], acc[i][0][3], acc[i][1][0], acc[i][1][1], acc[i][1][2], acc[i][1][3]};
-            if (p1.bias) {
-                x[0] += b0.x; x[1] += b0.y; x[2] += b0.z; x[3] += b0.w;
-                x[4] += b1.x; x[5] += b1.y; x[6] += b1.z; x[7] += b1.w;
-            }
-            half8 v;
-            if (p1.act1 == ACT_SILU) {
-#pragma unroll
-                for (int e = 0; e < 8; ++e) v[e] = round_to_half(x[e] * __builtin_amdgcn_rcpf(1.0f + __expf(-x[e])));
-            } else if (p1.act1 == ACT_RELU) {
-#pragma unroll
-                for (int e = 0; e < 8; ++e) v[e] = round_to_half(x[e] > 0.f ? x[e] : 0.f);
-            } else {
-#pragma unroll
-                for (int e = 0; e < 8; ++e) v[e] = round_to_half(x[e]);
-            }
-            const size_t m = ((size_t)t.n * p1.Ho + ho) * p1.Wo + wo;
-            *reinterpret_cast<half8*>(out + m * p1.ld_out + grp * 8) = v;
-        }
-    }
+__global__ __launch_bounds__(256) void conv_stem_pair_tail_kernel(const ConvArgs ps, const ConvArgs p1, const ConvArgs pt, const StemGeom g, unsigned in_bytes, int total_tiles) {
+    constexpr bool TAIL = true;
+#include "stem_pair_kernel_body.h"
 }
 
 }
@@ -134,8 +47,24 @@
     return stem_ok && conv_ok && chained && aligned;
 }
 
-int32_t conv_stem_pair_f16(const ConvArgs& s, const ConvArgs& c, hipStream_t stream) {
-    if (!conv_stem_pair_possible(s, c) || !s.in || !s.wgt || !c.wgt || !c.out) return TRTX_ERR_UNSUPPORTED;
+bool conv_stem_pair_tail_possible(const ConvArgs& s, const ConvArgs& c, const ConvArgs& t) {
+    ConvArgs cc = c;
+    cc.out = nullptr;
+    const bool fast_act = t.act1 == ACT_SILU || t.act1 == ACT_RELU || t.act1 == ACT_NONE;
+    const bool tail_ok = !t.f32 && !t.in_i8 && !t.out_i8 && !t.res_i8 && !t.residual && !t.up_C && t.act2 == ACT_NONE && fast_act && !t.scalar_out &&
+                         t.groups == 1 && t.dil_h == 1 && t.dil_w == 1 && t.Cin == 32 && t.CinK == 32 && t.Kpad >= 32 && t.Kpad % 8 == 0 && t.Cout == 32 &&
+                         t.Cout_pad == 32 && t.kh == 1 && t.kw == 1 && t.stride_h == 1 && t.stride_w == 1 && t.pad_h == 0 && t.pad_w == 0 &&
+                         t.ld_out % 8 == 0 && t.ld_out >= 32;
+    const bool chained = t.N == c.N && t.H == c.Ho && t.W == c.Wo && t.Ho == t.H && t.Wo == t.W;
+    const bool aligned = (reinterpret_cast<uintptr_t>(t.out) & 15) == 0 && (reinterpret_cast<uintptr_t>(t.wgt) & 15) == 0 &&
+                         (reinterpret_cast<uintptr_t>(t.bias) & 15) == 0;
+    return conv_stem_pair_possible(s, cc) && tail_ok && chained && aligned;
+}
+
+namespace {
+
+template <bool TAIL>
+int32_t launch_stem_pair(const ConvArgs& s, const ConvArgs& c, const ConvArgs& t, hipStream_t stream) {
     namespace px = pairidx;
     StemGeom g;
     g.PR = px::kPR;
@@ -153,7 +82,9 @@
     if (hipGetDevice(&dev) != hipSuccess) dev = 0;
     if (resident[0] != dev || resident[1] != (int)lds || resident[2] <= 0) {
         int per_cu = 0, cus = 0;
-        if (hipOccupancyMaxActiveBlocksPerMultiprocessor(&per_cu, conv_stem_pair_kernel, 256, lds) != hipSuccess || per_cu < 1) per_cu = 1;
+        const hipError_t occ = TAIL ? hipOccupancyMaxActiveBlocksPerMultiprocessor(&per_cu, conv_stem_pair_tail_kernel, 256, lds)
+                                    : hipOccupancyMaxActiveBlocksPerMultiprocessor(&per_cu, conv_stem_pair_kernel, 256, lds);
+        if (occ != hipSuccess || per_cu < 1) per_cu = 1;
         if (hipDeviceGetAttribute(&cus, hipDeviceAttributeMultiprocessorCount, dev) != hipSuccess || cus < 1) cus = 256;
         (void)hipGetLastError();
         resident[0] = dev;
@@ -161,8 +92,23 @@
         resident[2] = per_cu * cus;
     }
     const int grid = total < resident[2] ? total : resident[2];
-    TRTX_LAUNCH(conv_stem_pair_kernel, dim3((unsigned)grid), dim3(256), lds, stream, s, c, g, in_bytes, total);
-    return check_launch("conv_stem_pair_f16");
+    if constexpr (TAIL)
+        TRTX_LAUNCH(conv_stem_pair_tail_kernel, dim3((unsigned)grid), dim3(256), lds, stream, s, c, t, g, in_bytes, total);
+    else
+        TRTX_LAUNCH(conv_stem_pair_kernel, dim3((unsigned)grid), dim3(256), lds, stream, s, c, g, in_bytes, total);
+    return check_launch(TAIL ? "conv_stem_pair_tail_f16" : "conv_stem_pair_f16");
 }
 
 }
+
+int32_t conv_stem_pair_f16(const ConvArgs& s, const ConvArgs& c, hipStream_t stream) {
+    if (!conv_stem_pair_possible(s, c) || !s.in || !s.wgt || !c.wgt || !c.out) return TRTX_ERR_UNSUPPORTED;
+    return launch_stem_pair<false>(s, c, c, stream);
+}
+
+int32_t conv_stem_pair_tail_f16(const ConvArgs& s, const ConvArgs& c, const ConvArgs& t, hipStream_t stream) {
+    if (!conv_stem_pair_tail_possible(s, c, t) || !s.in || !s.wgt || !c.wgt || !t.wgt || !t.out) return TRTX_ERR_UNSUPPORTED;
+    return launch_stem_pair<true>(s, c, t, stream);
+}
+
+}
diff --git a/tensorrtx_amd/csrc/kernels/kernels.h b/tensorrtx_amd/csrc/kernels/kernels.h
--- a/tensorrtx_amd/csrc/kernels/kernels.h
+++ b/tensorrtx_amd/csrc/kernels/kernels.h
@@ -112,6 +112,8 @@
 int32_t conv_stem_frames_f32(const ConvArgs& a, const StemFrame* frames, hipStream_t s);
 bool conv_stem_pair_possible(const ConvArgs& stem, const ConvArgs& conv);
 int32_t conv_stem_pair_f16(const ConvArgs& stem, const ConvArgs& conv, hipStream_t s);
+bool conv_stem_pair_tail_possible(const ConvArgs& stem, const ConvArgs& conv, const ConvArgs& tail);
+int32_t conv_stem_pair_tail_f16(const ConvArgs& stem, const ConvArgs& conv, const ConvArgs& tail, hipStream_t s);
 bool conv_bneck_pair_possible(const ConvArgs& first, const ConvArgs& second);
 int32_t conv_bneck_pair_f16(const ConvArgs& first, const ConvArgs& second, hipStream_t s);
 int32_t conv_bneck_pair_or_two_f16(const ConvArgs& first, const ConvArgs& second, hipStream_t s);
diff --git a/tensorrtx_amd/csrc/kernels/stem_pair_kernel_body.h b/tensorrtx_amd/csrc/kernels/stem_pair_kernel_body.h
--- /dev/null
+++ b/tensorrtx_amd/csrc/kernels/stem_pair_kernel_body.h
@@ -0,0 +1,128 @@
+    extern __shared__ __attribute__((aligned(16))) float s_patch[];
+    char* const s_img = reinterpret_cast<char*>(s_patch) + pair_patch_bytes(ps.Cin);
+    const int tid = threadIdx.x;
+    const int lane = tid & 63;
+    const int wave = __builtin_amdgcn_readfirstlane(tid >> 6);
+    const int grp = lane >> 4, col = lane & 15;
+
+    StemRegs<1, 1> R;
+    stem_setup<1, 1>(ps, g, R);
+    half8 w1[2][px::kSteps];
+    {
+        const _Float16* __restrict__ w = static_cast<const _Float16*>(p1.wgt);
+#pragma unroll
+        for (int j = 0; j < 2; ++j)
+#pragma unroll
+            for (int kt = 0; kt < px::kSteps; ++kt)
+                w1[j][kt] = *reinterpret_cast<const half8*>(w + (size_t)px::weight_row_channel(j, col) * p1.Kpad + kt * 32 + grp * 8);
+    }
+    float4 b0 = make_float4(0.f, 0.f, 0.f, 0.f), b1 = b0;
+    if (p1.bias) {
+        b0 = *reinterpret_cast<const float4*>(p1.bias + grp * 8);
+        b1 = *reinterpret_cast<const float4*>(p1.bias + grp * 8 + 4);
+    }
+    _Float16* __restrict__ out = static_cast<_Float16*>(TAIL ? pt.out : p1.out);
+    half8 wt[2];
+    float4 tb0 = make_float4(0.f, 0.f, 0.f, 0.f), tb1 = tb0;
+    if constexpr (TAIL) {
+        const _Float16* __restrict__ w = static_cast<const _Float16*>(pt.wgt);
+#pragma unroll
+        for (int j = 0; j < 2; ++j) wt[j] = *reinterpret_cast<const half8*>(w + (size_t)px::weight_row_channel(j, col) * pt.Kpad + grp * 8);
+        if (pt.bias) {
+            tb0 = *reinterpret_cast<const float4*>(pt.bias + grp * 8);
+            tb1 = *reinterpret_cast<const float4*>(pt.bias + grp * 8 + 4);
+        }
+    }
+
+    auto fetch = [&](int tile) {
+        const px::Tile t = px::tile_of(tile, g.tiles_x, g.tiles_y);
+        stem_patch_fetch(ps, g, in_bytes, s_patch, t.n, px::patch_start(t.y0), px::patch_aligned_start(px::patch_start(t.x0)));
+    };
+    if ((int)blockIdx.x < total_tiles) fetch(blockIdx.x);
+    for (int tile = blockIdx.x; tile < total_tiles; tile += gridDim.x) {
+        const px::Tile t = px::tile_of(tile, g.tiles_x, g.tiles_y);
+        const int hi_start = px::patch_start(t.y0), wi_start = px::patch_start(t.x0);
+        const int al_start = px::patch_aligned_start(wi_start);
+        const int shift = wi_start - al_start;
+        asm volatile("s_waitcnt vmcnt(0)" ::: "memory");
+        __syncthreads();
+        stem_patch_tail(ps, g, s_patch, t.n, hi_start, al_start);
+        const int iy0 = px::region_start(t.y0), ix0 = px::region_start(t.x0);
+#pragma nounroll
+        for (int gi = wave; gi < px::kGroups; gi += 4) {
+            const px::RegionPixel rp = px::region_pixel(gi, lane);
+            floatx4 acc[1];
+            stem_group_mfma<1, 1>(R, s_patch + px::patch_offset(rp.ry, rp.rx, shift), acc);
+            half4 o = stem_finish4(ps, acc[0], R.bias4[0]);
+            const int iy = iy0 + rp.ry, ix = ix0 + rp.rx;
+            if ((unsigned)iy >= (unsigned)p1.H || (unsigned)ix >= (unsigned)p1.W) o = half4{0, 0, 0, 0};
+            if (rp.live) *reinterpret_cast<half4*>(s_img + px::image_offset(rp.ry, rp.rx, grp * 4)) = o;
+        }
+        __syncthreads();
+        const int next = tile + (int)gridDim.x;
+        if (next < total_tiles) fetch(next);
+        floatx4 acc[2][2];
+#pragma unroll
+        for (int i = 0; i < 2; ++i)
+#pragma unroll
+            for (int j = 0; j < 2; ++j) acc[i][j] = floatx4{0.f, 0.f, 0.f, 0.f};
+#pragma unroll
+        for (int kt = 0; kt < px::kSteps; ++kt) {
+            const int tap = px::step_tap(kt, lane);
+            half8 xf[2];
+#pragma unroll
+            for (int i = 0; i < 2; ++i) {
+                xf[i] = half8{0, 0, 0, 0, 0, 0, 0, 0};
+                if (tap < px::kTaps) xf[i] = *reinterpret_cast<const half8*>(s_img + px::frag_offset(2 * wave + i, col, tap, px::step_chunk(lane)));
+            }
+#pragma unroll
+            for (int j = 0; j < 2; ++j)
+#pragma unroll
+                for (int i = 0; i < 2; ++i) acc[i][j] = __builtin_amdgcn_mfma_f32_16x16x32_f16(w1[j][kt], xf[i], acc[i][j], 0, 0, 0);
+        }
+#pragma unroll
+        for (int i = 0; i < 2; ++i) {
+            const int ho = t.y0 + 2 * wave + i, wo = t.x0 + col;
+            if constexpr (!TAIL)
+                if (ho >= p1.Ho || wo >= p1.Wo) continue;
+            float x[8] = {acc[i][0][0], acc[i][0][1], acc[i][0][2], acc[i][0][3], acc[i][1][0], acc[i][1][1], acc[i][1][2], acc[i][1][3]};
+            if (p1.bias) {
+                x[0] += b0.x; x[1] += b0.y; x[2] += b0.z; x[3] += b0.w;
+                x[4] += b1.x; x[5] += b1.y; x[6] += b1.z; x[7] += b1.w;
+            }
+            half8 v;
+            if (p1.act1 == ACT_SILU) {
+#pragma unroll
+                for (int e = 0; e < 8; ++e) v[e] = round_to_half(x[e] * __builtin_amdgcn_rcpf(1.0f + __expf(-x[e])));
+            } else if (p1.act1 == ACT_RELU) {
+#pragma unroll
+                for (int e = 0; e < 8; ++e) v[e] = round_to_half(x[e] > 0.f ? x[e] : 0.f);
+            } else {
+#pragma unroll
+                for (int e = 0; e < 8; ++e) v[e] = round_to_half(x[e]);
+            }
+            if constexpr (TAIL) {
+                const floatx4 z = floatx4{0.f, 0.f, 0.f, 0.f};
+                const floatx4 t0 = __builtin_amdgcn_mfma_f32_16x16x32_f16(wt[0], v, z, 0, 0, 0);
+                const floatx4 t1 = __builtin_amdgcn_mfma_f32_16x16x32_f16(wt[1], v, z, 0, 0, 0);
+                float y[8] = {t0[0], t0[1], t0[2], t0[3], t1[0], t1[1], t1[2], t1[3]};
+                if (pt.bias) {
+                    y[0] += tb0.x; y[1] += tb0.y; y[2] += tb0.z; y[3] += tb0.w;
+                    y[4] += tb1.x; y[5] += tb1.y; y[6] += tb1.z; y[7] += tb1.w;
+                }
+                if (pt.act1 == ACT_SILU) {
+#pragma unroll
+                    for (int e = 0; e < 8; ++e) v[e] = round_to_half(y[e] * __builtin_amdgcn_rcpf(1.0f + __expf(-y[e])));
+                } else if (pt.act1 == ACT_RELU) {
+#pragma unroll
+                    for (int e = 0; e < 8; ++e) v[e] = round_to_half(y[e] > 0.f ? y[e] : 0.f);
+                } else {
+#pragma unroll
+                    for (int e = 0; e < 8; ++e) v[e] = round_to_half(y[e]);
+                }
+                if (ho >= p1.Ho || wo >= p1.Wo) continue;
+            }
+            const size_t m = ((size_t)t.n * p1.Ho + ho) * p1.Wo + wo;
+            *reinterpret_cast<half8*>(out + m * (TAIL ? pt.ld_out : p1.ld_out) + grp * 8) = v;
+        }
+    }
diff --git a/tensorrtx_amd/csrc/ops_capi.cpp b/tensorrtx_amd/csrc/ops_capi.cpp
--- a/tensorrtx_amd/csrc/ops_capi.cpp
+++ b/tensorrtx_amd/csrc/ops_capi.cpp
@@ -156,6 +156,21 @@
     c.bias = conv_bias;
     c.out = out;
     return conv_stem_pair_f16(s, c, static_cast<hipStream_t>(stream));
+}
+
+extern "C" int32_t trtx_op_conv_stem_pair_tail_f16(const float* in, int N, int C, int H, int W, const float* stem_w_taps_cout, const float* stem_bias, int stem_act,
+                                                   const void* conv_wpacked, const float* conv_bias, int conv_act, const void* tail_wpacked, const float* tail_bias,
+                                                   int tail_act, void* out, int ld_out, trtx_stream_t stream) {
+    if (!in || !stem_w_taps_cout || !conv_wpacked || !tail_wpacked || !out || N < 1 || C < 1 || H < 1 || W < 1) return TRTX_ERR_INVALID;
+    const ConvArgs s = op_stem_args(in, N, C, H, W, stem_w_taps_cout, stem_bias, 16, 3, 2, 1, stem_act);
+    ConvArgs c = op_conv_args(N, s.Ho, s.Wo, 16, 16, 32, 32, 3, 3, 2, 2, 1, 1, conv_act, 0, 0, 0);
+    c.wgt = conv_wpacked;
+    c.bias = conv_bias;
+    ConvArgs t = op_conv_args(N, c.Ho, c.Wo, 32, 32, 32, ld_out, 1, 1, 1, 1, 0, 0, tail_act, 0, 0, 0);
+    t.wgt = tail_wpacked;
+    t.bias = tail_bias;
+    t.out = out;
+    return conv_stem_pair_tail_f16(s, c, t, static_cast<hipStream_t>(stream));
 }
 
 static int32_t op_bneck_pair(const void* in, int N, int H, int W, int ld_in, int in_coff, const void* w1_packed, const float* bias1, int act1, const void* w2_packed,
diff --git a/tensorrtx_amd/csrc/options.cpp b/tensorrtx_amd/csrc/options.cpp
--- a/tensorrtx_amd/csrc/options.cpp
+++ b/tensorrtx_amd/csrc/options.cpp
@@ -30,6 +30,7 @@
     o.fold_upsample = !env_is("TRTX_FOLD_UPSAMPLE", 0);
     o.stem_pair = !env_is("TRTX_STEM_PAIR", 0);
     o.bneck_pair = !env_is("TRTX_BNECK_PAIR", 0);
+    o.pair_tail = env_int("TRTX_PAIR_TAIL", 3);
     o.ws = !env_set("TRTX_CONV_NOWS");
     o.wsk = !env_set("TRTX_CONV_NOWSK");
     o.gemm256 = !env_is("TRTX_GEMM256", 0);
diff --git a/tensorrtx_amd/csrc/options.h b/tensorrtx_amd/csrc/options.h
--- a/tensorrtx_amd/csrc/options.h
+++ b/tensorrtx_amd/csrc/options.h
@@ -16,6 +16,7 @@
     bool fold_upsample = true;
     bool stem_pair = true;
     bool bneck_pair = true;
+    int pair_tail = 3;
     bool ws = true;
     bool wsk = true;
     bool gemm256 = true;
diff --git a/tensorrtx_amd/csrc/runtime/engine.cpp b/tensorrtx_amd/csrc/runtime/engine.cpp
--- a/tensorrtx_amd/csrc/runtime/engine.cpp
+++ b/tensorrtx_amd/csrc/runtime/engine.cpp
@@ -134,6 +134,25 @@
         if (c->observer || c->tuning || k + 1 >= plan.ops.size()) return false;
         const POp &o = plan.ops[k], &nx = plan.ops[k + 1];
         return nx.bneck_pair && nx.kind == OP_CONV && o.kind == OP_CONV && o.igemm && nx.lane == o.lane && nx.in[0] == o.out[0];
+    };
+    auto conv_args_of = [&](const POp& o) {
+        ConvArgs a = o.conv;
+        const PTensor& ti = plan.tensors[o.in[0]];
+        a.in = R.ptr(o.in[0]);
+        a.out = R.ptr(o.out[0]);
+        a.residual = o.in.size() > 1 ? R.ptr(o.in[1]) : nullptr;
+        a.wgt = W + o.w_off;
+        a.bias = reinterpret_cast<const float*>(W + o.b_off);
+        a.N = o.stem ? (plan.explicit_batch ? (int)ti.dims.d[0] : batch) : (ti.nfix ? ti.nfix : batch) * ti.nmul;
+        a.M = a.N * a.Ho * a.Wo;
+        return a;
+    };
+    auto tail_in_pair = [&](size_t k) {
+        if (c->frames || c->observer || c->tuning || k < 1 || k + 1 >= plan.ops.size()) return false;
+        const POp &s = plan.ops[k - 1], &p = plan.ops[k], &t = plan.ops[k + 1];
+        if (!t.pair_tail || t.kind != OP_CONV || !p.stem_pair || p.kind != OP_CONV || s.kind != OP_CONV || !s.stem || s.lane != p.lane || t.lane != p.lane) return false;
+        const ConvArgs a = conv_args_of(s), b = conv_args_of(p);
+        return conv_stem_pair_possible(a, b) && conv_stem_pair_tail_possible(a, b, conv_args_of(t));
     };
     for (size_t k = 0; k < plan.ops.size(); ++k) {
         const POp& op = plan.ops[k];
@@ -184,10 +203,11 @@
                 if (op.stem_pair && pair_pending) {
                     pair_pending = false;
                     if (prof && probes[k].start && probes[k].stop) conv_set_launch_probe(&probes[k]);
-                    st = conv_stem_pair_f16(pair_stem, a, stream);
+                    st = tail_in_pair(k) ? conv_stem_pair_tail_f16(pair_stem, a, conv_args_of(plan.ops[k + 1]), stream) : conv_stem_pair_f16(pair_stem, a, stream);
                     conv_set_launch_probe(nullptr);
                     break;
                 }
+                if (op.pair_tail && k > 0 && tail_in_pair(k - 1)) break;
                 if (defers_to_next(k)) break;
                 if (op.bneck_pair && k > 0 && defers_to_next(k - 1)) {
                     const POp& fo = plan.ops[k - 1];
diff --git a/tensorrtx_amd/csrc/runtime/plan.cpp b/tensorrtx_amd/csrc/runtime/plan.cpp
--- a/tensorrtx_amd/csrc/runtime/plan.cpp
+++ b/tensorrtx_amd/csrc/runtime/plan.cpp
@@ -38,7 +38,7 @@
         o << "\",\"flops\":" << op.flops << ",\"bytes\":" << op.bytes;
         auto conv_fields = [&](const POp& op) {
             const ConvArgs& a = op.conv;
-            o << ",\"igemm\":" << (op.igemm ? "true" : "false") << ",\"stem\":" << (op.stem ? "true" : "false") << (op.stem_pair ? ",\"stem_pair\":true" : "")
+            o << ",\"igemm\":" << (op.igemm ? "true" : "false") << ",\"stem\":" << (op.stem ? "true" : "false") << (op.stem_pair ? ",\"stem_pair\":true" : "") << (op.pair_tail ? ",\"pair_tail\":true" : "")
               << (op.bneck_pair ? ",\"bneck_pair\":true" : "") << ",\"cin\":" << (a.in_i8 ? 2 * a.Cin : a.Cin) << ",\"cout\":" << a.Cout
               << ",\"k\":[" << a.kh << "," << a.kw << "],\"stride\":[" << a.stride_h << "," << a.stride_w << "],\"hw_in\":["
               << a.H << "," << a.W << "],\"hw_out\":[" << a.Ho << "," << a.Wo << "],\"act1\":" << a.act1
diff --git a/tensorrtx_amd/csrc/runtime/plan.h b/tensorrtx_amd/csrc/runtime/plan.h
--- a/tensorrtx_amd/csrc/runtime/plan.h
+++ b/tensorrtx_amd/csrc/runtime/plan.h
@@ -95,6 +95,7 @@
     bool stem = false;
     bool stem_pair = false;
     bool bneck_pair = false;
+    bool pair_tail = false;
     bool from_deconv = false;
     bool dw = false;
     bool grouped = false;
diff --git a/tensorrtx_amd/csrc/runtime/plan_passes.cpp b/tensorrtx_amd/csrc/runtime/plan_passes.cpp
--- a/tensorrtx_amd/csrc/runtime/plan_passes.cpp
+++ b/tensorrtx_amd/csrc/runtime/plan_passes.cpp
@@ -716,6 +716,45 @@
     }
 }
 
+void mark_pair_tail(Plan& plan, const PassInputs& e) {
+    if (!(e.opt.pair_tail & 1) || e.dt != DT_F16 || e.int8 || CalibrationLowering::active()) return;
+    const int n = (int)plan.ops.size();
+    for (int k = 1; k + 1 < n; ++k) {
+        const POp &st = plan.ops[k - 1], &cv = plan.ops[k];
+        POp& tl = plan.ops[k + 1];
+        if (!cv.stem_pair || cv.out.size() != 1 || st.kind != OP_CONV || !st.stem || st.in.empty()) continue;
+        if (tl.kind != OP_CONV || !tl.igemm || tl.stem || tl.stem_pair || tl.bneck_pair || tl.from_deconv || tl.in.size() != 1 || !tl.extra_in.empty() ||
+            tl.out.size() != 1 || tl.in[0] != cv.out[0])
+            continue;
+        const PTensor &mid = plan.tensors[cv.out[0]], &dst = plan.tensors[tl.out[0]];
+        if (mid.storage < 0 || plan.storages[mid.storage].kind != ST_ARENA || is_binding_tensor(plan, mid.id) || is_binding_tensor(plan, owner_of(plan, mid.id))) continue;
+        if (dst.storage == mid.storage || dst.layout != LAY_NHWC) continue;
+        bool shared = false;
+        auto touches = [&](const POp& op) {
+            for (const std::vector<int>* v : {&op.in, &op.out, &op.extra_in})
+                for (int t : *v)
+                    if (plan.tensors[t].storage == mid.storage) return true;
+            return false;
+        };
+        for (int j = 0; j < n && !shared; ++j) {
+            if (j == k || j == k + 1) continue;
+            shared = touches(plan.ops[j]);
+            for (const POp& m : plan.ops[j].group) shared = shared || touches(m);
+        }
+        if (shared) continue;
+        ConvArgs a = st.conv, b = cv.conv, t = tl.conv;
+        const PTensor &t_in = plan.tensors[st.in[0]], &st_out = plan.tensors[st.out[0]];
+        a.N = plan.explicit_batch ? (int)t_in.dims.d[0] : plan.max_batch;
+        a.M = a.N * a.Ho * a.Wo;
+        b.N = (st_out.nfix ? st_out.nfix : plan.max_batch) * st_out.nmul;
+        b.M = b.N * b.Ho * b.Wo;
+        t.N = (mid.nfix ? mid.nfix : plan.max_batch) * mid.nmul;
+        t.M = t.N * t.Ho * t.Wo;
+        if (!conv_stem_pair_tail_possible(a, b, t)) continue;
+        tl.pair_tail = true;
+    }
+}
+
 void assign_lanes(Plan& plan, const PassInputs& e, const std::vector<std::vector<int>>& deps) {
     const int nops = (int)plan.ops.size();
     int max_lanes = e.max_aux_streams >= 0 ? 1 + e.max_aux_streams : 4;
@@ -771,6 +810,12 @@
         for (int t : op.out) mark(t);
         if (op.bneck_pair && k > 0)
             for (int t : plan.ops[k - 1].in) mark(t);
+        if (k + 1 < nops && plan.ops[k + 1].pair_tail) {
+            for (int t : plan.ops[k + 1].in) mark(t);
+            for (int t : plan.ops[k + 1].out) mark(t);
+            if (k > 0)
+                for (int t : plan.ops[k - 1].in) mark(t);
+        }
     }
     std::vector<std::pair<int, int>> ws_storage;
     for (int k = 0; k < nops; ++k) {
@@ -833,10 +878,14 @@
     group_convs(plan, e);
     mark_stem_pair(plan, e);
     mark_bneck_pair(plan, e);
+    mark_pair_tail(plan, e);
     const std::vector<std::vector<int>> deps = op_dependencies(plan);
     assign_lanes(plan, e, deps);
     for (size_t k = 1; k < plan.ops.size(); ++k)
         if (plan.ops[k].bneck_pair && (plan.ops[k].lane != plan.ops[k - 1].lane || plan.ops[k - 1].signal)) plan.ops[k].bneck_pair = false;
+    for (size_t k = 1; k < plan.ops.size(); ++k)
+        if (plan.ops[k].pair_tail && (plan.ops[k].lane != plan.ops[k - 1].lane || !plan.ops[k].wait_ops.empty() || plan.ops[k - 1].signal || !plan.ops[k - 1].stem_pair))
+            plan.ops[k].pair_tail = false;
     plan_arena(plan, ancestors(plan, deps, true));
     return true;
 }
```

After: 40070. About the same (-0.6%).
